# iangitonga/tinyllama.cpp

Measured on AMD Instinct MI355X. Metric: decode tok/s TinyLlama-1.1B q4 ctx=2048, 1 GPU; achieved HBM GB/s vs peak, higher is better.
Workload: dtype q4 weights x q8 activations (int8 dot, f32 accumulate); 1 GPU; TinyLlama-1.1B q4 greedy single-token decode, batch 1 per GPU, steps end at n=2048 (BASELINE.json configs[3]); ctx=2048, graph=True, steps_per_graph_replay=4, kv_cache=q8 blocks (reference layout), argmax=device, parallelism=replicas x1

## Files before the change

### __graft_entry__.py

```python
import importlib.util
import os
import sys

ROOT = os.path.dirname(os.path.abspath(__file__))
PKG_DIR = os.path.join(ROOT, "tinyllama.cpp_amd")
PKG_NAME = "tinyllama_cpp_amd"


def load_package():
    if PKG_NAME in sys.modules:
        return sys.modules[PKG_NAME]
    spec = importlib.util.spec_from_file_location(
        PKG_NAME, os.path.join(PKG_DIR, "__init__.py"), submodule_search_locations=[PKG_DIR])
    mod = importlib.util.module_from_spec(spec)
    sys.modules[PKG_NAME] = mod
    spec.loader.exec_module(mod)
    return mod


def build():
    pkg = load_package()
    pkg.build.build_all()
    if ROOT not in sys.path:
        sys.path.insert(0, ROOT)
    from oracle import orc
    orc.build(ref=os.path.isdir("/root/reference"))
    if os.path.isdir("/root/reference"):
        orc.build_dropin()
    build_neighbour()
    api = pkg.hipabi.GtenHip()
    for name in api.SYMBOLS + api.SAMPLE_SYMBOLS + api.SCORE_SYMBOLS + api.PREFIX_SYMBOLS + api.PREFIX_DECODE_SYMBOLS + api.BIAS_SYMBOLS + api.LOGPROBS_SYMBOLS + api.NUCLEUS_SYMBOLS + api.PENALTY_SYMBOLS + api.FSM_SYMBOLS + api.REGEX_SYMBOLS + api.PREFIXES_SYMBOLS + api.GROUPS_SYMBOLS + api.CONTINUE_SYMBOLS + api.BEAM_SYMBOLS:
        getattr(api.lib, name)
    host = pkg.hostabi.GtenHost()
    for name in host.SYMBOLS + host.SAMPLE_SYMBOLS + host.SCORE_SYMBOLS + host.PREFIX_SYMBOLS + host.PREFIX_DECODE_SYMBOLS + host.BIAS_SYMBOLS + host.LOGPROBS_SYMBOLS + host.NUCLEUS_SYMBOLS + host.PENALTY_SYMBOLS + host.FSM_SYMBOLS + host.REGEX_SYMBOLS + host.PREFIXES_SYMBOLS + host.SAMPLES_SYMBOLS + host.SESSIONS_SYMBOLS + host.BEAM_SYMBOLS:
        getattr(host.lib, name)


def build_neighbour():
    import shutil
    import subprocess
    d = os.path.join(ROOT, "tools", "mfma_neighbour")
    src, lib = os.path.join(d, "neighbour.hip"), os.path.join(d, "libneighbour.so")
    hipcc = shutil.which("hipcc") or "/opt/rocm/bin/hipcc"
    if not os.path.exists(src) or not os.path.exists(hipcc):
        return
    if not os.path.exists(lib) or os.path.getmtime(lib) < os.path.getmtime(src):
        subprocess.run([hipcc, "--offload-arch=gfx950", "-O2", "-shared", "-fPIC", "-o", lib, src], check=True, capture_output=True)


def smoke():
    if ROOT not in sys.path:
        sys.path.insert(0, ROOT)
    sys.path.insert(0, os.path.join(ROOT, "tests"))
    pkg = load_package()
    from smoke_check import run_smoke
    run_smoke(pkg)


if __name__ == "__main__":
    build()
    print("build ok")
```

### include/gten_hip_ab.h

```cpp
#pragma once

#ifdef __cplusplus
extern "C" {
#endif

int gten_hip_set_decode_attn_classic(int v);

#ifdef __cplusplus
}
#endif
```

### tinyllama.cpp_amd/build.py

```python
import os
import shutil
import subprocess

PKG = os.path.dirname(os.path.abspath(__file__))
ROOT = os.path.dirname(PKG)
CSRC = os.path.join(PKG, "csrc")
HOST = os.path.join(PKG, "host")
INCLUDE = os.path.join(ROOT, "include")

HIP_LIB = os.path.join(CSRC, "libgten_hip.so")
HOST_LIB = os.path.join(HOST, "libgten_host.so")

HIPCC = shutil.which("hipcc") or "/opt/rocm/bin/hipcc"
HIP_FLAGS = ["--offload-arch=gfx950", "-O3", "-std=c++17", "-ffp-contract=off", "-fno-slp-vectorize",
             "-Xclang", "-target-feature", "-Xclang", "-packed-fp32-ops", "-fPIC", "-shared",
             "-mllvm", "-amdgpu-kernarg-preload-count=16",
             "-Wall", "-Wno-unused-function", "-I" + INCLUDE]
CXX_FLAGS = ["-std=c++17", "-O2", "-fopenmp", "-fPIC", "-shared", "-Wall", "-I" + INCLUDE, "-I" + PKG]


_EXTRA = os.environ.get("GTEN_HIP_EXTRA_FLAGS", "").split()
HIP_FLAGS += _EXTRA
_FLAGS_STAMP = os.path.join(CSRC, "_obj", "flags.txt")


def _newer(target, sources):
    if not os.path.exists(target):
        return True
    t = os.path.getmtime(target)
    return any(os.path.getmtime(s) > t for s in sources)


def _sources(d, exts):
    out = []
    for base, _, files in os.walk(d):
        out += [os.path.join(base, f) for f in files if f.endswith(exts)]
    return sorted(out)


HIP_FILE_FLAGS = {}
HIP_OBJ = os.path.join(CSRC, "_obj")


def build_hip(force=False):
    from concurrent.futures import ThreadPoolExecutor
    srcs = _sources(CSRC, (".hip",))
    hdrs = _sources(CSRC, (".h",)) + _sources(INCLUDE, (".h",)) + [os.path.abspath(__file__)]
    os.makedirs(HIP_OBJ, exist_ok=True)
    compile_flags = [f for f in HIP_FLAGS if f != "-shared"]
    stamp = " ".join(_EXTRA)
    if (open(_FLAGS_STAMP).read() if os.path.exists(_FLAGS_STAMP) else "") != stamp:
        force = True
        with open(_FLAGS_STAMP, "w") as f:
            f.write(stamp)
    jobs, objs = [], []
    for src in srcs:
        obj = os.path.join(HIP_OBJ, os.path.basename(src) + ".o")
        objs.append(obj)
        if force or _newer(obj, [src] + hdrs):
            jobs.append([HIPCC] + compile_flags + HIP_FILE_FLAGS.get(os.path.basename(src), []) + ["-c", "-o", obj, src])
    if jobs:
        with ThreadPoolExecutor(max_workers=4) as pool:
            for r in pool.map(lambda cmd: subprocess.run(cmd, capture_output=True, text=True), jobs):
                if r.returncode != 0:
                    raise RuntimeError("hipcc failed: " + " ".join(r.args) + "\n" + r.stderr[-4000:])
    if jobs or force or _newer(HIP_LIB, objs):
        subprocess.run([HIPCC, "--offload-arch=gfx950", "-shared", "-fPIC", "-o", HIP_LIB] + objs, check=True)
    return HIP_LIB


HOST_CLI = os.path.join(HOST, "tinyllama_cli")
CLI_SRC = os.path.join(HOST, "tinyllama_cli.cpp")


def build_host(force=False):
    srcs = [s for s in _sources(HOST, (".cpp",)) if s != CLI_SRC]
    if not srcs:
        return None
    deps = srcs + _sources(HOST, (".h",)) + _sources(os.path.join(PKG, "gten"), (".h",)) + _sources(INCLUDE, (".h",))
    if force or _newer(HOST_LIB, deps) or _newer(HOST_LIB, [HIP_LIB]):
        subprocess.run(["g++"] + CXX_FLAGS + ["-o", HOST_LIB] + srcs +
                       ["-L" + CSRC, "-lgten_hip", "-Wl,-rpath,$ORIGIN/../csrc"], check=True)
    if os.path.exists(CLI_SRC) and (force or _newer(HOST_CLI, deps + [CLI_SRC]) or _newer(HOST_CLI, [HIP_LIB])):
        cli_flags = [f for f in CXX_FLAGS if f not in ("-shared", "-fPIC")]
        subprocess.run(["g++"] + cli_flags + ["-o", HOST_CLI, CLI_SRC, "-L" + CSRC, "-lgten_hip", "-Wl,-rpath,$ORIGIN/../csrc"], check=True)
    return HOST_LIB


def build_all(force=False):
    build_hip(force)
    build_host(force)
```

### tinyllama.cpp_amd/csrc/gten_decode.hip

```cpp
#include "gten_dev.h"
#include "gten_rt.h"
#include "gten_hip_sample.h"
#include "gten_hip_bias.h"
#include "gten_hip_logprobs.h"
#include "gten_hip_nucleus.h"
#include "gten_hip_penalty.h"
#include "gten_hip_fsm.h"
#include "gten_hip_regex.h"
#include "gten_hip_ab.h"
#include "gten_hip_prefix_decode.h"
#include "gten_hip_prefixes.h"
#include "gten_hip_groups.h"

#include <cmath>
#include <vector>
#include <algorithm>

#define DEC_SHARE_RECORDS (GTEN_PREFIXES_MAX + GTEN_GROUPS_MAX)

using namespace gtd;

extern __shared__ __attribute__((aligned(16))) uint8_t g_smem[];

#define DEC_CHUNK 256
#define ATT1V_VROW 68
#define ATT1V_PCOL 72
#define DEC_MAX_LANES 4
#define DEC_ATT_MAXCH 8
#define GEMVM_F16_LDS_LIMIT 65536

static int g_only_family = -1;
#define DEC_LAUNCH(tag, kernel, grid, block, smem, ...)                                        \
    do {                                                                                       \
        if (g_only_family < 0 || g_only_family == (tag)) GTR_LAUNCH(tag, kernel, grid, block, smem, __VA_ARGS__); \
    } while (0)

#define DEC_LAUNCH_HOT(tag, kernel, grid, block, smem, hw, a) \
    DEC_LAUNCH(tag, kernel, grid, block, smem, (hw).w[0], (hw).w[1], (hw).w[2], (hw).w[3], (hw).w[4], (hw).w[5], (hw).w[6], a)

struct DecStep {
    int n;
    int advance;
    int stop;
};


struct ActStage {
    float* row;
    float* red;
    ActQ8 q8;
};

__device__ __forceinline__ ActStage carve_stage(int d)
{
    ActStage s;
    s.red = (float*)g_smem;
    s.row = (float*)(g_smem + 64);
    s.q8 = actq8_carve(g_smem + 64 + (size_t)d * 4, d >> 5);
    return s;
}
static size_t stage_bytes(int d) { return 64 + (size_t)d * 4 + (size_t)(d >> 5) * 40; }

enum { PRO_EMBED = 0, PRO_RESID = 1, PRO_ATT = 2, PRO_ATTW = 3, PRO_ACTQ8 = 4 };
enum { EPI_RAW = 0, EPI_SILUMUL = 1, EPI_STAGE = 2, EPI_STAGE_FRAG = 3 };

#define WXP_PLANES 8
#include "gten_decode_wx.h"
#include "gten_decode_wide_wx.h"
#include "gten_decode_ffn.h"
#include "gten_decode_wxp.h"
#include "gten_decode_attn.h"
#include "gten_decode_attn_w.h"
#include "gten_decode_attn_exact64.h"
#include "gten_decode_attn_wide.h"
#include "gten_decode_attn_hm.h"
#include "gten_decode_sample.h"
#include "gten_decode_logprobs.h"
static_assert(LP_TOP == GTEN_HIP_LOGPROBS_TOP && sizeof(LpRecord) == GTEN_HIP_LOGPROBS_RECORD_BYTES, "gten_decode_logprobs.h and include/gten_hip_logprobs.h disagree");
#include "gten_decode_nucleus.h"
static_assert(CUT_MASS_BITS == GTEN_HIP_NUCLEUS_MASS_BITS && sizeof(CutInfo) == GTEN_HIP_NUCLEUS_INFO_BYTES && sizeof(CutInfo) == sizeof(gten_hip_cut_info),
              "gten_decode_nucleus.h and include/gten_hip_nucleus.h disagree");
#include "gten_decode_penalty.h"
#include "gten_decode_fsm.h"


using namespace gtr;

struct CapturedGraph { hipGraph_t graph; hipGraphExec_t exec; };

struct SamplerState {
    SampleParam* samp = nullptr;
    std::vector<SampleParam> samp_host;
    int n_sampling = 0;
    float* bias = nullptr;
    int n_bound = 0;
    bool bias_on = false;
    LpRecord* lp = nullptr;
    int n_asking = 0;
    bool lp_on = false;
    CutParam* cut = nullptr;
    std::vector<CutParam> cut_host;
    bool cut_on = false;
    PenParam* pen = nullptr;
    std::vector<PenParam> pen_host;
    int n_penalised = 0;
    size_t pen_lds = 0;
    bool pen_on = false;
    uint16_t* fsm_next = nullptr;
    uint8_t* fsm_flags = nullptr;
    std::vector<uint8_t> fsm_flags_host;
    int fsm_states = 0;
    FsmParam* fsm = nullptr;
    std::vector<FsmParam> fsm_host;
    int32_t* fsm_state = nullptr;
    int n_fsm = 0;
    bool fsm_on = false;
    uint8_t* vocab_bytes = nullptr;
    int32_t* vocab_offsets = nullptr;
    long long vocab_n_bytes = 0;
};

struct gten_hip_decoder {
    gten_hip_decoder_desc d;
    std::vector<gten_hip_layer_ptrs> layers;
    DecStep* step = nullptr;
    int32_t* tokens = nullptr;
    int32_t* result = nullptr;
    int32_t* ids_stage = nullptr;
    float *qkv_raw = nullptr, *proj_raw = nullptr, *down_raw = nullptr;
    float *scores = nullptr, *stats = nullptr, *att_part = nullptr;
    uint8_t *xbuf = nullptr, *hbuf = nullptr;
    float* act_f = nullptr;
    int8_t* act_q = nullptr;
    float* act_d = nullptr;
    int* act_sum = nullptr;
    float* best_val = nullptr;
    int* best_idx = nullptr;
    int n_best = 0;
    std::vector<DecStep> slots;
    int dev_n = -1;
    std::vector<int> dev_ns;
    int only_family = -1;
    int n_seq = 1;
    const void** kv_tab = nullptr;
    std::vector<const void*> kv_real;
    std::vector<char> kv_parked;
    void* dummy_kv = nullptr;
    int8_t* stg_q = nullptr;
    float* stg_d = nullptr;
    int* stg_sum = nullptr;
    float* stg_f = nullptr;
    float* logits_m = nullptr;
    float* gu_raw = nullptr;
    int n_chunks = 0;
    CapturedGraph graphs[2][2][1 << DEC_MAX_LANES] = {};
    SamplerState smp;
    unsigned lane_mask = 0;
    int last_run_lanes = 0;
    const float2* rope = nullptr;
    float2* rope_now = nullptr;
    bool exact = false;
    int attn_classic = 0;
    bool persist_on = false;
    struct PersistState* persist = nullptr;
    uint8_t* hm = nullptr;
    size_t hm_seq_stride = 0, hm_cache_bytes = 0, hm_chunk_bytes = 0;
    std::vector<char> hm_dirty;
    unsigned long long hm_imports = 0, hm_import_launches = 0;
    struct Pfx {
        uint8_t* hm = nullptr;
        const void** tab = nullptr;
        DecStep* step = nullptr;
        std::vector<const void*> kv;
        int len = 0;
        char dirty = 0;
        bool stale = false;
        unsigned long long imports = 0;
    } pfx[DEC_SHARE_RECORDS];
    int* share_dev = nullptr;
    int* which_dev = nullptr;
    uint8_t** pfx_hm_tab = nullptr;
    bool pfxn = false;
    std::vector<int> share_rows, share_cur, share_which, which_cur;
    unsigned long long hm_skip_imports = 0;
    unsigned long long watch_epoch = 0;
    bool watch_foreign = false;
    int lanes = 1;
    hipStream_t lane_stream[DEC_MAX_LANES] = {nullptr, nullptr, nullptr, nullptr};
    hipEvent_t lane_fork = nullptr, lane_join[DEC_MAX_LANES] = {nullptr, nullptr, nullptr, nullptr};
    struct BeamSearch* beam = nullptr;
};
static hipError_t beam_destroy(gten_hip_decoder* dc);

static inline bool sampler_on(const gten_hip_decoder* dc) { return dc->smp.n_sampling + dc->smp.n_bound + dc->smp.n_asking + dc->smp.n_penalised + dc->smp.n_fsm > 0; }

struct StepEnd {
    int rows;
    const float* logits; int row_stride;
    const SampleParam* samp;
    DecStep* step;
    int32_t* result; int result_stride;
    int32_t* tokens;
    LpRecord* lp;
    const CutParam* cut;
    const PenParam* pen;
    const FsmParam* fsm; int32_t* fsm_state;
    const float* best_val; const int* best_idx; int n_best, best_stride;
};

static int launch_step_end(gten_hip_decoder* dc, const StepEnd& e)
{
    const SamplerState& s = dc->smp;
    const int V = dc->d.n_vocab, tok_stride = dc->d.max_ctx + 1, rec_stride = dc->d.max_ctx + 2;
    const dim3 grid(e.rows), block(SMP_THREADS);
    const bool on = sampler_on(dc);
    if (on && s.fsm_on)
        DEC_LAUNCH(KT_DEC_SAMPLE, k_dec_sample_fsm, grid, block, s.pen_lds, e.logits, V, e.row_stride, e.samp, e.step, e.result, e.result_stride, e.tokens,
                   tok_stride, (const float*)s.bias, e.lp, rec_stride, e.cut, e.pen, (const uint16_t*)s.fsm_next, (const uint8_t*)s.fsm_flags, s.fsm_states,
                   e.fsm, e.fsm_state);
    else if (on && s.pen_on)
        DEC_LAUNCH(KT_DEC_SAMPLE, k_dec_sample_pen, grid, block, s.pen_lds, e.logits, V, e.row_stride, e.samp, e.step, e.result, e.result_stride, e.tokens,
                   tok_stride, (const float*)s.bias, e.lp, rec_stride, e.cut, e.pen);
    else if (on && s.cut_on)
        DEC_LAUNCH(KT_DEC_SAMPLE, k_dec_sample_cut, grid, block, 0, e.logits, V, e.row_stride, e.samp, e.step, e.result, e.result_stride, e.tokens, tok_stride,
                   (const float*)s.bias, e.lp, rec_stride, e.cut);
    else if (on && s.lp_on)
        DEC_LAUNCH(KT_DEC_SAMPLE, k_dec_sample_lp, grid, block, 0, e.logits, V, e.row_stride, e.samp, e.step, e.result, e.result_stride, e.tokens, tok_stride,
                   (const float*)s.bias, e.lp, rec_stride);
    else if (on && s.bias_on)
        DEC_LAUNCH(KT_DEC_SAMPLE, k_dec_sample_b, grid, block, 0, e.logits, V, e.row_stride, e.samp, e.step, e.result, e.result_stride, e.tokens, tok_stride,
                   (const float*)s.bias);
    else if (on)
        DEC_LAUNCH(KT_DEC_SAMPLE, k_dec_sample, grid, block, 0, e.logits, V, e.row_stride, e.samp, e.step, e.result, e.result_stride, e.tokens, tok_stride);
    else
        DEC_LAUNCH(KT_DEC_ARGMAX, k_dec_argmax, grid, dim3(1024), 0, e.best_val, e.best_idx, e.n_best, e.step, e.result, e.best_stride, e.result_stride,
                   e.tokens, tok_stride);
    return 0;
}

struct LaneBufs {
    int n_seq;
    DecStep* step; int32_t* tokens; int32_t* result; const SampleParam* samp; LpRecord* lp; const CutParam* cut; const PenParam* pen;
    const FsmParam* fsm; int32_t* fsm_state;
    float *qkv_raw, *proj_raw, *down_raw, *scores, *stats, *att_part;
    uint8_t *xbuf, *hbuf;
    float* act_f; int8_t* act_q; float* act_d; int* act_sum;
    const void** kv_tab;
    int8_t* stg_q; float* stg_d; int* stg_sum; float* stg_f;
    float* logits_m; float* gu_raw; float2* rope_now;
};
static LaneBufs lane_bufs(const gten_hip_decoder* dc, int lane)
{
    const gten_hip_decoder_desc& d = dc->d;
    const size_t SL = (size_t)(dc->n_seq / dc->lanes), o = (size_t)lane * SL;
    const size_t E = (size_t)d.n_embd, F = (size_t)d.n_ffn, dh = E / d.n_heads, KV = dh * d.n_kv_heads, V = (size_t)d.n_vocab;
    const size_t planes = dc->n_seq >= 16 ? 2 : 1, H = (size_t)d.n_heads, C = (size_t)dc->n_chunks;
    LaneBufs b;
    b.n_seq = (int)SL;
    b.step = dc->step + o; b.tokens = dc->tokens + o * (d.max_ctx + 1); b.result = dc->result + o * (d.max_ctx + 2); b.samp = dc->smp.samp + o;
    b.lp = dc->smp.lp ? dc->smp.lp + o * (d.max_ctx + 2) : nullptr;
    b.cut = dc->smp.cut ? dc->smp.cut + o : nullptr;
    b.pen = dc->smp.pen ? dc->smp.pen + o : nullptr;
    b.fsm = dc->smp.fsm ? dc->smp.fsm + o : nullptr;
    b.fsm_state = dc->smp.fsm_state ? dc->smp.fsm_state + o * (d.max_ctx + 2) : nullptr;
    const size_t rplanes = dc->n_seq >= 16 ? (size_t)WXP_PLANES : 1;
    b.qkv_raw = dc->qkv_raw + o * rplanes * (E + 2 * KV);
    b.proj_raw = dc->proj_raw + o * rplanes * E; b.down_raw = dc->down_raw + o * rplanes * E;
    b.scores = dc->scores + o * H * d.max_ctx; b.stats = dc->stats + o * H * C * 2; b.att_part = dc->att_part + o * H * C * dh;
    b.xbuf = dc->xbuf + o * E * 4; b.hbuf = dc->hbuf + o * E * 4;
    b.act_f = dc->act_f + o * F; b.act_q = dc->act_q + o * 2 * F; b.act_d = dc->act_d + o * (F / 32); b.act_sum = dc->act_sum + o * (F / 32);
    b.kv_tab = dc->kv_tab ? dc->kv_tab + o * d.n_layers * 2 : nullptr;
    b.stg_q = dc->stg_q ? dc->stg_q + o * 2 * E : nullptr; b.stg_d = dc->stg_d ? dc->stg_d + o * (E / 32) : nullptr;
    b.stg_sum = dc->stg_sum ? dc->stg_sum + o * (E / 32) : nullptr; b.stg_f = dc->stg_f ? dc->stg_f + o * E : nullptr;
    b.logits_m = dc->logits_m ? dc->logits_m + o * V : nullptr; b.gu_raw = dc->gu_raw ? dc->gu_raw + o * planes * 2 * F : nullptr;
    b.rope_now = dc->rope_now + o * (dh / 2);
    return b;
}

static bool g_decode_exact = false;
static bool g_exact_now = false;
static bool g_lane_skip = false;
static bool g_kv_head_major = true;
#define PFX_SHARED_DEFAULT true
static bool g_pfx_shared = PFX_SHARED_DEFAULT;
struct PfxArgs { const uint8_t* k = nullptr; const int* share = nullptr; const uint8_t* const* tab = nullptr; size_t layer_off = 0; const int* which = nullptr; };
extern "C" int gten_hip_set_kv_head_major(int on)
{
    g_kv_head_major = on != 0;
    return 0;
}
extern "C" int gten_hip_set_decode_exact(int on)
{
    g_decode_exact = on != 0;
    return 0;
}
static int g_attn_classic = 0;
static int g_attn_classic_now = 0;
extern "C" int gten_hip_set_decode_attn_classic(int v)
{
    GTR_REQUIRE(v >= 0 && v <= 2, "gten_hip_set_decode_attn_classic: %d is not 0, 1 or 2", v);
    g_attn_classic = v;
    return 0;
}

static bool attention_grouped_ok(const AttnArgs& t, int n_seq)
{
    const int grp = t.n_heads / t.n_kv;
    const int min_seq = 8;
    if (t.adtype == GTEN_F16 && n_seq < 16) return false;
    return n_seq >= min_seq && (t.adtype == GTEN_Q8 || t.adtype == GTEN_F16) && t.d_head == 64 && (grp == 8 || grp == 4 || grp == 2 || grp == 1);
}

static int grp_shift1_of(int n_heads, int n_kv)
{
    const int grp = n_heads / n_kv;
    return (grp > 0 && (grp & (grp - 1)) == 0) ? __builtin_ctz(grp) + 1 : 0;
}

static bool attention_one_pass(int d_head);

static bool grouped_mm(const AttnArgs& t, int n_seq)
{
    return n_seq >= 16 && t.adtype == GTEN_Q8 && t.d_head == 64 && !g_exact_now;
}

static bool grouped_hm_f16(const AttnArgs& t, int n_seq)
{
    return n_seq >= 16 && t.adtype == GTEN_F16 && t.d_head == 64 && t.hm_k && !g_exact_now;
}

static bool grouped_one_pass(const AttnArgs& t, int n_seq)
{
    if (grouped_mm(t, n_seq) || grouped_hm_f16(t, n_seq)) return true;
    return attention_one_pass(t.d_head) && t.adtype == GTEN_Q8 && n_seq <= 8;
}

template <int GRP, int ADT>
static int launch_attention_g(const AttnArgs& t, int n_seq, const PfxArgs& pfx)
{
    constexpr size_t NW = (ADT == GTEN_Q8) ? 17 : 32;
    const dim3 grid(n_seq, t.n_chunks, t.n_kv);
    if constexpr (ADT == GTEN_Q8) if (grouped_mm(t, n_seq) && t.hm_k) {
        const int n_cq = (t.n_chunks + HM_WAVES - 1) / HM_WAVES;
        if (pfx.tab) {
            if (n_seq >= 128)
                DEC_LAUNCH(KT_DEC_ATTN_SCORE, (k_dec_attn_hm_pfxn<GRP, true>), dim3(n_seq * n_cq * t.n_kv), dim3(64 * HM_WAVES), 2048, t, n_seq, n_cq, pfx.tab, pfx.layer_off, pfx.share, pfx.which);
            else
                DEC_LAUNCH(KT_DEC_ATTN_SCORE, (k_dec_attn_hm_pfxn<GRP, false>), dim3(n_seq * n_cq * t.n_kv), dim3(64 * HM_WAVES), 2048, t, n_seq, n_cq, pfx.tab, pfx.layer_off, pfx.share, pfx.which);
            return 0;
        }
        if (pfx.k) {
            if (n_seq >= 128)
                DEC_LAUNCH(KT_DEC_ATTN_SCORE, (k_dec_attn_hm_pfx<GRP, true>), dim3(n_seq * n_cq * t.n_kv), dim3(64 * HM_WAVES), 2048, t, n_seq, n_cq, pfx.k, pfx.share);
            else
                DEC_LAUNCH(KT_DEC_ATTN_SCORE, (k_dec_attn_hm_pfx<GRP, false>), dim3(n_seq * n_cq * t.n_kv), dim3(64 * HM_WAVES), 2048, t, n_seq, n_cq, pfx.k, pfx.share);
            return 0;
        }
        if (n_seq >= 128) DEC_LAUNCH(KT_DEC_ATTN_SCORE, (k_dec_attn_hm<GRP, true>), dim3(n_seq * n_cq * t.n_kv), dim3(64 * HM_WAVES), 2048, t, n_seq, n_cq);
        else DEC_LAUNCH(KT_DEC_ATTN_SCORE, (k_dec_attn_hm<GRP, false>), dim3(n_seq * n_cq * t.n_kv), dim3(64 * HM_WAVES), 2048, t, n_seq, n_cq);
        return 0;
    }
    if constexpr (ADT == GTEN_Q8) if (grouped_mm(t, n_seq)) {
        const size_t smem = (size_t)DEC_CHUNK * 68 + 2 * 8 * 264 * 2 + 16 * 64 + 32 * 4 + 8 * 4 + (size_t)4 * (DEC_MAXGRP + 2) * 2 + 128 + 128 * 4 + 80 + 64;
        GTR_REQUIRE((n_seq * t.n_chunks) % 8 == 0, "decoder: %d sequences x %d chunks is not a multiple of 8", n_seq, t.n_chunks);
        DEC_LAUNCH(KT_DEC_ATTN_SCORE, (k_dec_attn_mm_g<GRP>), dim3(n_seq * t.n_chunks * t.n_kv), dim3(256), smem, t, n_seq);
        return 0;
    }
    if constexpr (ADT == GTEN_Q8) if (grouped_one_pass(t, n_seq)) {
        constexpr size_t GP = (GRP + 1) / 2;
        const size_t smem = (size_t)(8 * GRP + 4 * GRP + 8 + 64) * 4 + (size_t)4 * (GRP + 2) * 2 + (size_t)(GRP + 2) * 64 + 16 +
                            (ADT == GTEN_Q8 ? 0 : (size_t)(GRP + 1) * 64 * 4) + 2 * GP * DEC_CHUNK * 4 + (size_t)DEC_CHUNK * NW * 4;
        DEC_LAUNCH(KT_DEC_ATTN_SCORE, (k_dec_attn_one_g<GRP, true, ADT>), grid, dim3(256), smem, t);
        return 0;
    }
    const size_t smem1 = (size_t)(8 * GRP + 4 * GRP + 8 + 64) * 4 + (size_t)4 * (GRP + 2) * 2 + (size_t)(GRP + 2) * 64 + 64 +
                         (ADT == GTEN_Q8 ? 0 : (size_t)(GRP + 1) * 64 * 4 + 16);
    const size_t smem2 = (size_t)((GRP + 1) / 2 * 2) * DEC_CHUNK * 4 + (size_t)DEC_CHUNK * NW * 4 + (size_t)(16 + 8 * GRP) * 4;
    const bool exact = n_seq <= 8 || g_exact_now;
    if (smem2 > 64 * 1024) {
        GTR_CHECK(hipFuncSetAttribute((const void*)k_dec_attn_pv_g<GRP, true, ADT>, hipFuncAttributeMaxDynamicSharedMemorySize, (int)smem2));
        GTR_CHECK(hipFuncSetAttribute((const void*)k_dec_attn_pv_g<GRP, false, ADT>, hipFuncAttributeMaxDynamicSharedMemorySize, (int)smem2));
    }
    if constexpr (ADT == GTEN_F16) if (grouped_hm_f16(t, n_seq)) {
        const int n_cq = (t.n_chunks + HM_WAVES - 1) / HM_WAVES;
// ... 74 lines not shown
            if (g_attn_classic_now == 0) {
                if (t.adtype == GTEN_Q8) {
                    GTR_CHECK(hipFuncSetAttribute((const void*)k_dec_attn_one64w<GTEN_Q8>, hipFuncAttributeMaxDynamicSharedMemorySize, (int)smem_v));
                    DEC_LAUNCH_HOT(KT_DEC_ATTN_SCORE, k_dec_attn_one64w<GTEN_Q8>, g64, dim3(512), smem_v, hw, t);
                } else {
                    GTR_CHECK(hipFuncSetAttribute((const void*)k_dec_attn_one64w<GTEN_F16>, hipFuncAttributeMaxDynamicSharedMemorySize, (int)smem_v));
                    DEC_LAUNCH_HOT(KT_DEC_ATTN_SCORE, k_dec_attn_one64w<GTEN_F16>, g64, dim3(512), smem_v, hw, t);
                }
                return 0;
            }
            if (t.adtype == GTEN_Q8) {
                GTR_CHECK(hipFuncSetAttribute((const void*)k_dec_attn_one64v<GTEN_Q8>, hipFuncAttributeMaxDynamicSharedMemorySize, (int)smem_v));
                DEC_LAUNCH_HOT(KT_DEC_ATTN_SCORE, k_dec_attn_one64v<GTEN_Q8>, g64, dim3(256), smem_v, hw, t);
            } else {
                GTR_CHECK(hipFuncSetAttribute((const void*)k_dec_attn_one64v<GTEN_F16>, hipFuncAttributeMaxDynamicSharedMemorySize, (int)smem_v));
                DEC_LAUNCH_HOT(KT_DEC_ATTN_SCORE, k_dec_attn_one64v<GTEN_F16>, g64, dim3(256), smem_v, hw, t);
            }
            return 0;
        }
        if (t.adtype == GTEN_Q8) {
            if (multi) DEC_LAUNCH_HOT(KT_DEC_ATTN_SCORE, (k_dec_attn_one64<GTEN_Q8, true>), g64, dim3(256), smem, hw, t);
            else DEC_LAUNCH_HOT(KT_DEC_ATTN_SCORE, (k_dec_attn_one64<GTEN_Q8, false>), g64, dim3(256), smem, hw, t);
        } else {
            if (multi) DEC_LAUNCH_HOT(KT_DEC_ATTN_SCORE, (k_dec_attn_one64<GTEN_F16, true>), g64, dim3(256), smem, hw, t);
            else DEC_LAUNCH_HOT(KT_DEC_ATTN_SCORE, (k_dec_attn_one64<GTEN_F16, false>), g64, dim3(256), smem, hw, t);
        }
        return 0;
    }
    if (t.d_head == 64) {
        const size_t nw = (t.adtype == GTEN_Q8) ? 17 : 32;
        const size_t smem2 = (size_t)2 * DEC_CHUNK * 4 + (size_t)DEC_CHUNK * nw * 4;
        const unsigned long long geo = (unsigned long long)(unsigned)t.kv_pitch | ((unsigned long long)(unsigned)t.max_ctx << 32);
        const unsigned long long heads = ((unsigned long long)(unsigned)t.n_heads << 32) | ((unsigned long long)(unsigned)t.n_kv << 40) |
                                         ((unsigned long long)(unsigned)t.grp_shift1 << 48);
        const AttnHotWords hs{{(unsigned long long)(uintptr_t)t.qkv_raw, (unsigned long long)(uintptr_t)t.rope_now, (unsigned long long)(uintptr_t)t.kcache,
                               (unsigned long long)(uintptr_t)t.step, geo, (unsigned long long)(unsigned)t.n_embd | heads, (unsigned long long)(uintptr_t)t.scores}};
        const AttnHotWords hp{{(unsigned long long)(uintptr_t)t.scores, (unsigned long long)(uintptr_t)t.stats, (unsigned long long)(uintptr_t)t.vcache,
                               (unsigned long long)(uintptr_t)t.step, geo, (unsigned long long)(unsigned)t.n_chunks | heads, (unsigned long long)(uintptr_t)t.att_part}};
        const bool multi = agrid.z > 1 || t.kv_tab != nullptr;
        const dim3 g64(agrid.y, agrid.x, agrid.z);
#define ATT_LAUNCH2(ADT, MULTI)                                                                                                          \
        do {                                                                                                                             \
            DEC_LAUNCH_HOT(KT_DEC_ATTN_SCORE, (k_dec_attn_score64<ADT, MULTI>), g64, dim3(256), smem1, hs, t);                           \
            DEC_LAUNCH_HOT(KT_DEC_ATTN_PV, (k_dec_attn_pv64<ADT, MULTI>), g64, dim3(256), smem2, hp, t);                                 \
        } while (0)
        if (t.adtype == GTEN_Q8) { if (multi) ATT_LAUNCH2(GTEN_Q8, true); else ATT_LAUNCH2(GTEN_Q8, false); }
        else { if (multi) ATT_LAUNCH2(GTEN_F16, true); else ATT_LAUNCH2(GTEN_F16, false); }
#undef ATT_LAUNCH2
        return 0;
    }
    DEC_LAUNCH(KT_DEC_ATTN_SCORE, k_dec_attn_score, agrid, dim3(256), smem1, t);
    DEC_LAUNCH(KT_DEC_ATTN_PV, k_dec_attn_pv, agrid, dim3(256), (size_t)2 * DEC_CHUNK * 4, t);
    return 0;
}

template <int WT, int PRO>
static GemvHotWords hot_of(const Gemv8Args& a)
{
    GemvHotWords hw;
    GemvHot& h = hw.h;
    if (PRO == PRO_RESID) { h.p0 = a.res_raw; h.p1 = a.res_a; h.p2 = a.norm_w; }
    else if (PRO == PRO_EMBED) { h.p0 = a.table; h.p1 = a.tokens; h.p2 = a.norm_w; }
    else if (PRO == PRO_ATT || PRO == PRO_ATTW) {
        h.p0 = a.att_part; h.p1 = (const void*)(uintptr_t)((unsigned)a.d_head_shift | ((unsigned)a.n_chunks << 8));
        h.p2 = (PRO == PRO_ATTW) ? a.att_stats : nullptr;
    }
    else { h.p0 = (WT == GTEN_F16) ? (const void*)a.act_f : (const void*)a.act_q; h.p1 = a.act_d; h.p2 = a.act_sum; }
    h.qs0 = a.qs[0]; h.ds0 = a.ds[0]; h.d_in = a.d_in; h.rows0 = a.rows[0]; h.step = a.step;
    return hw;
}

template <int WT, int PRO>
static GemvHotWords hot_of_gemv8(const Gemv8Args& a)
{
    GemvHotWords hw = hot_of<WT, PRO>(a);
    const unsigned long long r1 = a.n_mats > 1 ? (unsigned)a.rows[1] : 0u, r2 = a.n_mats > 2 ? (unsigned)a.rows[2] : 0u;
    hw.w[4] = (unsigned long long)(uintptr_t)(a.n_mats > 1 ? a.qs[1] : nullptr);
    hw.w[5] = (unsigned long long)(unsigned)a.d_in | ((unsigned long long)(unsigned)a.rows[0] << 16) | (r1 << 32) | (r2 << 48);
    hw.w[6] = (PRO == PRO_RESID) ? (unsigned long long)(uintptr_t)(a.n_mats > 2 ? a.qs[2] : nullptr) : (unsigned long long)(uintptr_t)a.step;
    return hw;
}

template <int WT, int PRO, int NCH, int R, int NT, int NM = 0>
static int launch_gemv8(int tag, const Gemv8Args& a, int total_rows)
{
    const int rows_per_wg = (NT / 64) * R;
    const dim3 grid((total_rows + rows_per_wg - 1) / rows_per_wg), block(NT);
    for (int k = 0; k + 1 < a.n_mats; k++) GTR_REQUIRE(a.rows[k] % R == 0, "decoder: concatenated matrices must hold a multiple of %d rows", R);
    const GemvHotWords hw = hot_of_gemv8<WT, PRO>(a);
    DEC_LAUNCH_HOT(tag, (k_dec_gemv8<WT, PRO, NCH, R, EPI_RAW, NT, NM>), grid, block, stage_bytes((PRO == PRO_ACTQ8 && WT != GTEN_F16) ? 32 : a.d_in), hw, a);
    return 0;
}

template <int WT>
static int launch_gateup8(const Gemv8Args& a, int n_ffn)
{
    const dim3 grid(n_ffn / 32), block(512);
    GTR_REQUIRE(n_ffn % 32 == 0, "decoder: n_ffn %d is not a multiple of 32", n_ffn);
    const GemvHotWords hw = hot_of_gemv8<WT, PRO_RESID>(a);
    DEC_LAUNCH_HOT(KT_DEC_GEMV_GATEUP, (k_dec_gemv8<WT, PRO_RESID, (WT == GTEN_F16 ? 4 : 1), 8, EPI_SILUMUL, 512>), grid, block, stage_bytes(a.d_in), hw, a);
    return 0;
}

static void set_mat(Gemv8Args& a, int k, const void* w, int wdtype, int rows, int cols)
{
    const size_t nb = (size_t)cols / 32;
    a.qs[k] = (const uint8_t*)w;
    a.ds[k] = (wdtype == GTEN_F16) ? nullptr
                                   : (const uint16_t*)((const uint8_t*)w + (size_t)rows * nb * (wdtype == GTEN_Q4 ? 16 : 32));
    a.rows[k] = rows;
}

template <int WT>
static int enqueue_step_q8act(gten_hip_decoder* dc)
{
    const gten_hip_decoder_desc& d = dc->d;
    const int E = d.n_embd, F = d.n_ffn, dh = E / d.n_heads, KV = dh * d.n_kv_heads;
    const size_t kv_pitch = gten_hip_row_bytes(d.adtype, KV);
    constexpr bool F16W = (WT == GTEN_F16);
    constexpr int NE = F16W ? 4 : 1;
    constexpr int NF = F16W ? 11 : 3;
    constexpr int NF12 = F16W ? 12 : NF;
    const bool wideF = F > 2048, widerF = F16W && F > NF * 512;
    float* xbuf = (float*)dc->xbuf;
    float* hbuf = (float*)dc->hbuf;
    int rc;
    for (int l = 0; l < d.n_layers; l++) {
        const gten_hip_layer_ptrs& L = dc->layers[l];
        Gemv8Args a{};
        a.step = dc->step; a.d_in = E; a.n_mats = 3;
        set_mat(a, 0, L.wq, WT, E, E); set_mat(a, 1, L.wk, WT, KV, E); set_mat(a, 2, L.wv, WT, KV, E);
        a.out = dc->qkv_raw; a.norm_w = (const uint16_t*)L.attn_norm; a.x_out = xbuf;
        if (l == 0) {
            a.table = d.embed; a.rope = dc->rope; a.rope_now = dc->rope_now; a.rope_half = dh / 2; a.n_vocab = d.n_vocab; a.tokens = dc->tokens;
            rc = launch_gemv8<WT, PRO_EMBED, NE, 2, 512>(KT_DEC_GEMV_QKV, a, E + 2 * KV);
        } else {
            a.res_a = hbuf; a.res_raw = dc->down_raw;
            rc = launch_gemv8<WT, PRO_RESID, NE, 2, 512>(KT_DEC_GEMV_QKV, a, E + 2 * KV);
        }
        if (rc) return rc;
        AttnArgs t{};
        t.step = dc->step; t.qkv_raw = dc->qkv_raw; t.kcache = (uint8_t*)L.kcache; t.vcache = (uint8_t*)L.vcache;
        t.kv_pitch = kv_pitch; t.scores = dc->scores; t.stats = dc->stats; t.att_part = dc->att_part; t.rope = dc->rope; t.rope_now = dc->rope_now;
        t.adtype = d.adtype; t.n_heads = d.n_heads; t.n_kv = d.n_kv_heads; t.d_head = dh; t.max_ctx = d.max_ctx;
        t.n_chunks = dc->n_chunks; t.n_embd = E;
        const dim3 agrid(d.n_heads, dc->n_chunks);
        const size_t smem1 = (size_t)(16 + 3 * dh + 16) * 4 + 32 + (size_t)3 * dh + 64;
        if (int arc = launch_attention(t, agrid, smem1)) return arc;
        Gemv8Args o{};
        o.step = dc->step; o.d_in = E; o.n_mats = 1; set_mat(o, 0, L.wo, WT, E, E); o.out = dc->proj_raw;
        o.att_part = dc->att_part; o.d_head = dh; o.d_head_shift = __builtin_ctz(dh); o.n_chunks = dc->n_chunks;
        o.att_stats = dc->stats;
        rc = attention_one_pass(dh) ? launch_gemv8<WT, PRO_ATTW, NE, 1, 512, 1>(KT_DEC_GEMV_O, o, E)
                                    : launch_gemv8<WT, PRO_ATT, NE, 1, 512, 1>(KT_DEC_GEMV_O, o, E);
        if (rc) return rc;
        Gemv8Args gu{};
        gu.step = dc->step; gu.d_in = E; gu.n_mats = 2; set_mat(gu, 0, L.wgate, WT, F, E); set_mat(gu, 1, L.wup, WT, F, E);
        gu.res_a = xbuf; gu.res_raw = dc->proj_raw; gu.x_out = hbuf; gu.norm_w = (const uint16_t*)L.ffn_norm;
        gu.act_q = dc->act_q; gu.act_d = dc->act_d; gu.act_sum = dc->act_sum; gu.act_f = dc->act_f;
        if ((rc = launch_gateup8<WT>(gu, F))) return rc;
        Gemv8Args dn{};
        dn.step = dc->step; dn.d_in = F; dn.n_mats = 1; set_mat(dn, 0, L.wdown, WT, E, F); dn.out = dc->down_raw;
        dn.act_q = dc->act_q; dn.act_d = dc->act_d; dn.act_sum = dc->act_sum;
        dn.act_f = dc->act_f;
        rc = widerF ? launch_gemv8<WT, PRO_ACTQ8, NF12, 2, 256, 1>(KT_DEC_GEMV_DOWN, dn, E)
             : wideF ? launch_gemv8<WT, PRO_ACTQ8, NF, 2, 256, 1>(KT_DEC_GEMV_DOWN, dn, E)
                     : launch_gemv8<WT, PRO_ACTQ8, NE, 2, 256, 1>(KT_DEC_GEMV_DOWN, dn, E);
        if (rc) return rc;
    }
    Gemv8Args hd{};
    hd.step = dc->step; hd.d_in = E; hd.n_mats = 1; set_mat(hd, 0, d.lm_head, WT, d.n_vocab, E); hd.out = d.logits;
    hd.res_a = hbuf; hd.res_raw = dc->down_raw; hd.x_out = nullptr; hd.norm_w = (const uint16_t*)d.final_norm;
    hd.best_val = dc->best_val; hd.best_idx = dc->best_idx;
    if ((rc = launch_gemv8<WT, PRO_RESID, NE, F16W ? 4 : 8, 512, 1>(KT_DEC_GEMV_HEAD, hd, d.n_vocab))) return rc;
    return launch_step_end(dc, StepEnd{1, d.logits, 0, dc->smp.samp, dc->step, dc->result, 0, dc->tokens, dc->smp.lp, dc->smp.cut, dc->smp.pen, dc->smp.fsm, dc->smp.fsm_state,
                                       dc->best_val, dc->best_idx, dc->n_best, 0});
}

template <int WT, int PRO>
static int launch_stage(int tag, Gemv8Args a, int n_seq)
{
    const GemvHotWords hw = hot_of_gemv8<WT, PRO>(a);
    DEC_LAUNCH_HOT(tag, (k_dec_gemv8<WT, PRO, 1, 1, EPI_STAGE, 512>), dim3(n_seq), dim3(512), stage_bytes(a.d_in), hw, a);
    return 0;
}

template <int WT, int PRO>
static int launch_stage_frag(int tag, Gemv8Args a, int n_seq)
{
    a.frag_rt = (n_seq + 15) / 16;
    const GemvHotWords hw = hot_of_gemv8<WT, PRO>(a);
    DEC_LAUNCH_HOT(tag, (k_dec_gemv8<WT, PRO, 1, 1, EPI_STAGE_FRAG, 512>), dim3(n_seq), dim3(512), stage_bytes(a.d_in), hw, a);
    return 0;
}

static size_t gemvm_lds_bytes(int wt, int n_seq, int d, bool silumul)
{
    size_t b = silumul ? (size_t)n_seq * 64 * 4 : 0;
    if (wt == GTEN_F16) b += ((size_t)n_seq * ((d + 511) / 512 * 512) * 4 <= GEMVM_F16_LDS_LIMIT) ? (size_t)n_seq * d * 4 : 0;
    else b += (size_t)n_seq * (d + (size_t)(d / 32) * 8);
    return b + 16;
}

template <int WT, int NCH, int R, int S, int NT>
static int launch_gemvm(int tag, const Gemv8Args& a, int total_rows)
{
    const int rows_per_wg = (NT / 64) * R;
    for (int k = 0; k + 1 < a.n_mats; k++) GTR_REQUIRE(a.rows[k] % R == 0, "decoder: concatenated matrices must hold a multiple of %d rows", R);
    const GemvHotWords hw = hot_of<WT, PRO_ACTQ8>(a);
    const size_t lds = gemvm_lds_bytes(WT, S, a.d_in, false);
    static bool raised = false;
    if (lds > 64 * 1024 && !raised) {
        GTR_CHECK(hipFuncSetAttribute((const void*)k_dec_gemvm<WT, NCH, R, S, EPI_RAW, NT>, hipFuncAttributeMaxDynamicSharedMemorySize, (int)lds));
        raised = true;
    }
    DEC_LAUNCH_HOT(tag, (k_dec_gemvm<WT, NCH, R, S, EPI_RAW, NT>), dim3((total_rows + rows_per_wg - 1) / rows_per_wg), dim3(NT), lds, hw, a);
    return 0;
}

template <int WT, int S>
static int enqueue_step_multi(gten_hip_decoder* dc)
{
    const gten_hip_decoder_desc& d = dc->d;
    const int E = d.n_embd, F = d.n_ffn, dh = E / d.n_heads, KV = dh * d.n_kv_heads, V = d.n_vocab;
    const size_t kv_pitch = gten_hip_row_bytes(d.adtype, KV);
    constexpr bool F16W = (WT == GTEN_F16);
    constexpr int NE = F16W ? 4 : 1, NF = F16W ? 11 : 3, NF12 = F16W ? 12 : NF;
    constexpr int RH = F16W ? 2 : 4;
    const bool wideF = F > 2048, widerF = F16W && F > NF * 512;
    float* xbuf = (float*)dc->xbuf;
    float* hbuf = (float*)dc->hbuf;
    int rc;
    Gemv8Args base{};
    base.step = dc->step; base.tok_stride = d.max_ctx + 1; base.part_stride = d.n_heads * dc->n_chunks * dh;
    base.best_stride = dc->n_best;
    for (int l = 0; l < d.n_layers; l++) {
        const gten_hip_layer_ptrs& L = dc->layers[l];
        Gemv8Args st = base;
        st.d_in = E; st.norm_w = (const uint16_t*)L.attn_norm; st.x_out = xbuf;
        st.act_q = dc->stg_q; st.act_d = dc->stg_d; st.act_sum = dc->stg_sum; st.act_f = dc->stg_f;
        if (l == 0) {
            st.table = d.embed; st.rope = dc->rope; st.rope_now = dc->rope_now; st.rope_half = dh / 2; st.n_vocab = V; st.tokens = dc->tokens;
            rc = launch_stage<WT, PRO_EMBED>(KT_DEC_STAGE, st, S);
        } else {
            st.res_a = hbuf; st.res_raw = dc->down_raw; st.raw_stride = E;
            rc = launch_stage<WT, PRO_RESID>(KT_DEC_STAGE, st, S);
        }
        if (rc) return rc;
        Gemv8Args a = base;
        a.d_in = E; a.n_mats = 3;
        set_mat(a, 0, L.wq, WT, E, E); set_mat(a, 1, L.wk, WT, KV, E); set_mat(a, 2, L.wv, WT, KV, E);
        a.out = dc->qkv_raw; a.raw_stride = E + 2 * KV;
        a.act_q = dc->stg_q; a.act_d = dc->stg_d; a.act_sum = dc->stg_sum; a.act_f = dc->stg_f;
        if ((rc = launch_gemvm<WT, NE, 2, S, 256>(KT_DEC_GEMV_QKV, a, E + 2 * KV))) return rc;
        AttnArgs t{};
        t.step = dc->step; t.qkv_raw = dc->qkv_raw; t.kv_pitch = kv_pitch; t.scores = dc->scores; t.stats = dc->stats;
        t.att_part = dc->att_part; t.rope = dc->rope; t.rope_now = dc->rope_now;
// ... 642 lines not shown
    dc->layers.assign(layers, layers + d.n_layers);
    dc->n_chunks = (d.max_ctx + DEC_CHUNK - 1) / DEC_CHUNK;
    static_assert(GTEN_ROPE_MAX_POS <= DEC_ATT_MAXCH * DEC_CHUNK, "max_ctx (checked above) bounds the attention chunks the consumers request up front");
    const int E = d.n_embd, F = d.n_ffn, KV = dh * d.n_kv_heads;
    const size_t S = (size_t)n_seq;
    GTR_CHECK(hipMalloc((void**)&dc->step, S * sizeof(DecStep)));
    GTR_CHECK(hipMemset(dc->step, 0, S * sizeof(DecStep)));
    GTR_CHECK(hipMalloc((void**)&dc->tokens, S * (size_t)(d.max_ctx + 1) * 4));
    GTR_CHECK(hipMemset(dc->tokens, 0, S * (size_t)(d.max_ctx + 1) * 4));
    GTR_CHECK(hipMalloc((void**)&dc->result, S * (size_t)(d.max_ctx + 2) * 4));
    GTR_CHECK(hipMemset(dc->result, 0, S * (size_t)(d.max_ctx + 2) * 4));
    GTR_CHECK(hipMalloc((void**)&dc->smp.samp, S * sizeof(SampleParam)));
    GTR_CHECK(hipMemset(dc->smp.samp, 0, S * sizeof(SampleParam)));
    dc->smp.samp_host.assign(S, SampleParam{});
    const size_t planes = wide ? 2 : 1;
    GTR_CHECK(hipMalloc((void**)&dc->qkv_raw, (wide ? (size_t)WXP_PLANES : 1) * S * (size_t)(E + 2 * KV) * 4));
    GTR_CHECK(hipMalloc((void**)&dc->proj_raw, (wide ? (size_t)WXP_PLANES : 1) * S * (size_t)E * 4));
    GTR_CHECK(hipMalloc((void**)&dc->down_raw, (wide ? (size_t)WXP_PLANES : 1) * S * (size_t)E * 4));
    GTR_CHECK(hipMalloc((void**)&dc->scores, S * (size_t)d.n_heads * d.max_ctx * 4));
    GTR_CHECK(hipMalloc((void**)&dc->stats, (S * (size_t)d.n_heads * dc->n_chunks * 2 + 16) * 4));
    GTR_CHECK(hipMemset(dc->stats, 0, (S * (size_t)d.n_heads * dc->n_chunks * 2 + 16) * 4));
    GTR_CHECK(hipMalloc((void**)&dc->att_part, S * (size_t)d.n_heads * dc->n_chunks * dh * 4));
    GTR_CHECK(hipMalloc((void**)&dc->xbuf, S * (size_t)E * 4));
    GTR_CHECK(hipMalloc((void**)&dc->hbuf, S * (size_t)E * 4));
    const size_t stage_rows = wide ? 2 * ((S + 15) / 16 * 16) : S;
    GTR_CHECK(hipMalloc((void**)&dc->act_q, stage_rows * (size_t)F));
    GTR_CHECK(hipMemset(dc->act_q, 0, stage_rows * (size_t)F));
    GTR_CHECK(hipMalloc((void**)&dc->act_d, S * (size_t)(F / 32) * 4));
    GTR_CHECK(hipMalloc((void**)&dc->act_sum, S * (size_t)(F / 32) * 4));
    GTR_CHECK(hipMalloc((void**)&dc->act_f, S * (size_t)F * 4));
    {
        const int r = (n_seq == 1) ? (d.wdtype == GTEN_F16 ? 4 : 8) : (d.wdtype == GTEN_F16 ? 2 : 4);
        dc->n_best = ((d.n_vocab + 8 * r - 1) / (8 * r)) * 8;
    }
    GTR_CHECK(hipMalloc((void**)&dc->best_val, S * (size_t)dc->n_best * 4));
    GTR_CHECK(hipMalloc((void**)&dc->best_idx, S * (size_t)dc->n_best * 4));
    if (n_seq > 1) {
        GTR_CHECK(hipMalloc((void**)&dc->stg_q, stage_rows * (size_t)E));
        GTR_CHECK(hipMemset(dc->stg_q, 0, stage_rows * (size_t)E));
        GTR_CHECK(hipMalloc((void**)&dc->stg_d, S * (size_t)(E / 32) * 4));
        GTR_CHECK(hipMalloc((void**)&dc->stg_sum, S * (size_t)(E / 32) * 4));
        GTR_CHECK(hipMalloc((void**)&dc->stg_f, S * (size_t)E * 4));
        GTR_CHECK(hipMalloc((void**)&dc->logits_m, S * (size_t)d.n_vocab * 4));
        if (wide) {
            GTR_CHECK(hipMalloc((void**)&dc->gu_raw, planes * S * (size_t)2 * F * 4));
            if (d.wdtype != GTEN_F16)
            {
                if (int rc = (d.wdtype == GTEN_Q4) ? mmv_prepare<GTEN_Q4>() : mmv_prepare<GTEN_Q8>()) return rc;
                if (int rc = (d.wdtype == GTEN_Q4) ? mmvh_prepare<GTEN_Q4>() : mmvh_prepare<GTEN_Q8>()) return rc;
            }
        }
        std::vector<const void*> tab(S * d.n_layers * 2);
        for (size_t q = 0; q < S; q++)
            for (int l = 0; l < d.n_layers; l++) {
                const gten_hip_kv_ptrs& p = kv[q * d.n_layers + l];
                tab[(q * d.n_layers + l) * 2] = p.kcache;
                tab[(q * d.n_layers + l) * 2 + 1] = p.vcache;
            }
        GTR_CHECK(hipMalloc((void**)&dc->kv_tab, tab.size() * sizeof(void*)));
        GTR_CHECK(hipMemcpy(dc->kv_tab, tab.data(), tab.size() * sizeof(void*), hipMemcpyHostToDevice));
        dc->kv_real = tab;
        dc->kv_parked.assign(S, 0);
        const size_t cache_bytes = (size_t)d.max_ctx * gten_hip_row_bytes(d.adtype, KV);
        GTR_CHECK(hipMalloc(&dc->dummy_kv, 2 * cache_bytes));
        GTR_CHECK(hipMemset(dc->dummy_kv, 0, 2 * cache_bytes));
        const int grp = d.n_heads / d.n_kv_heads;
        if (wide && g_kv_head_major && !dc->exact && (d.adtype == GTEN_Q8 || d.adtype == GTEN_F16) && dh == 64 && (grp == 8 || grp == 4 || grp == 2 || grp == 1)) {
            dc->hm_chunk_bytes = d.adtype == GTEN_Q8 ? HM_CHUNK_BYTES : HMF_CHUNK_BYTES;
            dc->hm_cache_bytes = (size_t)d.n_kv_heads * dc->n_chunks * dc->hm_chunk_bytes;
            dc->hm_seq_stride = (size_t)d.n_layers * 2 * dc->hm_cache_bytes;
            GTR_CHECK(hipMalloc((void**)&dc->hm, S * dc->hm_seq_stride));
            GTR_CHECK(hipMemset(dc->hm, 0, S * dc->hm_seq_stride));
            dc->hm_dirty.assign(S, 1);
            for (size_t q = 0; q < S; q++)
                for (size_t i = 0; i < (size_t)d.n_layers * 2; i++)
                    kv_watch_add(dc->kv_real[q * d.n_layers * 2 + i], cache_bytes, dc, &dc->hm_dirty[q]);
        }
    }
    if (int rc = rope_table(dh, &dc->rope)) return rc;
    GTR_CHECK(hipMalloc((void**)&dc->rope_now, S * (size_t)(dh / 2) * sizeof(float2)));
    GTR_CHECK(hipMemset(dc->rope_now, 0, S * (size_t)(dh / 2) * sizeof(float2)));
    if (dc->persist_on && n_seq == 1 && !dc->exact)
        if (int rc = persist_prepare(dc)) return rc;
    return 0;
}

#if GTEN_WITH_PERSIST
static int g_cu_count = -1;
static int persist_prepare(gten_hip_decoder* dc)
{
    if (dc->persist) return 0;
    if (!g_persist_all.empty()) { dc->persist_on = false; return 0; }
    if (g_cu_count < 0) {
        int dev = 0;
        GTR_CHECK(hipGetDevice(&dev));
        hipDeviceProp_t prop;
        GTR_CHECK(hipGetDeviceProperties(&prop, dev));
        g_cu_count = prop.multiProcessorCount;
    }
    const gten_hip_decoder_desc& d = dc->d;
    if (!persist_supported(d, dc->n_seq, dc->n_chunks, g_cu_count)) { dc->persist_on = false; return 0; }
    const int G = g_cu_count, E = d.n_embd, F = d.n_ffn, dh = E / d.n_heads, KV = dh * d.n_kv_heads;
    auto* ps = new PersistState;
    dc->persist = ps;
    g_persist_all.push_back(ps);
    std::vector<PLayer> tab((size_t)d.n_layers);
    for (int l = 0; l < d.n_layers; l++) {
        const gten_hip_layer_ptrs& L = dc->layers[l];
        tab[l] = PLayer{(const uint8_t*)L.wq, (const uint8_t*)L.wk, (const uint8_t*)L.wv, (const uint8_t*)L.wo, (const uint8_t*)L.wgate,
                        (const uint8_t*)L.wup, (const uint8_t*)L.wdown, (const uint16_t*)L.attn_norm, (const uint16_t*)L.ffn_norm,
                        (uint8_t*)L.kcache, (uint8_t*)L.vcache};
    }
    GTR_CHECK(hipMalloc((void**)&ps->layers, tab.size() * sizeof(PLayer)));
    GTR_CHECK(hipMemcpy(ps->layers, tab.data(), tab.size() * sizeof(PLayer), hipMemcpyHostToDevice));
    GTR_CHECK(hipMalloc((void**)&ps->ctl, 64));
    const unsigned ctl0[16] = {1u, 0u};
    GTR_CHECK(hipMemcpy(ps->ctl, ctl0, 64, hipMemcpyHostToDevice));
    PArgs& a = ps->args;
    a.rpa = (E + 2 * KV + G - 1) / G; a.rpo = (E + G - 1) / G; a.rph = (d.n_vocab + G - 1) / G; a.rw = (a.rph + 7) / 8;
    const size_t n_q = (size_t)G * a.rpa, n_part = (size_t)d.n_heads * dc->n_chunks * 66, n_att = (size_t)E, n_proj = (size_t)G * a.rpo,
                 n_act = (size_t)10 * (F / 32) + 8, n_down = (size_t)G * a.rpo, n_best = (size_t)2 * G;
    const size_t total = n_q + n_part + n_att + n_proj + n_act + n_down + n_best + 64;
    GTR_CHECK(hipMalloc((void**)&ps->gran, total * 8));
    GTR_CHECK(hipMemset(ps->gran, 0, total * 8));
    pu64* p = ps->gran;
    a.gq = p; p += n_q; a.gpart = p; p += n_part; a.gatt = p; p += n_att; a.gproj = p; p += n_proj;
    a.gact = p; p += (n_act + 7) / 8 * 8; a.gdown = p; p += n_down; a.gbest = p;
    if (const char* e = getenv("GTEN_HIP_PERSIST_STAMPS"); e && e[0] == '1') {
        ps->n_stamps = d.n_layers * 20 + 8;
        GTR_CHECK(hipMalloc((void**)&ps->stamps, (size_t)(d.n_layers * 20 + 8) * 4));
        GTR_CHECK(hipMemset(ps->stamps, 0, (size_t)(d.n_layers * 20 + 8) * 4));
    }
    a.layers = ps->layers; a.step = dc->step; a.tokens = dc->tokens; a.result = dc->result;
    a.embed = (const uint8_t*)d.embed; a.final_norm = (const uint16_t*)d.final_norm; a.lm_head = (const uint8_t*)d.lm_head;
    a.logits = d.logits; a.rope = dc->rope; a.ctl = ps->ctl; a.stamps = ps->stamps;
    a.n_layers = d.n_layers; a.E = E; a.F = F; a.KV = KV; a.n_heads = d.n_heads; a.n_kv = d.n_kv_heads; a.n_vocab = d.n_vocab;
    a.max_ctx = d.max_ctx; a.n_chunks = dc->n_chunks; a.kv_pitch = (int)gten_hip_row_bytes(d.adtype, KV);
    ps->grid = G;
    ps->smem = persist_smem();
    GTR_CHECK(hipFuncSetAttribute((const void*)k_dec_persist<GTEN_Q4>, hipFuncAttributeMaxDynamicSharedMemorySize, (int)ps->smem));
    return 0;
}
static hipError_t persist_free(gten_hip_decoder* dc)
{
    if (!dc->persist) return hipSuccess;
    PersistState* ps = dc->persist;
    g_persist_all.erase(std::remove(g_persist_all.begin(), g_persist_all.end(), ps), g_persist_all.end());
    hipError_t first = hipSuccess;
    for (void* b : {(void*)ps->layers, (void*)ps->ctl, (void*)ps->gran, (void*)ps->stamps})
        if (b) { const hipError_t e = hipFree(b); if (e != hipSuccess && first == hipSuccess) first = e; }
    delete ps;
    dc->persist = nullptr;
    return first;
}
#else
static int persist_prepare(gten_hip_decoder* dc) { dc->persist_on = false; return 0; }
static hipError_t persist_free(gten_hip_decoder*) { return hipSuccess; }
#endif

static hipError_t drop_graphs(gten_hip_decoder* dc)
{
    hipError_t first = hipSuccess;
    auto rel = [&](hipError_t e) { if (e != hipSuccess && first == hipSuccess) first = e; };
    for (auto& by_steps : dc->graphs)
        for (auto& by_slot : by_steps)
            for (CapturedGraph& c : by_slot) {
// ... 978 lines not shown
```

### tinyllama.cpp_amd/csrc/gten_decode_wx.h

```cpp

template <typename T>
__device__ __forceinline__ const T* from_word(unsigned long long w)
{
    return (const T*)(const __attribute__((address_space(1))) T*)w;
}
template <typename T>
__device__ __forceinline__ void store_global(void* p, T v)
{
    *(__attribute__((address_space(1))) T*)(uintptr_t)p = v;
}

struct Gemv8Args {
    const DecStep* step;
    const uint8_t* qs[3];
    const uint16_t* ds[3];
    int rows[3];
    int n_mats;
    int d_in;
    float* out;
    const void* table; int n_vocab; const int32_t* tokens;
    const float* res_a; const float* res_raw;
    float* x_out;
    const uint16_t* norm_w;
    const float* att_part; int d_head, n_chunks;
// ... 83 lines not shown
{
    float amax = 0.f;
#pragma unroll
    for (int i = 0; i < EPT; i++) amax = fmaxf(amax, fabsf(v[i]));
    const Q8Scale s = q8_scale_from_absmax(grp_max<EPT>(amax));
    int q[EPT], sum = 0;
#pragma unroll
    for (int i = 0; i < EPT; i++) { q[i] = q8_round(v[i], s.scale); sum += q[i]; }
    const int k = sub * EPT;
    if (a.h16) {
        uint16_t* hd = (uint16_t*)a.q + ((((size_t)b * a.rt + (a.row >> 4)) * 64 + (k >> 3) * 16 + (a.row & 15)) * 8 + (k & 7));
        unsigned hw[EPT / 2];
#pragma unroll
        for (int i = 0; i < EPT; i += 4) {
            hw[i / 2] = (unsigned)f2h((float)q[i] * s.ddeq) | ((unsigned)f2h((float)q[i + 2] * s.ddeq) << 16);
            hw[i / 2 + 1] = (unsigned)f2h((float)q[i + 1] * s.ddeq) | ((unsigned)f2h((float)q[i + 3] * s.ddeq) << 16);
        }
        if (EPT == 8) *(uint4*)hd = make_uint4(hw[0], hw[1], hw[EPT / 2 - 2], hw[EPT / 2 - 1]);
        else *(uint2*)hd = make_uint2(hw[0], hw[1]);
        return;
    }
    int8_t* dst = a.q + ((((size_t)b * a.rt + (a.row >> 4)) * 64 + (k >> 3) * 16 + (a.row & 15)) * 8 + (k & 7));
    const int lo = (q[0] & 0xff) | ((q[1] & 0xff) << 8) | ((q[2] & 0xff) << 16) | ((q[3] & 0xff) << 24);
    if (EPT == 8) {
        int2 pk;
        pk.x = lo;
        pk.y = (q[EPT - 4] & 0xff) | ((q[EPT - 3] & 0xff) << 8) | ((q[EPT - 2] & 0xff) << 16) | ((q[EPT - 1] & 0xff) << 24);
        *(int2*)dst = pk;
    } else {
        *(int*)dst = lo;
    }
    sum = grp_sum_i<EPT>(sum);
    if (sub == 0) { a.d[(size_t)b * 16 * a.rt + a.row] = s.ddeq; a.sum[(size_t)b * 16 * a.rt + a.row] = sum; }
}

template <int EPT> __device__ __forceinline__ void ldN(const float* p, float (&v)[EPT])
{
    const float4 a = ((const float4*)p)[0];
    v[0] = a.x; v[1] = a.y; v[2] = a.z; v[3] = a.w;
    if (EPT == 8) {
        const float4 b = ((const float4*)p)[1];
        v[EPT - 4] = b.x; v[EPT - 3] = b.y; v[EPT - 2] = b.z; v[EPT - 1] = b.w;
    }
}
template <int EPT> __device__ __forceinline__ void stN(float* p, const float (&v)[EPT])
{
    ((float4*)p)[0] = make_float4(v[0], v[1], v[2], v[3]);
    if (EPT == 8) ((float4*)p)[1] = make_float4(v[EPT - 4], v[EPT - 3], v[EPT - 2], v[EPT - 1]);
}
template <int EPT> __device__ __forceinline__ float sumsq_treeN(const float (&v)[EPT])
{
    float s = (v[0] * v[0] + v[1] * v[1]) + (v[2] * v[2] + v[3] * v[3]);
    if (EPT == 8) s = s + ((v[EPT - 4] * v[EPT - 4] + v[EPT - 3] * v[EPT - 3]) + (v[EPT - 2] * v[EPT - 2] + v[EPT - 1] * v[EPT - 1]));
    return s;
}

__device__ __forceinline__ float max32(float v) { return nn_max32(v); }
__device__ __forceinline__ int sum32_i(int v) { return sum32_lanes_i(v); }
__device__ __forceinline__ float q8_round32(float v)
{
    const Q8Scale s = q8_scale_from_absmax(max32(fabsf(v)));
    return (float)q8_round(v, s.scale) * s.ddeq;
}
__device__ __forceinline__ float act_round32(float v, bool f16)
{
    return f16 ? h2f(f2h(v)) : q8_round32(v);
}

struct GemvHot {
    const void* p0;
    const void* p1;
    const void* p2;
    const uint8_t* qs0; const uint16_t* ds0;
    int d_in, rows0;
    const DecStep* step;
};
static_assert(sizeof(GemvHot) == 56, "seven 64-bit scalars: the preloadable part of the argument segment");
union GemvHotWords {
    unsigned long long w[7];
    GemvHot h;
    __host__ __device__ GemvHotWords() : w{0, 0, 0, 0, 0, 0, 0} {}
};

template <int WT, int PRO, int NCH, int R, int EPI, int NT, int NM = 0>
__global__ __launch_bounds__(NT) void k_dec_gemv8(const unsigned long long h0, const unsigned long long h1, const unsigned long long h2,
                                                  const unsigned long long h3, const unsigned long long h4, const unsigned long long h5,
                                                  const unsigned long long h6, const Gemv8Args a)
{
    GemvHot hot;
    hot.p0 = from_word<void>(h0); hot.p1 = from_word<void>(h1); hot.p2 = from_word<void>(h2);
    hot.qs0 = from_word<uint8_t>(h3);
    const uint8_t* hot_qs1 = from_word<uint8_t>(h4);
    hot.d_in = (int)(h5 & 0xffffu); hot.rows0 = (int)((h5 >> 16) & 0xffffu);
    const int hot_rows1 = (int)((h5 >> 32) & 0xffffu), hot_rows2 = (int)(h5 >> 48);
    const uint8_t* hot_qs2 = (PRO == PRO_RESID) ? from_word<uint8_t>(h6) : a.qs[2];
    hot.step = (PRO == PRO_RESID) ? nullptr : from_word<DecStep>(h6);
    constexpr int WBYTES = (WT == GTEN_Q4) ? 16 : 32;
    hot.ds0 = (const uint16_t*)(hot.qs0 + (size_t)hot.rows0 * (hot.d_in >> 5) * WBYTES);
    constexpr int EPT = 2048 / NT;
    constexpr int LPB = 32 / EPT;
    constexpr int NW = NT / 64;
    static_assert(NT == 256 || NT == 512, "256 or 512 threads");
    static_assert(EPI != EPI_SILUMUL || NT == 512, "the FFN slice epilogue wants 8 waves");
    constexpr bool F16W = (WT == GTEN_F16);
    const int d = hot.d_in, nb = d >> 5;
    ActStage s = carve_stage((PRO == PRO_ACTQ8 && !F16W) ? 32 : d);
    const int lane = threadIdx.x & 63, wid = threadIdx.x >> 6;
    constexpr bool STG = (EPI == EPI_STAGE || EPI == EPI_STAGE_FRAG);
    const int seq = STG ? blockIdx.x : 0;
    const int n = (PRO == PRO_RESID) ? 0 : hot.step[seq].n;
    const float* res_raw = (const float*)hot.p0 + (size_t)seq * a.raw_stride;
    const float* res_a = (const float*)hot.p1 + (size_t)seq * d;
    float* x_out = a.x_out ? a.x_out + (size_t)seq * d : nullptr;
    const int32_t* tokens = (const int32_t*)hot.p1 + (size_t)seq * a.tok_stride;
    constexpr bool ATT = (PRO == PRO_ATT || PRO == PRO_ATTW);
    const float* att_part = (const float*)hot.p0 + (size_t)seq * a.part_stride;
    const float* att_stats = (const float*)hot.p2 + (size_t)seq * a.stats_stride;
    const uint16_t* norm_w = (const uint16_t*)hot.p2;
    const int att_shift = (int)((uintptr_t)hot.p1 & 0xff), att_chunks = (int)(((uintptr_t)hot.p1 >> 8) & 0xffff), att_dh = 1 << att_shift;
    if (STG) {
        s.q8.q = a.act_q + (size_t)seq * d;
        s.q8.d = a.act_d + (size_t)seq * nb;
        s.q8.sum = a.act_sum + (size_t)seq * nb;
        if (F16W) s.row = a.act_f + (size_t)seq * d;
    }
    const bool stores_x = STG || blockIdx.x == 0;
    const int gi = threadIdx.x, base = gi * EPT, blk = gi / LPB, sub = gi % LPB;
    const bool on = base < d;
    const int sbase = on ? base : 0;

    float pin0[EPT], pin1[EPT];
#pragma unroll
    for (int i = 0; i < EPT; i++) { pin0[i] = 0.f; pin1[i] = 0.f; }
    if (PRO == PRO_RESID) { ldN<EPT>(res_raw + sbase, pin0); ldN<EPT>(res_a + sbase, pin1); }
    float pin0b[(STG && PRO == PRO_RESID) ? EPT : 1];
    if constexpr (STG && PRO == PRO_RESID) ldN<EPT>(res_raw + a.raw_plane + sbase, pin0b);
    float pinx[(STG && PRO == PRO_RESID) ? WXP_PLANES - 2 : 1][EPT];
    if constexpr (STG && PRO == PRO_RESID) {
        if (a.raw_nplanes == WXP_PLANES) {
#pragma unroll
            for (int q = 2; q < WXP_PLANES; q++) ldN<EPT>(res_raw + (size_t)q * a.raw_plane + sbase, pinx[q - 2]);
        }
    }
    unsigned nw[4] = {0, 0, 0, 0};
    if (PRO == PRO_EMBED || PRO == PRO_RESID) {
        if (EPT == 8) { const uint4 t = *(const uint4*)(norm_w + sbase); nw[0] = t.x; nw[1] = t.y; nw[2] = t.z; nw[3] = t.w; }
        else { const uint2 t = *(const uint2*)(norm_w + sbase); nw[0] = t.x; nw[1] = t.y; }
    }
    float apart[ATT ? DEC_ATT_MAXCH : 1][EPT];
    float2 cst[PRO == PRO_ATTW ? DEC_ATT_MAXCH : 1];
    if (PRO == PRO_ATTW) {
        const unsigned h = (unsigned)sbase >> att_shift;
#pragma unroll
        for (int j = 0; j < DEC_ATT_MAXCH; j++) cst[j] = ((const float2*)att_stats)[h * (unsigned)att_chunks + (unsigned)min(j, att_chunks - 1)];
    }
    if (ATT) {
        const unsigned h = (unsigned)sbase >> att_shift, e = (unsigned)sbase & (unsigned)(att_dh - 1);
        const unsigned row0 = h * (unsigned)att_chunks;
#pragma unroll
        for (int j = 0; j < DEC_ATT_MAXCH; j++)
            ldN<EPT>(att_part + (((row0 + (unsigned)min(j, att_chunks - 1)) << att_shift) + e), apart[j]);
    }
    unsigned emb[4] = {0, 0, 0, 0};
    float emb_delta = 0.f;
    if (PRO == PRO_EMBED && F16W) {
        const uint16_t* src = (const uint16_t*)hot.p0 + (size_t)tokens[n - 1] * d + sbase;
        if (EPT == 8) { const uint4 t = *(const uint4*)src; emb[0] = t.x; emb[1] = t.y; emb[2] = t.z; emb[3] = t.w; }
        else { const uint2 t = *(const uint2*)src; emb[0] = t.x; emb[1] = t.y; }
    }
    float2 rot_now = make_float2(1.f, 0.f);
    if (PRO == PRO_EMBED) rot_now = a.rope[(size_t)(n - 1) * a.rope_half + (threadIdx.x & (a.rope_half - 1))];
    if (PRO == PRO_EMBED && !F16W) {
        const int tok = tokens[n - 1];
        const int sb = on ? blk : 0, ssub = on ? sub : 0;
        const int byte0 = (ssub * EPT) & 15;
        const uint8_t* src;
        const uint16_t* dsp;
        if (WT == GTEN_Q4) {
            src = (const uint8_t*)hot.p0 + ((size_t)tok * nb + sb) * 16 + byte0;
            dsp = (const uint16_t*)((const uint8_t*)hot.p0 + (size_t)a.n_vocab * nb * 16);
        } else {
            src = (const uint8_t*)hot.p0 + (size_t)tok * nb * 32 + (size_t)((ssub * EPT) >> 4) * nb * 16 + (size_t)sb * 16 + byte0;
            dsp = (const uint16_t*)((const uint8_t*)hot.p0 + (size_t)a.n_vocab * nb * 32);
        }
        emb[0] = *(const unsigned*)src;
        if (EPT == 8) emb[1] = *(const unsigned*)(src + 4);
        emb_delta = h2f(dsp[(size_t)tok * nb + sb]);
    }

    const int rows0 = hot.rows0, rows1 = (NM != 1) ? hot_rows1 : 0, rows2 = (NM != 1) ? hot_rows2 : 0;
    const int total = rows0 + rows1 + rows2;
    const int r0 = (EPI == EPI_SILUMUL) ? (wid >> 2) * rows0 + blockIdx.x * 32 + (wid & 3) * R
                                        : (blockIdx.x * NW + wid) * R;
    uint4 wq[R][NCH], wq1[R][NCH];
    uint16_t wd[R][NCH];
    int lr0 = r0, rows_m = rows0;
    const uint8_t* qbase = hot.qs0;
    if (lr0 >= rows0 && rows1 > 0) {
        lr0 -= rows0; qbase = hot_qs1; rows_m = rows1;
        if (lr0 >= rows1 && rows2 > 0) { lr0 -= rows1; qbase = hot_qs2; rows_m = rows2; }
    }
    const uint16_t* dbase = (const uint16_t*)(qbase + (size_t)rows_m * nb * WBYTES);
#pragma unroll
    for (int j = 0; j < R; j++) {
        if (STG) break;
        const int lr = min(lr0 + j, rows_m - 1);
        const uint16_t* drow = dbase + (size_t)lr * nb;
#pragma unroll
        for (int c = 0; c < NCH; c++) {
            const int b = (c * 64 + lane < nb) ? c * 64 + lane : 0;
            if (F16W) {
                const int e = (c * 512 + lane * 8 < d) ? c * 512 + lane * 8 : 0;
                wq[j][c] = ld_w16((const uint16_t*)qbase + (size_t)lr * d + e);
                wq1[j][c] = make_uint4(0, 0, 0, 0);
                wd[j][c] = 0;
                continue;
            }
            if (WT == GTEN_Q4) {
                wq[j][c] = ld_w16((const uint4*)(qbase + (size_t)lr * nb * 16) + b);
            } else {
                const uint4* q0 = (const uint4*)(qbase + (size_t)lr * nb * 32);
                wq[j][c] = ld_w16(q0 + b);
                wq1[j][c] = ld_w16(q0 + nb + b);
            }
            wd[j][c] = ld_w2(drow + b);
        }
    }
    __builtin_amdgcn_sched_barrier(0);

    if (PRO != PRO_ACTQ8) {
        float v[EPT];
        float ss = 0.f;
        if (PRO == PRO_EMBED) {
#pragma unroll
            for (int i = 0; i < EPT; i++) {
                if (F16W) {
                    v[i] = h2f((uint16_t)((i & 1) ? (emb[i >> 1] >> 16) : (emb[i >> 1] & 0xffffu)));
                } else {
                    const unsigned byte = (emb[i >> 2] >> ((i & 3) * 8)) & 0xffu;
                    if (WT == GTEN_Q4) v[i] = (float)((((sub * EPT) < 16) ? (int)(byte >> 4) : (int)(byte & 0x0fu)) - 7) * emb_delta;
                    else v[i] = (float)(int)(int8_t)byte * emb_delta;
                }
            }
            if (WT == GTEN_Q4) q8_roundN<EPT>(v);
        } else if (PRO == PRO_RESID) {
#pragma unroll
            for (int i = 0; i < EPT; i++) v[i] = pin0[i];
            if constexpr (STG && PRO == PRO_RESID) {
#pragma unroll
                for (int i = 0; i < EPT; i++) v[i] += a.raw_plane ? pin0b[i] : 0.f;
                if (a.raw_nplanes == WXP_PLANES) {
#pragma unroll
                    for (int q = 2; q < WXP_PLANES; q++)
#pragma unroll
                        for (int i = 0; i < EPT; i++) v[i] += pinx[q - 2][i];
                }
            }
            act_roundN<WT, EPT>(v);
#pragma unroll
            for (int i = 0; i < EPT; i++) v[i] = pin1[i] + v[i];
            act_roundN<WT, EPT>(v);
        } else if (PRO == PRO_ATTW) {
            const int nch = (n + DEC_CHUNK - 1) / DEC_CHUNK;
            float M = -INFINITY;
#pragma unroll
            for (int j = 0; j < DEC_ATT_MAXCH; j++) M = fmaxf(M, (j < nch) ? cst[j].x : -INFINITY);
            float w[DEC_ATT_MAXCH], L = 0.f;
#pragma unroll
            for (int j = 0; j < DEC_ATT_MAXCH; j++) {
                w[j] = (j < nch) ? cst[j].y * __expf(cst[j].x - M) : 0.f;
                L += w[j];
            }
            const float rL = recip_rn(L);
#pragma unroll
            for (int j = 0; j < DEC_ATT_MAXCH; j++) w[j] = (nch == 1) ? 1.0f : w[j] * rL;
#pragma unroll
            for (int i = 0; i < EPT; i++) v[i] = 0.f;
#pragma unroll
            for (int j = 0; j < DEC_ATT_MAXCH; j++)
#pragma unroll
                for (int i = 0; i < EPT; i++) v[i] += (j < nch) ? w[j] * apart[j][i] : 0.f;
        } else {
            const int nch = (n + DEC_CHUNK - 1) / DEC_CHUNK;
#pragma unroll
            for (int i = 0; i < EPT; i++) v[i] = 0.f;
#pragma unroll
            for (int j = 0; j < DEC_ATT_MAXCH; j++)
#pragma unroll
                for (int i = 0; i < EPT; i++) v[i] += (j < nch) ? apart[j][i] : 0.f;
        }
        if (PRO == PRO_EMBED || PRO == PRO_RESID) {
            if (on) {
                if (x_out && stores_x) stN<EPT>(x_out + base, v);
                ss = sumsq_treeN<EPT>(v);
            }
            ss = block_sum_tree_n<NW, true>(ss, s.red);
            const float ms = ((d & (d - 1)) == 0) ? __builtin_ldexpf(ss, -__builtin_ctz(d)) : ss / (float)d;
            const float inv = recip_rn(sqrtf(ms) + 1e-6f);
#pragma unroll
            for (int i = 0; i < EPT; i++) {
                const uint16_t hw = (uint16_t)((i & 1) ? (nw[i >> 1] >> 16) : (nw[i >> 1] & 0xffffu));
                v[i] = v[i] * inv * h2f(hw);
            }
        }
        if (F16W) {
            act_roundN<WT, EPT>(v);
            if (EPI == EPI_STAGE_FRAG) {
                if (on) {
// ... 286 lines not shown
```

### tinyllama.cpp_amd/csrc/gten_dev.h

```cpp
#pragma once

#include <hip/hip_runtime.h>
#include <stdint.h>

#include "../../include/gten_hip.h"

#define GTEN_WAVE 64
#define GTEN_QBLK 32
#define GTEN_Q8_BYTES 34
#define GTEN_Q4_BYTES 18

namespace gtd {

__device__ __forceinline__ float h2f(uint16_t h)
{
    _Float16 x;
    __builtin_memcpy(&x, &h, 2);
    return (float)x;
}
__device__ __forceinline__ _Float16 f2hv(float f)
{
    asm("" : "+v"(f));
    return (_Float16)f;
}
__device__ __forceinline__ uint16_t f2h(float f)
{
    const _Float16 x = f2hv(f);
    uint16_t h;
    __builtin_memcpy(&h, &x, 2);
    return h;
}

#ifndef GTEN_NT_WEIGHTS
#define GTEN_NT_WEIGHTS 1
#endif
typedef unsigned gt_u4v __attribute__((ext_vector_type(4)));
__device__ __forceinline__ uint4 ld_w16(const void* p)
{
#if GTEN_NT_WEIGHTS
    const gt_u4v v = __builtin_nontemporal_load((const gt_u4v*)p);
#else
    const gt_u4v v = *(const gt_u4v*)p;
#endif
    return make_uint4(v.x, v.y, v.z, v.w);
}
__device__ __forceinline__ uint16_t ld_w2(const uint16_t* p)
{
#if GTEN_NT_WEIGHTS
    return __builtin_nontemporal_load(p);
#else
    return *p;
#endif
}

template <int CTRL, int ROW_MASK = 0xF>
__device__ __forceinline__ float dpp_mov(float v)
{
    return __int_as_float(__builtin_amdgcn_update_dpp(0, __float_as_int(v), CTRL, ROW_MASK, 0xF, false));
}
template <int CTRL, int ROW_MASK = 0xF>
__device__ __forceinline__ int dpp_mov_i(int v)
{
    return __builtin_amdgcn_update_dpp(0, v, CTRL, ROW_MASK, 0xF, false);
}
__device__ __forceinline__ float quad_max(float v)
{
    v = fmaxf(v, dpp_mov<0xB1>(v));
    return fmaxf(v, dpp_mov<0x4E>(v));
}
__device__ __forceinline__ int quad_sum_i(int v)
{
    v += dpp_mov_i<0xB1>(v);
    return v + dpp_mov_i<0x4E>(v);
}

template <int CTRL>
__device__ __forceinline__ int nn_max_step(int i)
{
    return max(i, __builtin_amdgcn_update_dpp(0, i, CTRL, 0xF, 0xF, false));
}
__device__ __forceinline__ float nn_max4(float v)
{
    int i = __float_as_int(v);
    i = nn_max_step<0xB1>(i);
    i = nn_max_step<0x4E>(i);
    return __int_as_float(i);
}
__device__ __forceinline__ float nn_max8(float v)
{
    int i = __float_as_int(nn_max4(v));
    i = nn_max_step<0x141>(i);
    return __int_as_float(i);
}
__device__ __forceinline__ float row16_absmax(float v)
{
    int i = __float_as_int(nn_max8(v));
    return __int_as_float(nn_max_step<0x140>(i));
}
__device__ __forceinline__ float nn_max32(float v)
{
    int i = __float_as_int(nn_max8(v));
    i = nn_max_step<0x140>(i);
    const auto r = __builtin_amdgcn_permlane16_swap(i, i, false, false);
    return __int_as_float(max((int)r[0], (int)r[1]));
}
__device__ __forceinline__ int sum32_lanes_i(int v)
{
    v += __builtin_amdgcn_update_dpp(0, v, 0xB1, 0xF, 0xF, false);
    v += __builtin_amdgcn_update_dpp(0, v, 0x4E, 0xF, 0xF, false);
    v += __builtin_amdgcn_update_dpp(0, v, 0x141, 0xF, 0xF, false);
    v += __builtin_amdgcn_update_dpp(0, v, 0x140, 0xF, 0xF, false);
    const auto r = __builtin_amdgcn_permlane16_swap(v, v, false, false);
    return (int)r[0] + (int)r[1];
}

__device__ __forceinline__ float wave_sum(float v)
{
    v += dpp_mov<0xB1>(v);
    v += dpp_mov<0x4E>(v);
    v += dpp_mov<0x141>(v);
    v += dpp_mov<0x140>(v);
    v += dpp_mov<0x142, 0xA>(v);
    v += dpp_mov<0x143, 0xC>(v);
    return __int_as_float(__builtin_amdgcn_readlane(__float_as_int(v), 63));
}
__device__ __forceinline__ float wave_max(float v)
{
#pragma unroll
    for (int o = 32; o > 0; o >>= 1) v = fmaxf(v, __shfl_xor(v, o, 64));
    return v;
}
template <int CTRL, int ROW_MASK>
__device__ __forceinline__ float dpp_keep(float v)
{
    return __int_as_float(__builtin_amdgcn_update_dpp(__float_as_int(v), __float_as_int(v), CTRL, ROW_MASK, 0xF, false));
// ... 422 lines not shown
```

### tinyllama.cpp_amd/hipabi.py

```python
import ctypes as C
import os

import numpy as np

from . import build as _build

I32, F16, F32, Q8, Q4 = 0, 1, 2, 3, 4


class GtenHipError(RuntimeError):
    pass


def _sig(lib, name, res, args):
    f = getattr(lib, name)
    f.restype = res
    f.argtypes = args
    return f


class DeviceBuffer:

    def __init__(self, api, nbytes):
        self.api = api
        self.nbytes = int(nbytes)
        p = C.c_void_p()
        api._check(api._malloc(C.byref(p), self.nbytes))
        self.ptr = p.value

    @classmethod
    def from_numpy(cls, api, arr):
        arr = np.ascontiguousarray(arr)
        buf = cls(api, arr.nbytes)
        buf.upload(arr)
        return buf

    def upload(self, arr, offset=0):
        arr = np.ascontiguousarray(arr)
        assert offset + arr.nbytes <= self.nbytes
        self.api._check(self.api._h2d(self.ptr + offset, arr.ctypes.data_as(C.c_void_p), arr.nbytes))

    def download(self, dtype=np.uint8, shape=None, offset=0, nbytes=None):
        nbytes = self.nbytes - offset if nbytes is None else nbytes
        out = np.empty(nbytes, dtype=np.uint8)
        self.api._check(self.api._d2h(out.ctypes.data_as(C.c_void_p), self.ptr + offset, nbytes))
        out = out.view(dtype)
        return out.reshape(shape) if shape is not None else out

    def zero(self, byte=0):
        self.api._check(self.api._memset(self.ptr, byte, self.nbytes))

    def free(self):
        if self.ptr:
            self.api._check(self.api._free(self.ptr))
            self.ptr = None

    def __del__(self):
        try:
            self.free()
        except Exception:
            pass


class BlockDesc(C.Structure):
    _fields_ = ([(k, C.c_int) for k in ("adtype", "wdtype", "n_embd", "n_heads", "n_kv_heads", "n_ffn")] +
                [(k, C.c_void_p) for k in ("attn_norm_w", "wq", "wk", "wv", "wo", "ffn_norm_w", "wgate", "wup", "wdown", "inp",
                                           "attn_norm_out", "q", "k", "v", "attn_out", "o", "h", "ffn_norm_out", "gate", "up", "down", "out")])


class RowCtx(C.Structure):
    _fields_ = [("k", C.c_void_p), ("v", C.c_void_p), ("len", C.c_int32)]


class GtenHip:

    SYMBOLS = [
        "gten_hip_device_count", "gten_hip_init", "gten_hip_last_error", "gten_hip_stream", "gten_hip_sync", "gten_hip_select_stream", "gten_hip_stream_wait", "gten_hip_stream_idle",
        "gten_hip_malloc", "gten_hip_free", "gten_hip_memset", "gten_hip_memcpy_h2d", "gten_hip_memcpy_d2h",
        "gten_hip_memcpy_d2d", "gten_hip_prof_enable", "gten_hip_prof_read", "gten_hip_prof_family_name",
        "gten_hip_selftest_q8scale", "gten_hip_row_bytes", "gten_hip_pack_weight", "gten_hip_token_embed",
        "gten_hip_block_rows", "gten_hip_set_block_rows", "gten_hip_matmul_2d", "gten_hip_rms_norm", "gten_hip_rotary_emb", "gten_hip_silu", "gten_hip_mul",
        "gten_hip_add", "gten_hip_qkv_attn", "gten_hip_argmax_row", "gten_hip_set_prefill_exact", "gten_hip_set_decode_exact", "gten_hip_set_decode_persistent", "gten_hip_persist_status", "gten_hip_set_row_segments", "gten_hip_row_segments_ok", "gten_hip_copy_ranges",
        "gten_hip_decoder_create", "gten_hip_decoder_destroy", "gten_hip_decoder_set_tokens",
        "gten_hip_decoder_step", "gten_hip_decoder_steps", "gten_hip_decoder_generate", "gten_hip_decoder_generate_multi", "gten_hip_decoder_step_ragged", "gten_hip_decoder_result", "gten_hip_decoder_time_family",
        "gten_hip_decoder_create_multi", "gten_hip_decoder_set_tokens_seq", "gten_hip_decoder_result_seq",
        "gten_hip_decoder_logits_seq",
        "gten_hip_decoder_lane_info", "gten_hip_set_lane_skip", "gten_hip_decoder_slot_start", "gten_hip_decoder_slot_start_until", "gten_hip_decoder_slot_park", "gten_hip_decoder_slot_bind", "gten_hip_decoder_slots_apply", "gten_hip_decoder_run", "gten_hip_decoder_run_lanes", "gten_hip_decoder_slot_ids", "gten_hip_decoder_slot_ids_all",
        "gten_hip_set_kv_head_major", "gten_hip_decoder_kv_info", "gten_hip_kv_watch_selftest", "gten_hip_set_ffn_streamed", "gten_hip_set_wx_planes",
    ]
    SAMPLE_SYMBOLS = ["gten_hip_decoder_set_sampling", "gten_hip_sample_rows"]
    BIAS_SYMBOLS = ["gten_hip_decoder_set_bias_table", "gten_hip_decoder_set_seq_bias", "gten_hip_sample_rows_biased", "gten_hip_decoder_bias_info"]
    BIAS_TABLES = 16
    LOGPROBS_SYMBOLS = ["gten_hip_decoder_set_logprobs", "gten_hip_decoder_logprobs", "gten_hip_decoder_logprobs_info", "gten_hip_row_top_logprobs"]
    LOGPROBS_TOP = 20
    NUCLEUS_SYMBOLS = ["gten_hip_decoder_set_cut", "gten_hip_decoder_cut_info", "gten_hip_sample_rows_cut"]
    CUT_INFO = np.dtype([("Z", np.uint64), ("n_cand", np.int32), ("n_nucleus", np.int32), ("n_minp", np.int32), ("n_keep", np.int32)])
    PENALTY_SYMBOLS = ["gten_hip_decoder_set_penalty", "gten_hip_decoder_penalty_info", "gten_hip_penalize_rows", "gten_hip_sample_rows_pen"]
    PENALTY_HISTORY_MAX = 65535
    FSM_SYMBOLS = ["gten_hip_fsm_check", "gten_hip_decoder_set_fsm", "gten_hip_decoder_set_seq_fsm", "gten_hip_decoder_fsm_info",
                   "gten_hip_decoder_slot_states", "gten_hip_mask_rows_fsm", "gten_hip_sample_rows_fsm"]
    REGEX_SYMBOLS = ["gten_hip_fsm_expand", "gten_hip_fsm_check_dev", "gten_hip_decoder_set_vocab_bytes", "gten_hip_decoder_set_fsm_parts"]
    FSM_EXPAND_CHUNK, FSM_EXPAND_PASS, FSM_EXPAND_STATES = 4096, 8, 64
    FSM_DEAD = 0xFFFF
    FSM_MAX_BYTES = 1 << 30
    AB_SYMBOLS = ["gten_hip_set_decode_attn_classic"]
    SCORE_SYMBOLS = ["gten_hip_row_logprobs"]
    PREFIX_SYMBOLS = ["gten_hip_block_rows_prefixed"]
    CONTINUE_SYMBOLS = ["gten_hip_block_rows_continued", "gten_hip_set_row_contexts"]
    PREFIX_DECODE_SYMBOLS = ["gten_hip_decoder_prefix_set", "gten_hip_decoder_slot_share", "gten_hip_decoder_prefix_info",
                             "gten_hip_set_prefix_decode_shared"]
    PREFIXES_SYMBOLS = ["gten_hip_decoder_prefixes_set", "gten_hip_decoder_prefixes_share",
                        "gten_hip_decoder_prefixes_info"]
    GROUPS_SYMBOLS = ["gten_hip_decoder_group_set", "gten_hip_decoder_group_share",
                      "gten_hip_decoder_groups_info"]
    BEAM_SYMBOLS = ["gten_hip_beam_round", "gten_hip_permute_sets", "gten_hip_decoder_beam_begin", "gten_hip_decoder_beam_round",
                    "gten_hip_decoder_beam_live", "gten_hip_decoder_beam_read", "gten_hip_decoder_beam_end", "gten_hip_decoder_beam_info"]
    BEAM_MAX = 8
    GROUPS_MAX = 64
    PREFIXES_MAX = 8

    def __init__(self, path=None):
        path = path or _build.HIP_LIB
        if not os.path.exists(path):
            raise GtenHipError(f"{path} is missing: run __graft_entry__.build() (hipcc --offload-arch=gfx950)")
        self.path = path
        self.lib = L = C.CDLL(path, mode=C.RTLD_GLOBAL)
        vp, sz, ci = C.c_void_p, C.c_size_t, C.c_int
        self._count = _sig(L, "gten_hip_device_count", ci, [])
        self._init = _sig(L, "gten_hip_init", ci, [ci])
        self._err = _sig(L, "gten_hip_last_error", C.c_char_p, [])
        self._stream = _sig(L, "gten_hip_stream", vp, [])
        self._sync = _sig(L, "gten_hip_sync", ci, [])
        self._selftest_q8 = _sig(L, "gten_hip_selftest_q8scale", ci, [C.POINTER(C.c_ulonglong), C.POINTER(C.c_ulonglong)])
        self._malloc = _sig(L, "gten_hip_malloc", ci, [C.POINTER(vp), sz])
        self._free = _sig(L, "gten_hip_free", ci, [vp])
        self._memset = _sig(L, "gten_hip_memset", ci, [vp, ci, sz])
        self._h2d = _sig(L, "gten_hip_memcpy_h2d", ci, [vp, vp, sz])
        self._d2h = _sig(L, "gten_hip_memcpy_d2h", ci, [vp, vp, sz])
        self._d2d = _sig(L, "gten_hip_memcpy_d2d", ci, [vp, vp, sz])
        self._row_bytes = _sig(L, "gten_hip_row_bytes", sz, [ci, ci])
        self._prof_enable = _sig(L, "gten_hip_prof_enable", ci, [ci])
        self._prof_read = _sig(L, "gten_hip_prof_read", ci, [ci, C.POINTER(ci), C.POINTER(C.c_double)])
        self._prof_name = _sig(L, "gten_hip_prof_family_name", C.c_char_p, [ci])
        self._pack = _sig(L, "gten_hip_pack_weight", ci, [vp, ci, ci, ci, vp])
        self._embed = _sig(L, "gten_hip_token_embed", ci, [vp, ci, ci, vp, vp, ci, sz, ci, ci, ci])
        self._matmul = _sig(L, "gten_hip_matmul_2d", ci, [vp, ci, sz, vp, ci, vp, ci, sz, ci, ci, ci, ci])
        self._rms = _sig(L, "gten_hip_rms_norm", ci, [vp, ci, sz, vp, vp, sz, ci, ci, ci])
        self._rope = _sig(L, "gten_hip_rotary_emb", ci, [vp, ci, sz, ci, ci, ci, ci])
        self._silu = _sig(L, "gten_hip_silu", ci, [vp, vp, ci, sz, ci, ci, ci])
        self._mul = _sig(L, "gten_hip_mul", ci, [vp, vp, vp, ci, sz, ci, ci, ci])
        self._add = _sig(L, "gten_hip_add", ci, [vp, vp, vp, ci, sz, ci, ci, ci])
        self._attn = _sig(L, "gten_hip_qkv_attn", ci, [vp, vp, vp, vp, ci, sz, sz, sz, ci, ci, ci, ci, ci])
        self._prefill_exact = _sig(L, "gten_hip_set_prefill_exact", ci, [ci])
        self._block_rows = _sig(L, "gten_hip_block_rows", ci, [C.POINTER(BlockDesc), ci, ci])
        self._block_rows_prefixed = _sig(L, "gten_hip_block_rows_prefixed", ci, [C.POINTER(BlockDesc), ci, vp, vp, ci])
        self._set_row_contexts = _sig(L, "gten_hip_set_row_contexts", ci, [vp, ci, ci])
        self._block_rows_continued = _sig(L, "gten_hip_block_rows_continued", ci, [C.POINTER(BlockDesc), ci, ci])
        self._set_block_rows = _sig(L, "gten_hip_set_block_rows", ci, [ci])
        self._prefix_decode_shared = _sig(L, "gten_hip_set_prefix_decode_shared", ci, [ci])
        self._group_set = _sig(L, "gten_hip_decoder_group_set", ci, [vp, ci, vp, ci])
        self._group_share = _sig(L, "gten_hip_decoder_group_share", ci, [vp, ci, ci, ci])
        self._groups_info = _sig(L, "gten_hip_decoder_groups_info", ci, [vp, ci, ci, C.POINTER(ci), C.POINTER(ci), C.POINTER(ci),
                                                                         C.POINTER(C.c_ulonglong), C.POINTER(ci)])
        self._decode_exact = _sig(L, "gten_hip_set_decode_exact", ci, [ci])
        self._decode_attn_classic = _sig(L, "gten_hip_set_decode_attn_classic", ci, [ci])
        self._decode_persistent = _sig(L, "gten_hip_set_decode_persistent", ci, [ci])
        self._kv_head_major = _sig(L, "gten_hip_set_kv_head_major", ci, [ci])
        self._kv_watch_selftest = _sig(L, "gten_hip_kv_watch_selftest", ci, [])
        self._ffn_streamed = _sig(L, "gten_hip_set_ffn_streamed", ci, [ci])
        self._wx_planes = _sig(L, "gten_hip_set_wx_planes", ci, [ci])
        self._lane_skip = _sig(L, "gten_hip_set_lane_skip", ci, [ci])
        self._persist_status = _sig(L, "gten_hip_persist_status", ci, [C.POINTER(ci), C.POINTER(C.c_ulonglong), C.POINTER(C.c_uint), C.c_void_p, ci])
        self._set_row_segments = _sig(L, "gten_hip_set_row_segments", ci, [C.c_void_p, ci])
        self._copy_ranges = _sig(L, "gten_hip_copy_ranges", ci, [C.c_void_p, ci])
        self._set_sampling = _sig(L, "gten_hip_decoder_set_sampling", ci, [vp, ci, ci, C.c_float, C.c_uint64, C.c_uint32])
        self._sample_rows = _sig(L, "gten_hip_sample_rows", ci, [vp, ci, ci, C.c_longlong, vp, vp, C.c_uint64, vp, vp, vp])
        self._sample_rows_biased = _sig(L, "gten_hip_sample_rows_biased", ci, [vp, ci, ci, C.c_longlong, vp, C.c_longlong, vp, vp, C.c_uint64, vp, vp, vp])
        self._set_bias_table = _sig(L, "gten_hip_decoder_set_bias_table", ci, [vp, ci, vp, vp, ci, C.c_float])
        self._set_seq_bias = _sig(L, "gten_hip_decoder_set_seq_bias", ci, [vp, ci, ci, ci])
        self._bias_info = _sig(L, "gten_hip_decoder_bias_info", ci, [vp, C.POINTER(ci), vp, vp, ci, C.POINTER(vp)])
        self._set_logprobs = _sig(L, "gten_hip_decoder_set_logprobs", ci, [vp, ci, ci])
        self._dec_logprobs = _sig(L, "gten_hip_decoder_logprobs", ci, [vp, ci, ci, ci, ci, vp, vp, vp])
        self._logprobs_info = _sig(L, "gten_hip_decoder_logprobs_info", ci, [vp, C.POINTER(ci), vp, C.POINTER(vp), C.POINTER(C.c_longlong), C.POINTER(ci)])
        self._row_top_logprobs = _sig(L, "gten_hip_row_top_logprobs", ci, [vp, ci, ci, C.c_longlong, vp, ci, vp, vp, vp])
        self._set_cut = _sig(L, "gten_hip_decoder_set_cut", ci, [vp, ci, C.c_float, C.c_float])
        self._cut_info = _sig(L, "gten_hip_decoder_cut_info", ci, [vp, vp, vp, vp, C.POINTER(ci)])
        self._sample_rows_cut = _sig(L, "gten_hip_sample_rows_cut", ci, [vp, ci, ci, C.c_longlong, vp, C.c_longlong, vp, vp, C.c_uint64, vp, vp, vp, vp, vp, vp])
        self._set_penalty = _sig(L, "gten_hip_decoder_set_penalty", ci, [vp, ci, C.c_float, C.c_float, C.c_float, ci, ci])
        self._penalty_info = _sig(L, "gten_hip_decoder_penalty_info", ci, [vp, vp, vp, vp, vp, vp, C.POINTER(ci)])
        self._penalize_rows = _sig(L, "gten_hip_penalize_rows", ci, [vp, ci, ci, C.c_longlong, vp, C.c_longlong, vp, vp, vp, vp, vp, vp, C.c_longlong])
        self._sample_rows_pen = _sig(L, "gten_hip_sample_rows_pen", ci, [vp, ci, ci, C.c_longlong, vp, C.c_longlong, vp, vp, C.c_uint64, vp, vp, vp, vp,
                                                                         vp, vp, vp, vp, vp, vp, vp])
        self._fsm_check = _sig(L, "gten_hip_fsm_check", ci, [vp, vp, C.c_longlong, C.c_longlong, C.POINTER(C.c_longlong)])
        self._set_fsm = _sig(L, "gten_hip_decoder_set_fsm", ci, [vp, vp, vp, ci])
        self._set_seq_fsm = _sig(L, "gten_hip_decoder_set_seq_fsm", ci, [vp, ci, ci, ci])
        self._fsm_info = _sig(L, "gten_hip_decoder_fsm_info", ci, [vp, C.POINTER(ci), vp, vp, C.POINTER(ci), ci, ci, ci, vp, C.POINTER(vp), C.POINTER(vp)])
        self._slot_states = _sig(L, "gten_hip_decoder_slot_states", ci, [vp, ci, ci, ci, vp])
        self._slot_start_until = _sig(L, "gten_hip_decoder_slot_start_until", ci, [vp, ci, ci, ci])
        self._slot_park = _sig(L, "gten_hip_decoder_slot_park", ci, [vp, ci])
        self._decoder_run = _sig(L, "gten_hip_decoder_run", ci, [vp, ci])
        self._slot_ids = _sig(L, "gten_hip_decoder_slot_ids", ci, [vp, ci, ci, ci, vp])
        self._fsm_expand = _sig(L, "gten_hip_fsm_expand", ci, [vp, vp, ci, ci, ci, vp, C.c_longlong, vp, vp, vp, ci, ci])
        self._fsm_check_dev = _sig(L, "gten_hip_fsm_check_dev", ci, [vp, vp, C.c_longlong, C.c_longlong, C.POINTER(C.c_longlong)])
        self._set_vocab_bytes = _sig(L, "gten_hip_decoder_set_vocab_bytes", ci, [vp, vp, vp])
        self._set_fsm_parts = _sig(L, "gten_hip_decoder_set_fsm_parts", ci, [vp, ci, vp, vp, ci])
        self._mask_rows_fsm = _sig(L, "gten_hip_mask_rows_fsm", ci, [vp, ci, ci, C.c_longlong, vp, vp, ci, vp, vp, vp, vp, vp, vp, vp, C.c_longlong])
        self._sample_rows_fsm = _sig(L, "gten_hip_sample_rows_fsm", ci, [vp, ci, ci, C.c_longlong, vp, vp, ci, vp, vp, vp, C.c_uint64, vp, vp, vp, vp,
                                                                         vp, vp, vp, vp, vp, vp, vp, vp])
        self._row_logprobs = _sig(L, "gten_hip_row_logprobs", ci, [vp, ci, ci, C.c_longlong, vp, vp, vp, vp])
        self._argmax_row = _sig(L, "gten_hip_argmax_row", ci, [vp, ci, vp])
        self._beam_round = _sig(L, "gten_hip_beam_round", ci, [vp, ci, vp, vp, vp, C.c_longlong, vp, ci, vp, vp, ci, vp])
        self._permute_sets = _sig(L, "gten_hip_permute_sets", ci, [vp, ci, sz, sz, vp, ci, vp, vp, ci])
        self._beam_begin = _sig(L, "gten_hip_decoder_beam_begin", ci, [vp, vp, ci, vp, ci])
        self._dec_beam_round = _sig(L, "gten_hip_decoder_beam_round", ci, [vp])
        self._beam_live = _sig(L, "gten_hip_decoder_beam_live", ci, [vp, C.POINTER(ci)])
        self._beam_read = _sig(L, "gten_hip_decoder_beam_read", ci, [vp, ci, vp, vp, vp])
        self._beam_end = _sig(L, "gten_hip_decoder_beam_end", ci, [vp])
        self._beam_info = _sig(L, "gten_hip_decoder_beam_info", ci, [vp, C.POINTER(ci), C.POINTER(C.c_ulonglong), C.POINTER(C.c_ulonglong)])
        self.initialised = False

    def _check(self, rc):
        if rc != 0:
            raise GtenHipError(f"gten_hip error {rc}: {self._err().decode(errors='replace')}")

    def device_count(self):
        return self._count()

    def init(self, device=0):
        if self.device_count() <= device:
            raise GtenHipError(f"no MI355X visible (device_count={self.device_count()}, asked for {device}); "
                               "there is no CPU fallback for the gten_hip path")
        self._check(self._init(device))
        self.initialised = True
        return self

    def sync(self):
        self._check(self._sync())

    def selftest_q8scale(self):
        a, b = C.c_ulonglong(0), C.c_ulonglong(0)
        self._check(self._selftest_q8(C.byref(a), C.byref(b)))
        return a.value, b.value

    def stream(self):
        return self._stream()

    def set_row_segments(self, starts):
        if not starts:
            self._check(self._set_row_segments(None, 0))
# ... 292 lines not shown
        w = max(n_top, 1)
        out = DeviceBuffer(self, 4 * n_rows * (1 + 2 * w))
        self._check(self._row_top_logprobs(logits.ptr, n_rows, n_vocab, row_stride, t.ptr, n_top, out.ptr, out.ptr + 4 * n_rows,
                                           out.ptr + 4 * n_rows * (1 + w)))
        self.sync()
        got = out.download(np.uint8)
        lp = got[: 4 * n_rows].view(np.float32).copy()
        ti = got[4 * n_rows: 4 * n_rows * (1 + w)].view(np.int32).reshape(n_rows, w)[:, :n_top].copy()
        tl = got[4 * n_rows * (1 + w):].view(np.float32).reshape(n_rows, w)[:, :n_top].copy()
        return lp, ti, tl

    def row_top_logprobs_rc(self, logits, n_rows, n_vocab, row_stride, n_top):
        buf = DeviceBuffer(self, 4 * max(n_rows, 1) * 48)
        buf.zero()
        r = 4 * max(n_rows, 1)
        return self._row_top_logprobs(logits.ptr, n_rows, n_vocab, row_stride, buf.ptr, n_top, buf.ptr + r, buf.ptr + 2 * r, buf.ptr + 24 * r)

    def row_logprobs_rc(self, logits, n_rows, n_vocab, row_stride):
        buf = DeviceBuffer(self, 16 * max(n_rows, 1))
        buf.zero()
        return self._row_logprobs(logits.ptr, n_rows, n_vocab, row_stride, buf.ptr, buf.ptr + 4 * max(n_rows, 1), None, None)

    def argmax_row(self, logits, n, offset=0):
        out = DeviceBuffer(self, 4)
        self._check(self._argmax_row(logits.ptr + offset, n, out.ptr))
        return int(out.download(np.int32)[0])

    BEAM_GROUP = np.dtype([("row0", np.int32), ("n_beams", np.int32), ("prompt_len", np.int32), ("max_new", np.int32), ("eos", np.int32)])
    BEAM_STATE = np.dtype([("cum", np.float32, 8), ("fin_final", np.float32, 8), ("fin_cum", np.float32, 8), ("fin_t", np.int32, 8),
                           ("fin_beam", np.int32, 8), ("n_fin", np.int32), ("done", np.int32), ("t", np.int32), ("stepped", np.int32)])

    def beam_round(self, groups, state, top_id, top_lp, row_stride, w, n_w, parent, ids, trellis_rows, next_id):
        self._check(self._beam_round(groups.ptr, groups.nbytes // self.BEAM_GROUP.itemsize, state.ptr, top_id.ptr, top_lp.ptr, int(row_stride), w.ptr,
                                     int(n_w), parent.ptr, ids.ptr, int(trellis_rows), next_id.ptr))

    def permute_sets_rc(self, ranges, offset, nbytes, groups, n_groups, state, parent, trellis_rows=1):
        rec = np.zeros(len(ranges), np.dtype([("base", np.uint64, 8), ("group", np.int32), ("pad", np.int32)]))
        for i, (g, bases) in enumerate(ranges):
            rec["group"][i] = g
            rec["base"][i, : len(bases)] = bases
        return self._permute_sets(rec.ctypes.data_as(C.c_void_p), len(ranges), int(offset), int(nbytes), int(groups), int(n_groups),
                                  int(state) if state else None, int(parent), int(trellis_rows))

    def permute_sets(self, ranges, offset, nbytes, groups, n_groups, state, parent, trellis_rows=1):
        self._check(self.permute_sets_rc(ranges, offset, nbytes, groups, n_groups, state, parent, trellis_rows))

    def decoder_beam_begin(self, dec, groups, w):
        g = np.array([tuple(int(v) for v in x) for x in groups], dtype=self.BEAM_GROUP)
        w = np.ascontiguousarray(w, dtype=np.float32)
        return self._beam_begin(dec, g.ctypes.data_as(C.c_void_p), len(g), w.ctypes.data_as(C.c_void_p), len(w))

    def decoder_beam_round(self, dec):
        self._check(self._dec_beam_round(dec))

    def decoder_beam_live(self, dec):
        n = C.c_int(-1)
        self._check(self._beam_live(dec, C.byref(n)))
        return n.value

    def decoder_beam_read(self, dec, g, max_new):
        st = np.zeros(1, self.BEAM_STATE)
        par, ids = np.zeros((max_new, 8), np.int32), np.zeros((max_new, 8), np.int32)
        self._check(self._beam_read(dec, int(g), st.ctypes.data_as(C.c_void_p), par.ctypes.data_as(C.c_void_p), ids.ctypes.data_as(C.c_void_p)))
        t = int(st["t"][0])
        return st[0], par[:t].copy(), ids[:t].copy()

    def decoder_beam_end(self, dec):
        return self._beam_end(dec)

    def decoder_beam_info(self, dec):
        r, b, n = C.c_int(0), C.c_ulonglong(0), C.c_ulonglong(0)
        self._check(self._beam_info(dec, C.byref(r), C.byref(b), C.byref(n)))
        return r.value, b.value, n.value

    def last_error(self):
        return self._err().decode(errors="replace")

    def set_decode_exact(self, on):
        self._check(self._decode_exact(1 if on else 0))

    def set_decode_attn_classic(self, on):
        self._check(self._decode_attn_classic(int(on)))

    def decoder_group_set(self, dec, g, kv, rows):
        if kv is None:
            return self._group_set(dec, int(g), None, 0)
        kv = np.ascontiguousarray(kv, dtype=np.uint64).reshape(-1, 2)
        return self._group_set(dec, int(g), kv.ctypes.data_as(C.c_void_p), int(rows))

    def decoder_group_share(self, dec, seq, g, rows):
        return self._group_share(dec, int(seq), int(g), int(rows))

    def decoder_groups_info(self, dec, seq, g=0):
        sg, ch, rows, imp, sh = C.c_int(-1), C.c_int(0), C.c_int(0), C.c_ulonglong(0), C.c_int(0)
        self._check(self._groups_info(dec, int(seq), int(g), C.byref(sg), C.byref(ch), C.byref(rows), C.byref(imp), C.byref(sh)))
        return sg.value, ch.value, rows.value, imp.value, sh.value

    def set_prefix_decode_shared(self, on):
        self._check(self._prefix_decode_shared(-1 if on is None else 1 if on else 0))

    def set_kv_head_major(self, on):
        self._check(self._kv_head_major(1 if on else 0))

    def set_ffn_streamed(self, on):
        self._check(self._ffn_streamed(1 if on else 0))

    def set_wx_planes(self, on):
        self._check(self._wx_planes(1 if on else 0))

    def kv_watch_selftest(self):
        return int(self._kv_watch_selftest())

    def set_decode_persistent(self, on):
        self._check(self._decode_persistent(1 if on else 0))

    def set_lane_skip(self, on):
        self._check(self._lane_skip(1 if on else 0))

    def persist_status(self, n_stamps=0):
        nd, nl, ab = C.c_int(0), C.c_ulonglong(0), C.c_uint(0)
        st = (C.c_uint * max(n_stamps, 1))()
        self._check(self._persist_status(C.byref(nd), C.byref(nl), C.byref(ab), C.cast(st, C.c_void_p) if n_stamps else None, n_stamps))
        return nd.value, nl.value, ab.value, list(st)[:n_stamps]

    def set_prefill_exact(self, on):
        self._check(self._prefill_exact(1 if on else 0))

    def select_stream(self, idx):
        self._check(self.lib.gten_hip_select_stream(int(idx)))

    def set_block_rows(self, on):
        self._check(self._set_block_rows(1 if on else 0))

    def block_rows(self, n, start_pos, ints, bufs):
        d = BlockDesc()
        for k, v in ints.items():
            setattr(d, k, int(v))
        for k, v in bufs.items():
            setattr(d, k, v.ptr)
        rc = self._block_rows(C.byref(d), n, start_pos)
        if rc == 1:
            return False
        self._check(rc)
        return True

    def block_rows_prefixed(self, n, ints, bufs, k_prefix, v_prefix, prefix_len):
        d = BlockDesc()
        for k, v in ints.items():
            setattr(d, k, int(v))
        for k, v in bufs.items():
            setattr(d, k, v.ptr)
        rc = self._block_rows_prefixed(C.byref(d), n, getattr(k_prefix, "ptr", k_prefix), getattr(v_prefix, "ptr", v_prefix), int(prefix_len))
        if rc == 1:
            return False
        self._check(rc)
        return True

    def set_row_contexts(self, contexts):
        if not contexts:
            self._check(self._set_row_contexts(None, 0, 0))
            return
        n_layers, n_seg = len(contexts), len(contexts[0])
        arr = (RowCtx * (n_layers * n_seg))()
        for l, row in enumerate(contexts):
            if len(row) != n_seg:
                raise ValueError("set_row_contexts: every layer lists the same segments")
# ... 103 lines not shown
```

### tinyllama.cpp_amd/hostabi.py

```python
import ctypes as C
import os

import numpy as np

from . import build as _build
from .hipabi import GtenHipError, load as _load_hip


class HostConfig(C.Structure):
    _fields_ = [(k, C.c_int) for k in
                ("n_vocab", "max_ctx", "n_embd", "n_ffn", "n_layers", "n_heads", "n_kv_heads", "wdtype", "adtype")]

    def weight_shapes(self):
        E, F, V = self.n_embd, self.n_ffn, self.n_vocab
        KV = (E // self.n_heads) * self.n_kv_heads
        W, F16 = self.wdtype, 1
        out = [(V, E, W)]
        for _ in range(self.n_layers):
            out += [(E, E, W), (KV, E, W), (KV, E, W), (E, E, W), (F, E, W), (F, E, W), (E, F, W), (1, E, F16), (1, E, F16)]
        return out + [(1, E, F16), (V, E, W)]


class HostPenalties(C.Structure):
    _fields_ = ([(k, C.c_void_p) for k in ("rep", "freq", "pres", "last_n", "count_prompt")] +
                [(k, C.c_float) for k in ("rep_all", "freq_all", "pres_all")] + [(k, C.c_int32) for k in ("last_n_all", "count_prompt_all")])


def _sig(lib, name, res, args):
    f = getattr(lib, name)
    f.restype = res
    f.argtypes = args
    return f


class GtenHost:
    SYMBOLS = [
        "gten_host_default_config", "gten_host_model_create", "gten_host_model_free", "gten_host_model_n_weights",
        "gten_host_model_weight_bytes", "gten_host_model_set_weight", "gten_host_model_load_gten",
        "gten_host_model_load_synthetic", "gten_host_model_logits", "gten_host_model_greedy", "gten_host_model_generate",
        "gten_host_tokenizer_create", "gten_host_tokenizer_free", "gten_host_tokenizer_encode", "gten_host_tokenizer_decode",
        "gten_host_synth_weight", "gten_host_write_gten", "gten_host_synthetic_tokens",
        "gten_host_model_set_fast_decode", "gten_host_model_decode_begin", "gten_host_model_decode_step", "gten_host_model_decode_steps", "gten_host_batch_decode_steps",
        "gten_host_model_decode_result", "gten_host_model_time_family",
        "gten_host_batch_create", "gten_host_batch_free", "gten_host_batch_load_synthetic", "gten_host_batch_set_weight",
        "gten_host_batch_prefill", "gten_host_batch_prefill_many", "gten_host_batch_generate", "gten_host_batch_serve", "gten_host_batch_serve2", "gten_host_batch_set_serve_schedule", "gten_host_batch_set_serve_spares", "gten_host_batch_set_serve_ramp", "gten_host_batch_decode_begin", "gten_host_batch_decode_step", "gten_host_batch_decode_step_ragged",
        "gten_host_batch_decode_result", "gten_host_batch_logits", "gten_host_batch_time_family", "gten_host_batch_kv_info", "gten_host_batch_seq_steps",
    ]
    SAMPLE_SYMBOLS = ["gten_host_model_generate_topk", "gten_host_batch_generate_topk", "gten_host_batch_serve_topk"]
    BIAS_SYMBOLS = ["gten_host_model_set_bias_table", "gten_host_batch_set_bias_table", "gten_host_batch_set_sampling", "gten_host_batch_set_seq_bias",
                    "gten_host_batch_bias_info", "gten_host_model_set_seq_bias", "gten_host_model_set_sampling", "gten_host_model_step_logits", "gten_host_model_generate_biased", "gten_host_batch_generate_biased",
                    "gten_host_batch_serve_biased"]
    LOGPROBS_SYMBOLS = ["gten_host_model_set_logprobs", "gten_host_batch_set_logprobs", "gten_host_model_logprobs", "gten_host_batch_logprobs",
                        "gten_host_model_generate_lp", "gten_host_batch_generate_lp", "gten_host_batch_serve_lp", "gten_host_model_score_top"]
    LOGPROBS_TOP = 20
    NUCLEUS_SYMBOLS = ["gten_host_model_set_cut", "gten_host_batch_set_cut", "gten_host_model_cut_info", "gten_host_batch_cut_info",
                       "gten_host_model_generate_nucleus", "gten_host_batch_generate_nucleus", "gten_host_batch_serve_nucleus"]
    PENALTY_SYMBOLS = ["gten_host_model_set_penalty", "gten_host_batch_set_penalty", "gten_host_model_penalty_info", "gten_host_batch_penalty_info",
                       "gten_host_model_generate_penalized", "gten_host_batch_generate_penalized", "gten_host_batch_serve_penalized"]
    FSM_SYMBOLS = ["gten_host_fsm_create", "gten_host_fsm_free", "gten_host_fsm_add_stop", "gten_host_fsm_add_choices", "gten_host_fsm_add_table",
                   "gten_host_fsm_n_states", "gten_host_fsm_tables", "gten_host_model_set_fsm", "gten_host_batch_set_fsm", "gten_host_model_fsm_info",
                   "gten_host_batch_fsm_info", "gten_host_model_set_seq_fsm", "gten_host_batch_set_seq_fsm", "gten_host_model_fsm_states",
                   "gten_host_batch_fsm_states", "gten_host_batch_fsm_decoder", "gten_host_model_generate_fsm", "gten_host_batch_generate_fsm", "gten_host_batch_serve_fsm"]
    REGEX_SYMBOLS = ["gten_host_fsm_set_vocab", "gten_host_tokenizer_vocab_bytes", "gten_host_fsm_add_regex", "gten_host_regex_byte_dfa",
                     "gten_host_fsm_n_regex"]
    SCORE_SYMBOLS = ["gten_host_model_score", "gten_host_model_logits_all", "gten_host_model_score_many"]
    PREFIX_SYMBOLS = ["gten_host_batch_set_prefix", "gten_host_batch_prefix_info"]
    PREFIX_DECODE_SYMBOLS = ["gten_host_batch_prefix_decode_info", "gten_host_batch_prefix_decode_share",
                             "gten_host_set_prefix_decode_shared"]
    PREFIXES_SYMBOLS = ["gten_host_batch_prefixes_set", "gten_host_batch_prefixes_info", "gten_host_batch_prefixes_decode_info",
                        "gten_host_batch_prefixes_decode_share", "gten_host_batch_prefixes_steps",
                        "gten_host_prefixes_match"]
    SAMPLES_SYMBOLS = ["gten_host_batch_serve_samples", "gten_host_batch_samples_info", "gten_host_batch_set_groups_cap",
                       "gten_host_batch_group_decode_set", "gten_host_batch_group_decode_share", "gten_host_batch_groups_decode_info",
                       "gten_host_samples_rank", "gten_host_samples_rank_records"]
    GROUPS_MAX = 64
    SESSIONS_SYMBOLS = ["gten_host_batch_extend_info", "gten_host_batch_extend_many", "gten_host_session_plan", "gten_host_batch_sessions_reserve",
                        "gten_host_batch_session_open", "gten_host_batch_session_close", "gten_host_batch_session_info", "gten_host_batch_session_ids",
                        "gten_host_batch_session_truncate", "gten_host_batch_sessions_info", "gten_host_batch_serve_sessions"]
    SESSIONS_MAX = 256
    BEAM_SYMBOLS = ["gten_host_batch_beam_search", "gten_host_beam_weights", "gten_host_beam_backtrack", "gten_host_beam_finalize"]
    BEAM_MAX = 8
    BEAM_ENDED = ("eos", "length")
    SAMPLES_MAX = 64

    def __init__(self, path=None):
        path = path or _build.HOST_LIB
        if not os.path.exists(path):
            raise GtenHipError(f"{path} is missing: run __graft_entry__.build()")
        self.hip = _load_hip()
        self.lib = L = C.CDLL(path)
        vp, sz, ci = C.c_void_p, C.c_size_t, C.c_int
        cfgp = C.POINTER(HostConfig)
        self._defcfg = _sig(L, "gten_host_default_config", None, [cfgp, ci, ci])
        self._create = _sig(L, "gten_host_model_create", vp, [cfgp])
        self._free = _sig(L, "gten_host_model_free", None, [vp])
        self._nw = _sig(L, "gten_host_model_n_weights", ci, [vp])
        self._wb = _sig(L, "gten_host_model_weight_bytes", sz, [vp, ci])
        self._setw = _sig(L, "gten_host_model_set_weight", ci, [vp, ci, vp, sz])
        self._loadg = _sig(L, "gten_host_model_load_gten", ci, [vp, C.c_char_p])
        self._loads = _sig(L, "gten_host_model_load_synthetic", ci, [vp, C.c_uint64])
        self._logits = _sig(L, "gten_host_model_logits", ci, [vp, vp, ci, ci, vp])
        self._greedy = _sig(L, "gten_host_model_greedy", ci, [vp, vp, ci, ci, ci])
        self._generate = _sig(L, "gten_host_model_generate", ci, [vp, vp, ci, ci, ci])
        self._generate_topk = _sig(L, "gten_host_model_generate_topk", ci, [vp, vp, ci, ci, ci, ci, C.c_float, C.c_uint64, C.c_uint32])
        self._bserve_topk = _sig(L, "gten_host_batch_serve_topk", ci, [vp, vp, vp, ci, ci, ci, ci, ci, ci, vp, vp, vp, vp, ci, vp, vp, ci,
                                                                      C.c_float, C.c_uint64])
        self._bgen_topk = _sig(L, "gten_host_batch_generate_topk", ci, [vp, vp, vp, ci, ci, ci, ci, C.c_float, C.c_uint64, vp, vp, vp])
        self._m_bias_table = _sig(L, "gten_host_model_set_bias_table", ci, [vp, ci, vp, vp, ci, C.c_float])
        self._b_bias_table = _sig(L, "gten_host_batch_set_bias_table", ci, [vp, ci, vp, vp, ci, C.c_float])
        self._b_set_sampling = _sig(L, "gten_host_batch_set_sampling", ci, [vp, ci, ci, C.c_float, C.c_uint64, C.c_uint32])
        self._b_seq_bias = _sig(L, "gten_host_batch_set_seq_bias", ci, [vp, ci, ci, ci])
        self._m_seq_bias = _sig(L, "gten_host_model_set_seq_bias", ci, [vp, ci, ci])
        self._m_set_sampling = _sig(L, "gten_host_model_set_sampling", ci, [vp, ci, C.c_float, C.c_uint64, C.c_uint32])
        self._m_step_logits = _sig(L, "gten_host_model_step_logits", ci, [vp, vp])
        self._b_bias_info = _sig(L, "gten_host_batch_bias_info", ci, [vp, vp, vp])
        self._generate_biased = _sig(L, "gten_host_model_generate_biased", ci, [vp, vp, ci, ci, ci, ci, C.c_float, C.c_uint64, C.c_uint32, ci, ci])
        self._bgen_biased = _sig(L, "gten_host_batch_generate_biased", ci, [vp, vp, vp, ci, ci, ci, vp, vp, ci, C.c_float, C.c_uint64, vp, vp, vp, vp, vp])
        self._bserve_biased = _sig(L, "gten_host_batch_serve_biased", ci, [vp, vp, vp, ci, ci, ci, ci, ci, ci, vp, vp, vp, vp, ci, vp, vp, ci,
                                                                          C.c_float, C.c_uint64, vp, vp])
        self._m_set_lp = _sig(L, "gten_host_model_set_logprobs", ci, [vp, ci])
        self._b_set_lp = _sig(L, "gten_host_batch_set_logprobs", ci, [vp, ci, ci])
        self._m_lp = _sig(L, "gten_host_model_logprobs", ci, [vp, ci, ci, ci, vp, vp, vp])
        self._b_lp = _sig(L, "gten_host_batch_logprobs", ci, [vp, ci, ci, ci, ci, vp, vp, vp])
        self._generate_lp = _sig(L, "gten_host_model_generate_lp", ci, [vp, vp, ci, ci, ci, ci, C.c_float, C.c_uint64, C.c_uint32, ci, ci, ci, vp, vp, vp])
        self._bgen_lp = _sig(L, "gten_host_batch_generate_lp", ci, [vp, vp, vp, ci, ci, ci, vp, vp, ci, C.c_float, C.c_uint64, vp, vp, vp, vp, vp,
                                                                    vp, ci, vp, vp, vp])
        self._bserve_lp = _sig(L, "gten_host_batch_serve_lp", ci, [vp, vp, vp, ci, ci, ci, ci, ci, ci, vp, vp, vp, vp, ci, vp, vp, ci,
                                                                  C.c_float, C.c_uint64, vp, vp, vp, ci, vp, vp, vp])
        self._m_set_cut = _sig(L, "gten_host_model_set_cut", ci, [vp, C.c_float, C.c_float])
        self._b_set_cut = _sig(L, "gten_host_batch_set_cut", ci, [vp, ci, C.c_float, C.c_float])
        self._m_cut_info = _sig(L, "gten_host_model_cut_info", ci, [vp, vp, vp, vp])
        self._b_cut_info = _sig(L, "gten_host_batch_cut_info", ci, [vp, vp, vp, vp])
        self._generate_nuc = _sig(L, "gten_host_model_generate_nucleus", ci, [vp, vp, ci, ci, ci, ci, C.c_float, C.c_uint64, C.c_uint32, ci, ci, ci,
                                                                              C.c_float, C.c_float, vp, vp, vp])
        self._bgen_nuc = _sig(L, "gten_host_batch_generate_nucleus", ci, [vp, vp, vp, ci, ci, ci, vp, vp, ci, C.c_float, C.c_uint64, vp, vp, vp, vp, vp,
                                                                          vp, ci, vp, vp, vp, vp, vp, C.c_float, C.c_float])
        self._bserve_nuc = _sig(L, "gten_host_batch_serve_nucleus", ci, [vp, vp, vp, ci, ci, ci, ci, ci, ci, vp, vp, vp, vp, ci, vp, vp, ci,
                                                                         C.c_float, C.c_uint64, vp, vp, vp, ci, vp, vp, vp, vp, vp, C.c_float, C.c_float])
        pen = C.POINTER(HostPenalties)
        self._m_set_pen = _sig(L, "gten_host_model_set_penalty", ci, [vp, C.c_float, C.c_float, C.c_float, ci, ci])
        self._b_set_pen = _sig(L, "gten_host_batch_set_penalty", ci, [vp, ci, C.c_float, C.c_float, C.c_float, ci, ci])
        self._m_pen_info = _sig(L, "gten_host_model_penalty_info", ci, [vp, vp, vp, vp, vp, vp])
        self._b_pen_info = _sig(L, "gten_host_batch_penalty_info", ci, [vp, vp, vp, vp, vp, vp])
        self._generate_pen = _sig(L, "gten_host_model_generate_penalized", ci, [vp, vp, ci, ci, ci, ci, C.c_float, C.c_uint64, C.c_uint32, ci, ci, ci,
                                                                                C.c_float, C.c_float, vp, vp, vp, pen])
        self._bgen_pen = _sig(L, "gten_host_batch_generate_penalized", ci, [vp, vp, vp, ci, ci, ci, vp, vp, ci, C.c_float, C.c_uint64, vp, vp, vp, vp, vp,
                                                                            vp, ci, vp, vp, vp, vp, vp, C.c_float, C.c_float, pen])
        self._bserve_pen = _sig(L, "gten_host_batch_serve_penalized", ci, [vp, vp, vp, ci, ci, ci, ci, ci, ci, vp, vp, vp, vp, ci, vp, vp, ci,
                                                                           C.c_float, C.c_uint64, vp, vp, vp, ci, vp, vp, vp, vp, vp, C.c_float, C.c_float, pen])
        self._fsm_create = _sig(L, "gten_host_fsm_create", vp, [ci])
        self._fsm_free = _sig(L, "gten_host_fsm_free", None, [vp])
        self._fsm_add_stop = _sig(L, "gten_host_fsm_add_stop", ci, [vp, vp, vp, ci])
        self._fsm_add_choices = _sig(L, "gten_host_fsm_add_choices", ci, [vp, vp, vp, ci])
        self._fsm_add_table = _sig(L, "gten_host_fsm_add_table", ci, [vp, vp, vp, ci])
        self._fsm_n_states = _sig(L, "gten_host_fsm_n_states", ci, [vp])
        self._fsm_tables = _sig(L, "gten_host_fsm_tables", ci, [vp, C.POINTER(vp), C.POINTER(vp)])
        self._fsm_set_vocab = _sig(L, "gten_host_fsm_set_vocab", ci, [vp, vp, vp])
        self._tok_vocab_bytes = _sig(L, "gten_host_tokenizer_vocab_bytes", C.c_longlong, [vp, ci, vp, ci, vp, C.c_longlong, vp])
        self._fsm_add_regex = _sig(L, "gten_host_fsm_add_regex", ci, [vp, C.c_char_p, ci, C.POINTER(ci)])
        self._regex_byte_dfa = _sig(L, "gten_host_regex_byte_dfa", ci, [C.c_char_p, vp, vp, ci, C.POINTER(ci)])
        self._fsm_n_regex = _sig(L, "gten_host_fsm_n_regex", ci, [vp])
        self._m_set_fsm = _sig(L, "gten_host_model_set_fsm", ci, [vp, vp])
        self._b_set_fsm = _sig(L, "gten_host_batch_set_fsm", ci, [vp, vp])
        self._m_fsm_info = _sig(L, "gten_host_model_fsm_info", ci, [vp, C.POINTER(ci), vp, vp])
        self._b_fsm_info = _sig(L, "gten_host_batch_fsm_info", ci, [vp, C.POINTER(ci), vp, vp])
        self._m_set_seq_fsm = _sig(L, "gten_host_model_set_seq_fsm", ci, [vp, ci, ci])
        self._b_set_seq_fsm = _sig(L, "gten_host_batch_set_seq_fsm", ci, [vp, ci, ci, ci])
        self._m_fsm_states = _sig(L, "gten_host_model_fsm_states", ci, [vp, ci, ci, vp])
        self._b_fsm_states = _sig(L, "gten_host_batch_fsm_states", ci, [vp, ci, ci, ci, vp])
        self._b_fsm_decoder = _sig(L, "gten_host_batch_fsm_decoder", vp, [vp])
        self._generate_fsm = _sig(L, "gten_host_model_generate_fsm", ci, [vp, vp, ci, ci, ci, ci, C.c_float, C.c_uint64, C.c_uint32, ci, ci, ci,
                                                                          C.c_float, C.c_float, vp, vp, vp, pen, ci, vp])
        self._bgen_fsm = _sig(L, "gten_host_batch_generate_fsm", ci, [vp, vp, vp, ci, ci, ci, vp, vp, ci, C.c_float, C.c_uint64, vp, vp, vp, vp, vp,
                                                                      vp, ci, vp, vp, vp, vp, vp, C.c_float, C.c_float, pen, vp, vp])
        self._bserve_fsm = _sig(L, "gten_host_batch_serve_fsm", ci, [vp, vp, vp, ci, ci, ci, ci, ci, ci, vp, vp, vp, vp, ci, vp, vp, ci,
                                                                     C.c_float, C.c_uint64, vp, vp, vp, ci, vp, vp, vp, vp, vp, C.c_float, C.c_float, pen,
                                                                     vp, vp])
        self._bserve_sessions = _sig(L, "gten_host_batch_serve_sessions", ci, [vp, vp, vp, ci, ci, ci, ci, ci, ci, vp, vp, vp, vp, ci, vp, vp, ci,
                                                                               C.c_float, C.c_uint64, vp, vp, vp, ci, vp, vp, vp, vp, vp, C.c_float, C.c_float, pen,
                                                                               vp, vp, vp])
        self._bsess_reserve = _sig(L, "gten_host_batch_sessions_reserve", ci, [vp, ci])
        self._bsess_open = _sig(L, "gten_host_batch_session_open", ci, [vp])
        self._bsess_close = _sig(L, "gten_host_batch_session_close", ci, [vp, ci])
        self._bsess_info = _sig(L, "gten_host_batch_session_info", ci, [vp, ci, C.POINTER(ci), C.POINTER(ci), C.POINTER(ci), C.POINTER(ci)])
        self._bsess_ids = _sig(L, "gten_host_batch_session_ids", ci, [vp, ci, vp, ci])
        self._bsess_truncate = _sig(L, "gten_host_batch_session_truncate", ci, [vp, ci, ci])
        _ull = C.c_ulonglong
        self._bsessions_info = _sig(L, "gten_host_batch_sessions_info", ci, [vp, C.POINTER(ci), C.POINTER(_ull), C.POINTER(_ull), C.POINTER(_ull),
                                                                             C.POINTER(_ull), C.POINTER(_ull)])
        self._score_top = _sig(L, "gten_host_model_score_top", ci, [vp, vp, ci, ci, vp, ci, vp, vp, vp, vp])
        self._score = _sig(L, "gten_host_model_score", ci, [vp, vp, ci, ci, vp, vp, vp])
        self._logits_all = _sig(L, "gten_host_model_logits_all", ci, [vp, vp, ci, ci, vp])
        self._score_many = _sig(L, "gten_host_model_score_many", ci, [vp, vp, vp, ci, vp, vp, vp])
        self._tok_create = _sig(L, "gten_host_tokenizer_create", vp, [C.c_char_p, ci])
        self._tok_free = _sig(L, "gten_host_tokenizer_free", None, [vp])
        self._tok_encode = _sig(L, "gten_host_tokenizer_encode", ci, [vp, C.c_char_p, ci, vp, ci])
        self._tok_decode = _sig(L, "gten_host_tokenizer_decode", C.c_char_p, [vp, ci, ci])
        self._setfast = _sig(L, "gten_host_model_set_fast_decode", ci, [vp, ci])
        self._dbegin = _sig(L, "gten_host_model_decode_begin", ci, [vp, vp, ci])
        self._dstep = _sig(L, "gten_host_model_decode_step", ci, [vp, ci, ci])
        self._dsteps = _sig(L, "gten_host_model_decode_steps", ci, [vp, ci, ci, ci])
        self._bsteps = _sig(L, "gten_host_batch_decode_steps", ci, [vp, ci, ci, ci])
        self._dresult = _sig(L, "gten_host_model_decode_result", ci, [vp, ci, C.POINTER(C.c_int32)])
        self._timefam = _sig(L, "gten_host_model_time_family", ci, [vp, ci, ci, ci, C.POINTER(C.c_double), C.POINTER(ci)])
        self._bcreate = _sig(L, "gten_host_batch_create", vp, [cfgp, ci])
        self._bfree = _sig(L, "gten_host_batch_free", None, [vp])
        self._bloads = _sig(L, "gten_host_batch_load_synthetic", ci, [vp, C.c_uint64])
        self._bsetw = _sig(L, "gten_host_batch_set_weight", ci, [vp, ci, vp, sz])
        self._bprefill = _sig(L, "gten_host_batch_prefill", ci, [vp, ci, vp, ci, vp])
        self._bprefill_many = _sig(L, "gten_host_batch_prefill_many", ci, [vp, vp, vp, vp, ci, vp])
        self._bbegin = _sig(L, "gten_host_batch_decode_begin", ci, [vp, ci, vp, ci])
        self._bstep = _sig(L, "gten_host_batch_decode_step", ci, [vp, ci, ci])
        self._bstepr = _sig(L, "gten_host_batch_decode_step_ragged", ci, [vp, vp, ci])
        self._bgen = _sig(L, "gten_host_batch_generate", ci, [vp, vp, vp, ci, ci, ci, vp, vp])
        self._bserve = _sig(L, "gten_host_batch_serve2", ci, [vp, vp, vp, ci, ci, ci, ci, ci, ci, vp, vp, vp, vp, ci])
        self._bsched = _sig(L, "gten_host_batch_set_serve_schedule", ci, [vp, ci])
        self._bspares = _sig(L, "gten_host_batch_set_serve_spares", ci, [vp, ci])
        self._bramp = _sig(L, "gten_host_batch_set_serve_ramp", ci, [vp, ci])
        self._bresult = _sig(L, "gten_host_batch_decode_result", ci, [vp, ci, ci, C.POINTER(C.c_int32)])
        self._blogits = _sig(L, "gten_host_batch_logits", ci, [vp, ci, vp])
        self._btime = _sig(L, "gten_host_batch_time_family", ci, [vp, ci, ci, ci, C.POINTER(C.c_double), C.POINTER(ci)])
        self._bseqsteps = _sig(L, "gten_host_batch_seq_steps", ci, [vp, ci, vp, ci, ci, ci])
        self._bkvinfo = _sig(L, "gten_host_batch_kv_info", ci, [vp, C.POINTER(ci), C.POINTER(C.c_ulonglong), C.POINTER(C.c_ulonglong)])
        self._bsetprefix = _sig(L, "gten_host_batch_set_prefix", ci, [vp, vp, ci])
        self._bprefixinfo = _sig(L, "gten_host_batch_prefix_info", ci, [vp, C.POINTER(ci), C.POINTER(C.c_ulonglong), C.POINTER(C.c_ulonglong)])
        self._bpdinfo = _sig(L, "gten_host_batch_prefix_decode_info", ci,
                             [vp, ci, C.POINTER(ci), C.POINTER(ci), C.POINTER(C.c_ulonglong), C.POINTER(C.c_ulonglong)])
        self._bpdshare = _sig(L, "gten_host_batch_prefix_decode_share", ci, [vp, ci, ci])
        self._pdshared = _sig(L, "gten_host_set_prefix_decode_shared", ci, [ci])
        ull = C.c_ulonglong
        self._bpsset = _sig(L, "gten_host_batch_prefixes_set", ci, [vp, ci, vp, ci])
        self._bpsinfo = _sig(L, "gten_host_batch_prefixes_info", ci, [vp, ci, C.POINTER(ci), C.POINTER(ull), C.POINTER(ull)])
        self._bpsdinfo = _sig(L, "gten_host_batch_prefixes_decode_info", ci,
                              [vp, ci, C.POINTER(ci), C.POINTER(ci), ci, C.POINTER(ci), C.POINTER(ull), C.POINTER(ci)])
        self._bpsdshare = _sig(L, "gten_host_batch_prefixes_decode_share", ci, [vp, ci, ci, ci])
        self._bpssteps = _sig(L, "gten_host_batch_prefixes_steps", ci, [vp, ci, vp, ci, ci, ci])
        self._psmatch = _sig(L, "gten_host_prefixes_match", ci, [vp, vp, ci, ci, vp, ci])
        self._bserve_samples = _sig(L, "gten_host_batch_serve_samples", ci, [vp, vp, vp, ci, ci, ci, ci, ci, ci, vp, vp, vp, vp, ci, vp, vp, ci,
                                                                             C.c_float, C.c_uint64, vp, vp, vp, ci, vp, vp, vp, vp, vp, C.c_float, C.c_float, pen,
                                                                             vp, vp, vp, ci])
        self._bsamples_info = _sig(L, "gten_host_batch_samples_info", ci, [vp, C.POINTER(ull), C.POINTER(ull), C.POINTER(ull), C.POINTER(ull), C.POINTER(ci)])
        self._bgroups_cap = _sig(L, "gten_host_batch_set_groups_cap", ci, [vp, ci])
        self._bextend_many = _sig(L, "gten_host_batch_extend_many", ci, [vp, vp, vp, vp, vp, ci, vp, vp])
        self._bextend_info = _sig(L, "gten_host_batch_extend_info", ci, [vp, C.POINTER(ull), C.POINTER(ull), C.POINTER(ull), C.POINTER(ull)])
        self._session_plan = _sig(L, "gten_host_session_plan", ci, [ci, ci, ci, ci, C.POINTER(ci), C.POINTER(ci), C.POINTER(ci)])
        self._bbeam = _sig(L, "gten_host_batch_beam_search", ci, [vp, vp, vp, ci, ci, ci, ci, C.c_float, vp, vp, vp, vp, vp, vp, C.POINTER(ci)])
        self._beam_weights = _sig(L, "gten_host_beam_weights", ci, [ci, C.c_float, vp])
        self._beam_backtrack = _sig(L, "gten_host_beam_backtrack", ci, [vp, vp, ci, ci, ci, vp])
        self._beam_finalize = _sig(L, "gten_host_beam_finalize", ci, [vp, vp, vp, ci, ci, vp, ci, vp, vp, vp, vp, vp])
        self._bgdset = _sig(L, "gten_host_batch_group_decode_set", ci, [vp, ci, ci, ci])
        self._bgdshare = _sig(L, "gten_host_batch_group_decode_share", ci, [vp, ci, ci, ci])
        self._bgdinfo = _sig(L, "gten_host_batch_groups_decode_info", ci, [vp, ci, ci, C.POINTER(ci), C.POINTER(ci), C.POINTER(ci), C.POINTER(ull), C.POINTER(ci)])
        self._samples_rank = _sig(L, "gten_host_samples_rank", ci, [vp, vp, ci, vp])
# ... 9 lines not shown

    def synth_weight(self, cfg, seed, idx):
        rows, cols, dt = cfg.weight_shapes()[idx]
        out = np.zeros(rows * self.hip.row_bytes(dt, cols), np.uint8)
        rc = self._synthw(C.byref(cfg), seed, idx, out.ctypes.data_as(C.c_void_p), out.size)
        if rc:
            raise GtenHipError(f"gten_host_synth_weight rc={rc}")
        return out

    def write_gten(self, cfg, seed, path):
        rc = self._writeg(C.byref(cfg), seed, path.encode())
        if rc:
            raise GtenHipError(f"gten_host_write_gten rc={rc}")

    def set_prefix_decode_shared(self, on):
        rc = self._pdshared(-1 if on is None else 1 if on else 0)
        if rc:
            raise GtenHipError(f"gten_host_set_prefix_decode_shared rc={rc}")

    def samples_rank(self, logprob_sum, n_new):
        sums, nn = np.ascontiguousarray(logprob_sum, dtype=np.float64), np.ascontiguousarray(n_new, dtype=np.int32)
        assert len(sums) == len(nn)
        order = np.zeros(max(len(nn), 1), np.int32)
        rc = self._samples_rank(_ptr(sums), _ptr(nn), len(nn), _ptr(order))
        if rc:
            raise ValueError(f"samples_rank rc={rc}")
        return order[: len(nn)].copy()

    def samples_rank_records(self, records, n_prompt, n_new):
        rec, nn = np.ascontiguousarray(records, dtype=np.float32), np.ascontiguousarray(n_new, dtype=np.int32)
        assert rec.ndim == 2 and rec.shape[0] == len(nn)
        order = np.zeros(max(len(nn), 1), np.int32)
        rc = self._samples_rank_records(_ptr(rec), rec.shape[1], int(n_prompt), _ptr(nn), len(nn), _ptr(order))
        if rc:
            raise ValueError(f"samples_rank_records rc={rc}")
        return order[: len(nn)].copy()

    def prefixes_match(self, prefixes, prompt):
        prefixes = [[] if p is None else list(p) for p in prefixes]
        lens = np.ascontiguousarray([len(p) for p in prefixes], dtype=np.int32)
        max_len = int(lens.max()) if len(prefixes) else 0
        flat = np.zeros((max(len(prefixes), 1), max(max_len, 1)), np.int32)
        for i, p in enumerate(prefixes):
            flat[i, :len(p)] = p
        prompt = np.ascontiguousarray(prompt, dtype=np.int32)
        return self._psmatch(flat.ctypes.data_as(C.c_void_p), lens.ctypes.data_as(C.c_void_p), len(prefixes), max(max_len, 1),
                             prompt.ctypes.data_as(C.c_void_p), len(prompt))

    def beam_weights(self, max_new, length_penalty):
        w = np.zeros(max_new + 1, np.float32)
        if self._beam_weights(int(max_new), float(length_penalty), _ptr(w)):
            raise GtenHipError("beam_weights: bad arguments")
        return w

    def beam_backtrack(self, parent, ids, t, b):
        parent, ids = np.ascontiguousarray(parent, dtype=np.int32).reshape(-1, 8), np.ascontiguousarray(ids, dtype=np.int32).reshape(-1, 8)
        out = np.zeros(max(int(t), 1), np.int32)
        n = self._beam_backtrack(_ptr(parent), _ptr(ids), len(parent), int(t), int(b), _ptr(out))
        return None if n < 0 else out[:n].copy()

    def beam_finalize(self, state, parent, ids, n_beams, w, max_new):
        parent, ids = np.ascontiguousarray(parent, dtype=np.int32).reshape(-1, 8), np.ascontiguousarray(ids, dtype=np.int32).reshape(-1, 8)
        st = np.frombuffer(np.asarray(state).tobytes(), np.uint8).copy()
        assert st.size == 176
        w = np.ascontiguousarray(w, dtype=np.float32)
        oi, on = np.zeros((n_beams, max_new), np.int32), np.zeros(n_beams, np.int32)
        of, oc, oe = np.zeros(n_beams, np.float32), np.zeros(n_beams, np.float32), np.zeros(n_beams, np.int32)
        n = self._beam_finalize(_ptr(st), _ptr(parent), _ptr(ids), len(parent), int(n_beams), _ptr(w), int(max_new), _ptr(oi), _ptr(on), _ptr(of), _ptr(oc), _ptr(oe))
        if n < 0:
            raise GtenHipError("beam_finalize: bad arguments")
        return [(oi[i, : on[i]].copy(), of[i], oc[i], self.BEAM_ENDED[oe[i]]) for i in range(n)]

    def session_plan(self, n_ids, rows, n_new, segmented=True):
        ctx, k, path = C.c_int(0), C.c_int(0), C.c_int(0)
        if self._session_plan(int(n_ids), int(rows), int(n_new), 1 if segmented else 0, C.byref(ctx), C.byref(k), C.byref(path)) != 0:
            return None
        return ctx.value, k.value, path.value

    def synthetic_tokens(self, count, seed=12345, n_vocab=32003):
        out = np.zeros(count, np.int32)
        self._stoks(out.ctypes.data_as(C.c_void_p), count, seed, n_vocab)
        return out

    def model(self, cfg):
        return HostModel(self, cfg)

    def batch(self, cfg, n_seq):
        return HostBatch(self, cfg, n_seq)

    def tokenizer(self, path, vocab_size=32000):
        return HostTokenizer(self, path, vocab_size)


def bias_pairs(pairs=(), fill=0.0, allow=None):
    if allow is not None:
        merged = {int(i): 0.0 for i in allow}
        if len(merged) != len(list(allow)):
            raise ValueError("allow lists an id twice")
        for i, v in pairs:
            if int(i) in merged:
                merged[int(i)] = float(v)
            else:
                raise ValueError(f"pair id {i} is not among the allowed ids")
        pairs, fill = list(merged.items()), -np.inf
    ids = np.ascontiguousarray([int(i) for i, _ in pairs], dtype=np.int32)
    values = np.ascontiguousarray([float(v) for _, v in pairs], dtype=np.float32)
    return ids, values, float(fill)


SERVE_STATS = ("prompt_tokens", "new_tokens", "steps", "admissions", "prefill_s", "decode_s", "lane_steps", "lane_rows", "moved")


def _ptr(a):
    return None if a is None else a.ctypes.data_as(C.c_void_p)


def _pack(prompts):
    mp = max(len(p) for p in prompts)
    pr, npr = np.zeros((len(prompts), mp), np.int32), np.zeros(len(prompts), np.int32)
    for j, p in enumerate(prompts):
        pr[j, : len(p)] = p
        npr[j] = len(p)
    return pr, npr, mp


def _each(v, n, dt, full=False):
    if v is None:
        return None, None
    if np.isscalar(v):
        return (np.full(n, v, dt), None) if full else (None, v)
    a = np.ascontiguousarray(v, dtype=dt)
    assert len(a) == n
    return a, None


def _request_args(n, top_k, temp, seed):
    (ks, k1), (ts, t1) = _each(top_k, n, np.int32), _each(temp, n, np.float32)
    return [_ptr(ks), _ptr(ts), 0 if ks is not None else int(k1), 1.0 if ts is not None else float(t1), C.c_uint64(int(seed))]


def _full_args(n, *pairs):
    return [_ptr(_each(v, n, dt, full=True)[0]) for v, dt in pairs]


def _n_tops(n_top, n):
    if n_top is None:
        return None, 0
    a = np.full(n, n_top, np.int32) if np.isscalar(n_top) else np.ascontiguousarray([-1 if v is None else v for v in n_top], dtype=np.int32)
    assert len(a) == n
    return a, max(int(a.max()), 0)


def _records(n_top, n, width):
    nt, tw = _n_tops(n_top, n)
    lp, ti, tl = np.zeros((n, width), np.float32), np.full((n, width, tw), -1, np.int32), np.zeros((n, width, tw), np.float32)
    return [_ptr(nt), tw, _ptr(lp), _ptr(ti), _ptr(tl)], (lp, ti, tl)


def _samples_counts(n, n_prompts):
    ns = np.ascontiguousarray(np.broadcast_to(np.asarray(n, np.int32), (n_prompts,)))
    assert ns.min() >= 1 and ns.max() <= GtenHost.SAMPLES_MAX, "samples per prompt in [1, 64]"
    return ns


def _cut_args(n, top_p, min_p):
    (ps, p1), (ms, m1) = _each(top_p, n, np.float32), _each(min_p, n, np.float32)
# ... 318 lines not shown
    def generate(self, prompt, max_tokens, eos=-1):
        buf = np.zeros(max_tokens, np.int32)
        buf[: len(prompt)] = prompt
        total = self.host._generate(self.h, buf.ctypes.data_as(C.c_void_p), len(prompt), max_tokens, eos)
        return buf[:total].copy()

    def generate_topk(self, prompt, max_tokens, eos, top_k, temp, seed, stream=0):
        buf = np.zeros(max(max_tokens, len(prompt)), np.int32)
        buf[: len(prompt)] = prompt
        total = self.host._generate_topk(self.h, buf.ctypes.data_as(C.c_void_p), len(prompt), max_tokens, eos, int(top_k), float(temp),
                                         C.c_uint64(int(seed)), C.c_uint32(int(stream)))
        if total < 0:
            raise GtenHipError(f"generate_topk rc={total}")
        return buf[:total].copy()

    def set_bias_table_rc(self, table, pairs=(), fill=0.0, allow=None):
        ids, values, fill = bias_pairs(pairs, fill, allow)
        return self.host._m_bias_table(self.h, int(table), ids.ctypes.data_as(C.c_void_p), values.ctypes.data_as(C.c_void_p), len(ids), C.c_float(fill))

    def set_bias_table(self, table, pairs=(), fill=0.0, allow=None):
        rc = self.set_bias_table_rc(table, pairs, fill, allow)
        if rc:
            raise GtenHipError(f"set_bias_table rc={rc}: {self.host.hip._err().decode(errors='replace')}")

    def set_seq_bias_rc(self, table, until=0):
        return self.host._m_seq_bias(self.h, int(table), int(until))

    def set_sampling(self, top_k, temp=1.0, seed=0, stream=0):
        rc = self.host._m_set_sampling(self.h, int(top_k), float(temp), C.c_uint64(int(seed)), C.c_uint32(int(stream)))
        if rc:
            raise GtenHipError(f"set_sampling rc={rc}")

    def step_logits(self):
        out = np.zeros(self.cfg.n_vocab, np.float32)
        rc = self.host._m_step_logits(self.h, out.ctypes.data_as(C.c_void_p))
        if rc:
            raise GtenHipError(f"step_logits rc={rc}")
        return out

    def generate_biased(self, prompt, max_tokens, eos=-1, top_k=0, temp=1.0, seed=0, stream=0, table=-1, min_new=0):
        buf = np.zeros(max(max_tokens, len(prompt)), np.int32)
        buf[: len(prompt)] = prompt
        total = self.host._generate_biased(self.h, buf.ctypes.data_as(C.c_void_p), len(prompt), max_tokens, eos, int(top_k), float(temp),
                                           C.c_uint64(int(seed)), C.c_uint32(int(stream)), int(table), int(min_new))
        if total < 0:
            raise GtenHipError(f"generate_biased rc={total}")
        return buf[:total].copy()

    def set_logprobs_rc(self, n_top):
        return self.host._m_set_lp(self.h, int(n_top))

    def set_logprobs(self, n_top):
        rc = self.set_logprobs_rc(n_top)
        if rc:
            raise GtenHipError(f"set_logprobs rc={rc}: {self.host.hip._err().decode(errors='replace')}")

    def logprobs(self, n_from, count, n_top):
        lp, ti, tl = np.zeros(count, np.float32), np.full((count, n_top), -1, np.int32), np.zeros((count, n_top), np.float32)
        rc = self.host._m_lp(self.h, int(n_from), int(count), int(n_top), lp.ctypes.data_as(C.c_void_p), ti.ctypes.data_as(C.c_void_p),
                             tl.ctypes.data_as(C.c_void_p))
        if rc:
            raise GtenHipError(f"logprobs rc={rc}: {self.host.hip._err().decode(errors='replace')}")
        return lp, ti, tl

    def generate_logprobs(self, prompt, max_tokens, n_top, eos=-1, top_k=0, temp=1.0, seed=0, stream=0, table=-1, min_new=0):
        width = max(max_tokens, len(prompt))
        buf = np.zeros(width, np.int32)
        buf[: len(prompt)] = prompt
        lp, ti, tl = np.zeros(width, np.float32), np.full((width, n_top), -1, np.int32), np.zeros((width, n_top), np.float32)
        total = self.host._generate_lp(self.h, buf.ctypes.data_as(C.c_void_p), len(prompt), max_tokens, eos, int(top_k), float(temp),
                                       C.c_uint64(int(seed)), C.c_uint32(int(stream)), int(table), int(min_new), int(n_top),
                                       lp.ctypes.data_as(C.c_void_p), ti.ctypes.data_as(C.c_void_p), tl.ctypes.data_as(C.c_void_p))
        if total < 0:
            raise GtenHipError(f"generate_logprobs rc={total}: {self.host.hip._err().decode(errors='replace')}")
        return buf[:total].copy(), lp[:total].copy(), ti[:total].copy(), tl[:total].copy()

    def set_cut_rc(self, top_p, min_p):
        return self.host._m_set_cut(self.h, C.c_float(top_p), C.c_float(min_p))

    def set_cut(self, top_p=1.0, min_p=0.0):
        rc = self.set_cut_rc(top_p, min_p)
        if rc:
            raise GtenHipError(f"set_cut rc={rc}: {self.host.hip._err().decode(errors='replace')}")

    def cut_info(self):
        a, b, t = np.zeros(1, np.float32), np.zeros(1, np.float32), np.zeros(1, np.float32)
        on = self.host._m_cut_info(self.h, _ptr(a), _ptr(b), _ptr(t))
        if on < 0:
            raise GtenHipError(f"cut_info rc={on}")
        return a[0], b[0], t[0], bool(on)

    def generate_nucleus(self, prompt, max_tokens, eos=-1, top_k=0, temp=1.0, seed=0, stream=0, top_p=1.0, min_p=0.0, table=-1, min_new=0,
                         n_top=None):
        width = max(max_tokens, len(prompt))
        buf = np.zeros(width, np.int32)
        buf[: len(prompt)] = prompt
        ask = n_top is not None and n_top >= 0
        w = int(n_top) if ask else 0
        lp, ti, tl = np.zeros(width, np.float32), np.full((width, w), -1, np.int32), np.zeros((width, w), np.float32)
        total = self.host._generate_nuc(self.h, _ptr(buf), len(prompt), max_tokens, eos, int(top_k), float(temp), C.c_uint64(int(seed)),
                                        C.c_uint32(int(stream)), int(table), int(min_new), w if ask else -1, C.c_float(top_p), C.c_float(min_p),
                                        _ptr(lp) if ask else None, _ptr(ti) if ask else None, _ptr(tl) if ask else None)
        if total < 0:
            raise GtenHipError(f"generate_nucleus rc={total}: {self.host.hip._err().decode(errors='replace')}")
        ids = buf[:total].copy()
        return (ids, lp[:total].copy(), ti[:total].copy(), tl[:total].copy()) if ask else ids

    def set_penalty_rc(self, rep, freq=0.0, pres=0.0, start=0, last_n=0):
        return self.host._m_set_pen(self.h, C.c_float(rep), C.c_float(freq), C.c_float(pres), int(start), int(last_n))

    def set_penalty(self, rep=1.0, freq=0.0, pres=0.0, start=0, last_n=0):
        rc = self.set_penalty_rc(rep, freq, pres, start, last_n)
        if rc:
            raise GtenHipError(f"set_penalty rc={rc}: {self.host.hip._err().decode(errors='replace')}")

    def penalty_info(self):
        r, f, p, s, l = np.zeros(1, np.float32), np.zeros(1, np.float32), np.zeros(1, np.float32), np.zeros(1, np.int32), np.zeros(1, np.int32)
        on = self.host._m_pen_info(self.h, _ptr(r), _ptr(f), _ptr(p), _ptr(s), _ptr(l))
        if on < 0:
            raise GtenHipError(f"penalty_info rc={on}")
        return r[0], f[0], p[0], int(s[0]), int(l[0]), bool(on)

    def generate_penalized(self, prompt, max_tokens, eos=-1, top_k=0, temp=1.0, seed=0, stream=0, rep=1.0, freq=0.0, pres=0.0, last_n=0,
                           count_prompt=True, top_p=1.0, min_p=0.0, table=-1, min_new=0, n_top=None):
        width = max(max_tokens, len(prompt))
        buf = np.zeros(width, np.int32)
        buf[: len(prompt)] = prompt
        ask = n_top is not None and n_top >= 0
        w = int(n_top) if ask else 0
        lp, ti, tl = np.zeros(width, np.float32), np.full((width, w), -1, np.int32), np.zeros((width, w), np.float32)
        pen = _penalty_arg(1, float(rep), float(freq), float(pres), int(last_n), bool(count_prompt))
        total = self.host._generate_pen(self.h, _ptr(buf), len(prompt), max_tokens, eos, int(top_k), float(temp), C.c_uint64(int(seed)),
                                        C.c_uint32(int(stream)), int(table), int(min_new), w if ask else -1, C.c_float(top_p), C.c_float(min_p),
                                        _ptr(lp) if ask else None, _ptr(ti) if ask else None, _ptr(tl) if ask else None, C.byref(pen))
        if total < 0:
            raise GtenHipError(f"generate_penalized rc={total}: {self.host.hip._err().decode(errors='replace')}")
        ids = buf[:total].copy()
        return (ids, lp[:total].copy(), ti[:total].copy(), tl[:total].copy()) if ask else ids

    def set_fsm_rc(self, fsm):
        return self.host._m_set_fsm(self.h, fsm.h if fsm is not None else None)

    def set_fsm(self, fsm):
        rc = self.set_fsm_rc(fsm)
        if rc:
            raise GtenHipError(f"set_fsm rc={rc}: {self.host.hip._err().decode(errors='replace')}")

    def fsm_info(self):
        return _fsm_info(self.host._m_fsm_info, self.h, 1)

    def set_seq_fsm_rc(self, state, pos=0):
        return self.host._m_set_seq_fsm(self.h, int(state), int(pos))

    def set_seq_fsm(self, state, pos=0):
        rc = self.set_seq_fsm_rc(state, pos)
        if rc:
            raise GtenHipError(f"set_seq_fsm rc={rc}: {self.host.hip._err().decode(errors='replace')}")

    def fsm_states(self, n_from, count):
        out = np.zeros(max(count, 1), np.int32)
        rc = self.host._m_fsm_states(self.h, int(n_from), int(count), _ptr(out))
        if rc:
            raise GtenHipError(f"fsm_states rc={rc}: {self.host.hip._err().decode(errors='replace')}")
        return out[:count].copy()

    def generate_fsm(self, prompt, max_tokens, fsm_start, eos=-1, top_k=0, temp=1.0, seed=0, stream=0, rep=1.0, freq=0.0, pres=0.0, last_n=0,
# ... 145 lines not shown
    def set_serve_ramp(self, percent):
        self._ck(self.host._bramp(self.h, int(percent)), "set_serve_ramp")

    def serve(self, prompts, max_tokens, eos=-1, slice_steps=16, max_new=0, max_new_each=None):
        return self._serve(self.host._bserve, "batch_serve", prompts, max_tokens, eos, slice_steps, max_new, max_new_each)

    def serve_topk(self, prompts, max_tokens, eos, top_k, temp, seed, slice_steps=16, max_new=0, max_new_each=None):
        return self._serve(self.host._bserve_topk, "batch_serve_topk", prompts, max_tokens, eos, slice_steps, max_new, max_new_each,
                           *_request_args(len(prompts), top_k, temp, seed))

    def set_bias_table_rc(self, table, pairs=(), fill=0.0, allow=None):
        ids, values, fill = bias_pairs(pairs, fill, allow)
        return self.host._b_bias_table(self.h, int(table), ids.ctypes.data_as(C.c_void_p), values.ctypes.data_as(C.c_void_p), len(ids), C.c_float(fill))

    def set_bias_table(self, table, pairs=(), fill=0.0, allow=None):
        rc = self.set_bias_table_rc(table, pairs, fill, allow)
        if rc:
            raise GtenHipError(f"batch_set_bias_table rc={rc}: {self.host.hip._err().decode(errors='replace')}")

    def set_sampling(self, seq, top_k, temp=1.0, seed=0, stream=0):
        self._ck(self.host._b_set_sampling(self.h, int(seq), int(top_k), float(temp), C.c_uint64(int(seed)), C.c_uint32(int(stream))), "batch_set_sampling")

    def set_seq_bias_rc(self, seq, table, until=0):
        return self.host._b_seq_bias(self.h, int(seq), int(table), int(until))

    def set_seq_bias(self, seq, table, until=0):
        self._ck(self.set_seq_bias_rc(seq, table, until), "batch_set_seq_bias")

    def bias_info(self):
        t, u = np.zeros(self.n_seq, np.int32), np.zeros(self.n_seq, np.int32)
        n = self.host._b_bias_info(self.h, t.ctypes.data_as(C.c_void_p), u.ctypes.data_as(C.c_void_p))
        if n < 0:
            raise GtenHipError(f"batch_bias_info rc={n}")
        return n, t, u

    def generate_biased(self, prompts, max_tokens, eos=-1, top_k=0, temp=1.0, seed=0, streams=None, tables=None, min_new=None):
        n = self.n_seq
        return self._generate(self.host._bgen_biased, "batch_generate_biased", prompts, max_tokens, eos,
                              _request_args(n, top_k, temp, seed) + _full_args(n, (streams, np.uint32), (tables, np.int32), (min_new, np.int32)))

    def serve_biased(self, prompts, max_tokens, eos, top_k, temp, seed, tables=None, min_new=None, slice_steps=16, max_new=0, max_new_each=None):
        n = len(prompts)
        return self._serve(self.host._bserve_biased, "batch_serve_biased", prompts, max_tokens, eos, slice_steps, max_new, max_new_each,
                           *_request_args(n, top_k, temp, seed), *_full_args(n, (tables, np.int32), (min_new, np.int32)))

    def set_logprobs_rc(self, seq, n_top):
        return self.host._b_set_lp(self.h, int(seq), int(n_top))

    def set_logprobs(self, seq, n_top):
        rc = self.set_logprobs_rc(seq, n_top)
        if rc:
            raise GtenHipError(f"batch_set_logprobs rc={rc}: {self.host.hip._err().decode(errors='replace')}")

    def logprobs(self, seq, n_from, count, n_top):
        lp, ti, tl = np.zeros(count, np.float32), np.full((count, n_top), -1, np.int32), np.zeros((count, n_top), np.float32)
        rc = self.host._b_lp(self.h, int(seq), int(n_from), int(count), int(n_top), lp.ctypes.data_as(C.c_void_p), ti.ctypes.data_as(C.c_void_p),
                             tl.ctypes.data_as(C.c_void_p))
        if rc:
            raise GtenHipError(f"batch_logprobs rc={rc}: {self.host.hip._err().decode(errors='replace')}")
        return lp, ti, tl

    def generate_logprobs(self, prompts, max_tokens, n_top, eos=-1, top_k=0, temp=1.0, seed=0, streams=None, tables=None, min_new=None):
        n = self.n_seq
        args, rec = _records(n_top, n, max_tokens)
        ids = self._generate(self.host._bgen_lp, "batch_generate_lp", prompts, max_tokens, eos,
                             _request_args(n, top_k, temp, seed) + _full_args(n, (streams, np.uint32), (tables, np.int32), (min_new, np.int32)), args)
        return (ids, *rec)

    def serve_logprobs(self, prompts, max_tokens, eos, top_k, temp, seed, n_top, tables=None, min_new=None, slice_steps=16, max_new=0,
                       max_new_each=None):
        n = len(prompts)
        args, rec = _records(n_top, n, max(max_tokens, max(len(p) for p in prompts)))
        ids, st = self._serve(self.host._bserve_lp, "batch_serve_lp", prompts, max_tokens, eos, slice_steps, max_new, max_new_each,
                              *_request_args(n, top_k, temp, seed), *_full_args(n, (tables, np.int32), (min_new, np.int32)), *args)
        return (ids, st, *rec)

    def set_cut_rc(self, seq, top_p, min_p):
        return self.host._b_set_cut(self.h, int(seq), C.c_float(top_p), C.c_float(min_p))

    def set_cut(self, seq, top_p=1.0, min_p=0.0):
        rc = self.set_cut_rc(seq, top_p, min_p)
        if rc:
            raise GtenHipError(f"batch_set_cut rc={rc}: {self.host.hip._err().decode(errors='replace')}")

    def cut_info(self):
        a, b, t = np.zeros(self.n_seq, np.float32), np.zeros(self.n_seq, np.float32), np.zeros(self.n_seq, np.float32)
        on = self.host._b_cut_info(self.h, _ptr(a), _ptr(b), _ptr(t))
        if on < 0:
            raise GtenHipError(f"batch_cut_info rc={on}")
        return a, b, t, bool(on)

    def generate_nucleus(self, prompts, max_tokens, eos=-1, top_k=0, temp=1.0, seed=0, streams=None, top_p=1.0, min_p=0.0, tables=None,
                         min_new=None, n_top=None):
        n = self.n_seq
        args, rec = _records(n_top, n, max_tokens)
        if n_top is None:
            args = [None, 0, None, None, None]
        ids = self._generate(self.host._bgen_nuc, "batch_generate_nucleus", prompts, max_tokens, eos,
                             _request_args(n, top_k, temp, seed) + _full_args(n, (streams, np.uint32), (tables, np.int32), (min_new, np.int32)),
                             args + _cut_args(n, top_p, min_p))
        return ids if n_top is None else (ids, *rec)

    def serve_nucleus(self, prompts, max_tokens, eos, top_k, temp, seed, top_p=1.0, min_p=0.0, tables=None, min_new=None, n_top=None,
                      slice_steps=16, max_new=0, max_new_each=None):
        n = len(prompts)
        args, rec = _records(n_top, n, max(max_tokens, max(len(p) for p in prompts)))
        if n_top is None:
            args = [None, 0, None, None, None]
        ids, st = self._serve(self.host._bserve_nuc, "batch_serve_nucleus", prompts, max_tokens, eos, slice_steps, max_new, max_new_each,
                              *_request_args(n, top_k, temp, seed), *_full_args(n, (tables, np.int32), (min_new, np.int32)), *args,
                              *_cut_args(n, top_p, min_p))
        return (ids, st) if n_top is None else (ids, st, *rec)

    def set_penalty_rc(self, seq, rep, freq=0.0, pres=0.0, start=0, last_n=0):
        return self.host._b_set_pen(self.h, int(seq), C.c_float(rep), C.c_float(freq), C.c_float(pres), int(start), int(last_n))

    def set_penalty(self, seq, rep=1.0, freq=0.0, pres=0.0, start=0, last_n=0):
        rc = self.set_penalty_rc(seq, rep, freq, pres, start, last_n)
        if rc:
            raise GtenHipError(f"batch_set_penalty rc={rc}: {self.host.hip._err().decode(errors='replace')}")

    def penalty_info(self):
        n = self.n_seq
        r, f, p, s, l = np.zeros(n, np.float32), np.zeros(n, np.float32), np.zeros(n, np.float32), np.zeros(n, np.int32), np.zeros(n, np.int32)
        on = self.host._b_pen_info(self.h, _ptr(r), _ptr(f), _ptr(p), _ptr(s), _ptr(l))
        if on < 0:
            raise GtenHipError(f"batch_penalty_info rc={on}")
        return r, f, p, s, l, bool(on)

    def generate_penalized(self, prompts, max_tokens, eos=-1, top_k=0, temp=1.0, seed=0, streams=None, rep=1.0, freq=0.0, pres=0.0, last_n=0,
                           count_prompt=True, top_p=1.0, min_p=0.0, tables=None, min_new=None, n_top=None):
        n = self.n_seq
        args, rec = _records(n_top, n, max_tokens)
        if n_top is None:
            args = [None, 0, None, None, None]
        pen = _penalty_arg(n, rep, freq, pres, last_n, count_prompt)
        ids = self._generate(self.host._bgen_pen, "batch_generate_penalized", prompts, max_tokens, eos,
                             _request_args(n, top_k, temp, seed) + _full_args(n, (streams, np.uint32), (tables, np.int32), (min_new, np.int32)),
                             args + _cut_args(n, top_p, min_p) + [C.byref(pen)])
        return ids if n_top is None else (ids, *rec)

    def serve_penalized(self, prompts, max_tokens, eos, top_k, temp, seed, rep=1.0, freq=0.0, pres=0.0, last_n=0, count_prompt=True, top_p=1.0,
                        min_p=0.0, tables=None, min_new=None, n_top=None, slice_steps=16, max_new=0, max_new_each=None):
        n = len(prompts)
        args, rec = _records(n_top, n, max(max_tokens, max(len(p) for p in prompts)))
        if n_top is None:
            args = [None, 0, None, None, None]
        pen = _penalty_arg(n, rep, freq, pres, last_n, count_prompt)
        ids, st = self._serve(self.host._bserve_pen, "batch_serve_penalized", prompts, max_tokens, eos, slice_steps, max_new, max_new_each,
                              *_request_args(n, top_k, temp, seed), *_full_args(n, (tables, np.int32), (min_new, np.int32)), *args,
                              *_cut_args(n, top_p, min_p), C.byref(pen))
        return (ids, st) if n_top is None else (ids, st, *rec)

    def set_fsm_rc(self, fsm):
        return self.host._b_set_fsm(self.h, fsm.h if fsm is not None else None)

    def set_fsm(self, fsm):
        rc = self.set_fsm_rc(fsm)
        if rc:
            raise GtenHipError(f"batch_set_fsm rc={rc}: {self.host.hip._err().decode(errors='replace')}")

    def fsm_info(self):
        return _fsm_info(self.host._b_fsm_info, self.h, self.n_seq)

    def set_seq_fsm_rc(self, seq, state, pos=0):
        return self.host._b_set_seq_fsm(self.h, int(seq), int(state), int(pos))
# ... 288 lines not shown
```

Baseline: 2135 tok/s.

## Keep a budgeted subset of decode weights cache-resident via temporal loads

Adds a planner that ranks the per-step weight launches (QKV, O, gate/up, down per layer, plus the LM head) by size. It marks the smallest ones as resident until a byte budget is used up; the budget defaults to 160 MiB minus the KV cache and scratch. Marked launches use a kernel variant whose weight loads are ordinary cacheable loads instead of nontemporal ones, so those weights can stay in the large last-level cache across decode steps and need less HBM traffic. The trade-off is that cached weights compete with KV-cache and activation traffic for that cache. The plan applies only for single-sequence, non-exact, non-persistent decoders, and it adds query and override APIs plus an environment knob.

```diff
diff --git a/__graft_entry__.py b/__graft_entry__.py
--- a/__graft_entry__.py
+++ b/__graft_entry__.py
@@ -29,10 +29,10 @@
         orc.build_dropin()
     build_neighbour()
     api = pkg.hipabi.GtenHip()
-    for name in api.SYMBOLS + api.SAMPLE_SYMBOLS + api.SCORE_SYMBOLS + api.PREFIX_SYMBOLS + api.PREFIX_DECODE_SYMBOLS + api.BIAS_SYMBOLS + api.LOGPROBS_SYMBOLS + api.NUCLEUS_SYMBOLS + api.PENALTY_SYMBOLS + api.FSM_SYMBOLS + api.REGEX_SYMBOLS + api.PREFIXES_SYMBOLS + api.GROUPS_SYMBOLS + api.CONTINUE_SYMBOLS + api.BEAM_SYMBOLS:
+    for name in api.SYMBOLS + api.SAMPLE_SYMBOLS + api.SCORE_SYMBOLS + api.PREFIX_SYMBOLS + api.PREFIX_DECODE_SYMBOLS + api.BIAS_SYMBOLS + api.LOGPROBS_SYMBOLS + api.NUCLEUS_SYMBOLS + api.PENALTY_SYMBOLS + api.FSM_SYMBOLS + api.REGEX_SYMBOLS + api.PREFIXES_SYMBOLS + api.GROUPS_SYMBOLS + api.CONTINUE_SYMBOLS + api.BEAM_SYMBOLS + api.AB_SYMBOLS:
         getattr(api.lib, name)
     host = pkg.hostabi.GtenHost()
-    for name in host.SYMBOLS + host.SAMPLE_SYMBOLS + host.SCORE_SYMBOLS + host.PREFIX_SYMBOLS + host.PREFIX_DECODE_SYMBOLS + host.BIAS_SYMBOLS + host.LOGPROBS_SYMBOLS + host.NUCLEUS_SYMBOLS + host.PENALTY_SYMBOLS + host.FSM_SYMBOLS + host.REGEX_SYMBOLS + host.PREFIXES_SYMBOLS + host.SAMPLES_SYMBOLS + host.SESSIONS_SYMBOLS + host.BEAM_SYMBOLS:
+    for name in host.SYMBOLS + host.SAMPLE_SYMBOLS + host.SCORE_SYMBOLS + host.PREFIX_SYMBOLS + host.PREFIX_DECODE_SYMBOLS + host.BIAS_SYMBOLS + host.LOGPROBS_SYMBOLS + host.NUCLEUS_SYMBOLS + host.PENALTY_SYMBOLS + host.FSM_SYMBOLS + host.REGEX_SYMBOLS + host.PREFIXES_SYMBOLS + host.SAMPLES_SYMBOLS + host.SESSIONS_SYMBOLS + host.BEAM_SYMBOLS + host.RESIDENT_SYMBOLS:
         getattr(host.lib, name)
 
 
diff --git a/include/gten_hip_ab.h b/include/gten_hip_ab.h
--- a/include/gten_hip_ab.h
+++ b/include/gten_hip_ab.h
@@ -1,4 +1,6 @@
 #pragma once
+
+#include "gten_hip.h"
 
 #ifdef __cplusplus
 extern "C" {
@@ -6,6 +8,12 @@
 
 int gten_hip_set_decode_attn_classic(int v);
 
+int gten_hip_set_weight_resident_mb(int mb);
+int gten_hip_set_weight_resident_bytes(long long bytes);
+long long gten_hip_weight_resident_bytes(void);
+int gten_hip_decoder_resident(gten_hip_decoder* dec, int* launches, long long* bytes);
+int gten_hip_decoder_resident_budget(gten_hip_decoder* dec, long long* budget, long long* overhead);
+
 #ifdef __cplusplus
 }
 #endif
diff --git a/include/gten_host_resident.h b/include/gten_host_resident.h
--- /dev/null
+++ b/include/gten_host_resident.h
@@ -0,0 +1,19 @@
+#ifndef GTEN_HOST_RESIDENT_H
+#define GTEN_HOST_RESIDENT_H
+
+#include "gten_host.h"
+
+#ifdef __cplusplus
+extern "C" {
+#endif
+
+int gten_host_model_resident(gten_host_model* m, int* launches, long long* bytes, long long* budget, long long* overhead);
+int gten_host_batch_resident(gten_host_batch* b, int* launches, long long* bytes, long long* budget, long long* overhead);
+
+int gten_host_resident_plan(int n_layers, int n_embd, int n_ffn, int kv_width, int n_vocab, int block_bytes, long long budget,
+                            unsigned char* resident_out, long long* launch_bytes_out, long long* bytes_out);
+
+#ifdef __cplusplus
+}
+#endif
+#endif
diff --git a/tinyllama.cpp_amd/build.py b/tinyllama.cpp_amd/build.py
--- a/tinyllama.cpp_amd/build.py
+++ b/tinyllama.cpp_amd/build.py
@@ -45,7 +45,7 @@
 def build_hip(force=False):
     from concurrent.futures import ThreadPoolExecutor
     srcs = _sources(CSRC, (".hip",))
-    hdrs = _sources(CSRC, (".h",)) + _sources(INCLUDE, (".h",)) + [os.path.abspath(__file__)]
+    hdrs = _sources(CSRC, (".h",)) + _sources(INCLUDE, (".h",)) + [os.path.join(HOST, "resident_plan.h"), os.path.abspath(__file__)]
     os.makedirs(HIP_OBJ, exist_ok=True)
     compile_flags = [f for f in HIP_FLAGS if f != "-shared"]
     stamp = " ".join(_EXTRA)
diff --git a/tinyllama.cpp_amd/csrc/gten_decode.hip b/tinyllama.cpp_amd/csrc/gten_decode.hip
--- a/tinyllama.cpp_amd/csrc/gten_decode.hip
+++ b/tinyllama.cpp_amd/csrc/gten_decode.hip
@@ -11,8 +11,10 @@
 #include "gten_hip_prefix_decode.h"
 #include "gten_hip_prefixes.h"
 #include "gten_hip_groups.h"
+#include "../host/resident_plan.h"
 
 #include <cmath>
+#include <cstdlib>
 #include <vector>
 #include <algorithm>
 
@@ -163,6 +165,9 @@
     int attn_classic = 0;
     bool persist_on = false;
     struct PersistState* persist = nullptr;
+    gten::ResidentPlan resident;
+    long long resident_overhead = 0;
+    long long resident_budget = 0;
     uint8_t* hm = nullptr;
     size_t hm_seq_stride = 0, hm_cache_bytes = 0, hm_chunk_bytes = 0;
     std::vector<char> hm_dirty;
@@ -300,6 +305,48 @@
 {
     GTR_REQUIRE(v >= 0 && v <= 2, "gten_hip_set_decode_attn_classic: %d is not 0, 1 or 2", v);
     g_attn_classic = v;
+    return 0;
+}
+
+#ifndef GTEN_RESIDENT_MB_DEFAULT
+#define GTEN_RESIDENT_MB_DEFAULT 160
+#endif
+static long long g_resident_bytes = -1;
+static long long resident_setting_bytes()
+{
+    if (g_resident_bytes >= 0) return g_resident_bytes;
+    if (const char* e = getenv("GTEN_HIP_RESIDENT_MB"); e && e[0]) {
+        char* end = nullptr;
+        const long v = strtol(e, &end, 10);
+        if (end != e && *end == 0 && v >= 0 && v <= (1 << 20)) return (long long)v << 20;
+    }
+    return (long long)GTEN_RESIDENT_MB_DEFAULT << 20;
+}
+extern "C" int gten_hip_set_weight_resident_mb(int mb)
+{
+    GTR_REQUIRE(mb >= 0 && mb <= (1 << 20), "gten_hip_set_weight_resident_mb: %d MiB is not in [0, 2^20]", mb);
+    g_resident_bytes = (long long)mb << 20;
+    return 0;
+}
+extern "C" int gten_hip_set_weight_resident_bytes(long long bytes)
+{
+    GTR_REQUIRE(bytes >= 0 && bytes <= (1ll << 40), "gten_hip_set_weight_resident_bytes: %lld is not in [0, 2^40]", bytes);
+    g_resident_bytes = bytes;
+    return 0;
+}
+extern "C" long long gten_hip_weight_resident_bytes(void) { return resident_setting_bytes(); }
+extern "C" int gten_hip_decoder_resident(gten_hip_decoder* dc, int* launches, long long* bytes)
+{
+    GTR_REQUIRE(dc, "decoder_resident: null decoder");
+    if (launches) *launches = dc->resident.launches;
+    if (bytes) *bytes = dc->resident.bytes;
+    return 0;
+}
+extern "C" int gten_hip_decoder_resident_budget(gten_hip_decoder* dc, long long* budget, long long* overhead)
+{
+    GTR_REQUIRE(dc, "decoder_resident_budget: null decoder");
+    if (budget) *budget = dc->resident_budget;
+    if (overhead) *overhead = dc->resident_overhead;
     return 0;
 }
 
@@ -540,23 +587,26 @@
 }
 
 template <int WT, int PRO, int NCH, int R, int NT, int NM = 0>
-static int launch_gemv8(int tag, const Gemv8Args& a, int total_rows)
+static int launch_gemv8(int tag, const Gemv8Args& a, int total_rows, bool keep)
 {
     const int rows_per_wg = (NT / 64) * R;
     const dim3 grid((total_rows + rows_per_wg - 1) / rows_per_wg), block(NT);
     for (int k = 0; k + 1 < a.n_mats; k++) GTR_REQUIRE(a.rows[k] % R == 0, "decoder: concatenated matrices must hold a multiple of %d rows", R);
     const GemvHotWords hw = hot_of_gemv8<WT, PRO>(a);
-    DEC_LAUNCH_HOT(tag, (k_dec_gemv8<WT, PRO, NCH, R, EPI_RAW, NT, NM>), grid, block, stage_bytes((PRO == PRO_ACTQ8 && WT != GTEN_F16) ? 32 : a.d_in), hw, a);
+    const size_t lds = stage_bytes((PRO == PRO_ACTQ8 && WT != GTEN_F16) ? 32 : a.d_in);
+    if (keep) DEC_LAUNCH_HOT(tag, (k_dec_gemv8<WT, PRO, NCH, R, EPI_RAW, NT, NM, WLD_KEEP>), grid, block, lds, hw, a);
+    else DEC_LAUNCH_HOT(tag, (k_dec_gemv8<WT, PRO, NCH, R, EPI_RAW, NT, NM>), grid, block, lds, hw, a);
     return 0;
 }
 
 template <int WT>
-static int launch_gateup8(const Gemv8Args& a, int n_ffn)
+static int launch_gateup8(const Gemv8Args& a, int n_ffn, bool keep)
 {
     const dim3 grid(n_ffn / 32), block(512);
     GTR_REQUIRE(n_ffn % 32 == 0, "decoder: n_ffn %d is not a multiple of 32", n_ffn);
     const GemvHotWords hw = hot_of_gemv8<WT, PRO_RESID>(a);
-    DEC_LAUNCH_HOT(KT_DEC_GEMV_GATEUP, (k_dec_gemv8<WT, PRO_RESID, (WT == GTEN_F16 ? 4 : 1), 8, EPI_SILUMUL, 512>), grid, block, stage_bytes(a.d_in), hw, a);
+    if (keep) DEC_LAUNCH_HOT(KT_DEC_GEMV_GATEUP, (k_dec_gemv8<WT, PRO_RESID, (WT == GTEN_F16 ? 4 : 1), 8, EPI_SILUMUL, 512, 0, WLD_KEEP>), grid, block, stage_bytes(a.d_in), hw, a);
+    else DEC_LAUNCH_HOT(KT_DEC_GEMV_GATEUP, (k_dec_gemv8<WT, PRO_RESID, (WT == GTEN_F16 ? 4 : 1), 8, EPI_SILUMUL, 512>), grid, block, stage_bytes(a.d_in), hw, a);
     return 0;
 }
 
@@ -583,18 +633,20 @@
     float* xbuf = (float*)dc->xbuf;
     float* hbuf = (float*)dc->hbuf;
     int rc;
+    const auto keep = [&](size_t i) { return i < dc->resident.resident.size() && dc->resident.resident[i] != 0; };
     for (int l = 0; l < d.n_layers; l++) {
         const gten_hip_layer_ptrs& L = dc->layers[l];
+        const size_t l4 = (size_t)l * 4;
         Gemv8Args a{};
         a.step = dc->step; a.d_in = E; a.n_mats = 3;
         set_mat(a, 0, L.wq, WT, E, E); set_mat(a, 1, L.wk, WT, KV, E); set_mat(a, 2, L.wv, WT, KV, E);
         a.out = dc->qkv_raw; a.norm_w = (const uint16_t*)L.attn_norm; a.x_out = xbuf;
         if (l == 0) {
             a.table = d.embed; a.rope = dc->rope; a.rope_now = dc->rope_now; a.rope_half = dh / 2; a.n_vocab = d.n_vocab; a.tokens = dc->tokens;
-            rc = launch_gemv8<WT, PRO_EMBED, NE, 2, 512>(KT_DEC_GEMV_QKV, a, E + 2 * KV);
+            rc = launch_gemv8<WT, PRO_EMBED, NE, 2, 512>(KT_DEC_GEMV_QKV, a, E + 2 * KV, keep(l4));
         } else {
             a.res_a = hbuf; a.res_raw = dc->down_raw;
-            rc = launch_gemv8<WT, PRO_RESID, NE, 2, 512>(KT_DEC_GEMV_QKV, a, E + 2 * KV);
+            rc = launch_gemv8<WT, PRO_RESID, NE, 2, 512>(KT_DEC_GEMV_QKV, a, E + 2 * KV, keep(l4));
         }
         if (rc) return rc;
         AttnArgs t{};
@@ -609,28 +661,28 @@
         o.step = dc->step; o.d_in = E; o.n_mats = 1; set_mat(o, 0, L.wo, WT, E, E); o.out = dc->proj_raw;
         o.att_part = dc->att_part; o.d_head = dh; o.d_head_shift = __builtin_ctz(dh); o.n_chunks = dc->n_chunks;
         o.att_stats = dc->stats;
-        rc = attention_one_pass(dh) ? launch_gemv8<WT, PRO_ATTW, NE, 1, 512, 1>(KT_DEC_GEMV_O, o, E)
-                                    : launch_gemv8<WT, PRO_ATT, NE, 1, 512, 1>(KT_DEC_GEMV_O, o, E);
+        rc = attention_one_pass(dh) ? launch_gemv8<WT, PRO_ATTW, NE, 1, 512, 1>(KT_DEC_GEMV_O, o, E, keep(l4 + 1))
+                                    : launch_gemv8<WT, PRO_ATT, NE, 1, 512, 1>(KT_DEC_GEMV_O, o, E, keep(l4 + 1));
         if (rc) return rc;
         Gemv8Args gu{};
         gu.step = dc->step; gu.d_in = E; gu.n_mats = 2; set_mat(gu, 0, L.wgate, WT, F, E); set_mat(gu, 1, L.wup, WT, F, E);
         gu.res_a = xbuf; gu.res_raw = dc->proj_raw; gu.x_out = hbuf; gu.norm_w = (const uint16_t*)L.ffn_norm;
         gu.act_q = dc->act_q; gu.act_d = dc->act_d; gu.act_sum = dc->act_sum; gu.act_f = dc->act_f;
-        if ((rc = launch_gateup8<WT>(gu, F))) return rc;
+        if ((rc = launch_gateup8<WT>(gu, F, keep(l4 + 2)))) return rc;
         Gemv8Args dn{};
         dn.step = dc->step; dn.d_in = F; dn.n_mats = 1; set_mat(dn, 0, L.wdown, WT, E, F); dn.out = dc->down_raw;
         dn.act_q = dc->act_q; dn.act_d = dc->act_d; dn.act_sum = dc->act_sum;
         dn.act_f = dc->act_f;
-        rc = widerF ? launch_gemv8<WT, PRO_ACTQ8, NF12, 2, 256, 1>(KT_DEC_GEMV_DOWN, dn, E)
-             : wideF ? launch_gemv8<WT, PRO_ACTQ8, NF, 2, 256, 1>(KT_DEC_GEMV_DOWN, dn, E)
-                     : launch_gemv8<WT, PRO_ACTQ8, NE, 2, 256, 1>(KT_DEC_GEMV_DOWN, dn, E);
+        rc = widerF ? launch_gemv8<WT, PRO_ACTQ8, NF12, 2, 256, 1>(KT_DEC_GEMV_DOWN, dn, E, keep(l4 + 3))
+             : wideF ? launch_gemv8<WT, PRO_ACTQ8, NF, 2, 256, 1>(KT_DEC_GEMV_DOWN, dn, E, keep(l4 + 3))
+                     : launch_gemv8<WT, PRO_ACTQ8, NE, 2, 256, 1>(KT_DEC_GEMV_DOWN, dn, E, keep(l4 + 3));
         if (rc) return rc;
     }
     Gemv8Args hd{};
     hd.step = dc->step; hd.d_in = E; hd.n_mats = 1; set_mat(hd, 0, d.lm_head, WT, d.n_vocab, E); hd.out = d.logits;
     hd.res_a = hbuf; hd.res_raw = dc->down_raw; hd.x_out = nullptr; hd.norm_w = (const uint16_t*)d.final_norm;
     hd.best_val = dc->best_val; hd.best_idx = dc->best_idx;
-    if ((rc = launch_gemv8<WT, PRO_RESID, NE, F16W ? 4 : 8, 512, 1>(KT_DEC_GEMV_HEAD, hd, d.n_vocab))) return rc;
+    if ((rc = launch_gemv8<WT, PRO_RESID, NE, F16W ? 4 : 8, 512, 1>(KT_DEC_GEMV_HEAD, hd, d.n_vocab, keep((size_t)d.n_layers * 4)))) return rc;
     return launch_step_end(dc, StepEnd{1, d.logits, 0, dc->smp.samp, dc->step, dc->result, 0, dc->tokens, dc->smp.lp, dc->smp.cut, dc->smp.pen, dc->smp.fsm, dc->smp.fsm_state,
                                        dc->best_val, dc->best_idx, dc->n_best, 0});
 }
@@ -1439,6 +1491,17 @@
     GTR_CHECK(hipMemset(dc->rope_now, 0, S * (size_t)(dh / 2) * sizeof(float2)));
     if (dc->persist_on && n_seq == 1 && !dc->exact)
         if (int rc = persist_prepare(dc)) return rc;
+    {
+        const int block_bytes = d.wdtype == GTEN_F16 ? gten::kResidentBlockF16 : d.wdtype == GTEN_Q8 ? gten::kResidentBlockQ8 : gten::kResidentBlockQ4;
+        const long long kv_bytes = 2ll * d.n_layers * d.max_ctx * (long long)gten_hip_row_bytes(d.adtype, KV);
+        const long long scratch = 4ll * ((E + 2 * KV) + 2 * E + (long long)d.n_heads * d.max_ctx + 2ll * d.n_heads * dc->n_chunks + 16 +
+                                         (long long)d.n_heads * dc->n_chunks * dh + 2 * E + 2 * (F / 32) + F + 2 * dc->n_best + d.n_vocab) + F;
+        dc->resident_overhead = kv_bytes + scratch;
+        if (n_seq == 1 && !dc->exact && !dc->persist_on) {
+            dc->resident_budget = gten::resident_budget(resident_setting_bytes(), kv_bytes, scratch);
+            dc->resident = gten::resident_plan(gten::resident_step_launches(d.n_layers, E, F, KV, d.n_vocab, block_bytes), dc->resident_budget);
+        }
+    }
     return 0;
 }
 
diff --git a/tinyllama.cpp_amd/csrc/gten_decode_wx.h b/tinyllama.cpp_amd/csrc/gten_decode_wx.h
--- a/tinyllama.cpp_amd/csrc/gten_decode_wx.h
+++ b/tinyllama.cpp_amd/csrc/gten_decode_wx.h
@@ -189,7 +189,7 @@
     __host__ __device__ GemvHotWords() : w{0, 0, 0, 0, 0, 0, 0} {}
 };
 
-template <int WT, int PRO, int NCH, int R, int EPI, int NT, int NM = 0>
+template <int WT, int PRO, int NCH, int R, int EPI, int NT, int NM = 0, int WLD = WLD_NT>
 __global__ __launch_bounds__(NT) void k_dec_gemv8(const unsigned long long h0, const unsigned long long h1, const unsigned long long h2,
                                                   const unsigned long long h3, const unsigned long long h4, const unsigned long long h5,
                                                   const unsigned long long h6, const Gemv8Args a)
@@ -318,19 +318,19 @@
             const int b = (c * 64 + lane < nb) ? c * 64 + lane : 0;
             if (F16W) {
                 const int e = (c * 512 + lane * 8 < d) ? c * 512 + lane * 8 : 0;
-                wq[j][c] = ld_w16((const uint16_t*)qbase + (size_t)lr * d + e);
+                wq[j][c] = ld_w16<WLD>((const uint16_t*)qbase + (size_t)lr * d + e);
                 wq1[j][c] = make_uint4(0, 0, 0, 0);
                 wd[j][c] = 0;
                 continue;
             }
             if (WT == GTEN_Q4) {
-                wq[j][c] = ld_w16((const uint4*)(qbase + (size_t)lr * nb * 16) + b);
+                wq[j][c] = ld_w16<WLD>((const uint4*)(qbase + (size_t)lr * nb * 16) + b);
             } else {
                 const uint4* q0 = (const uint4*)(qbase + (size_t)lr * nb * 32);
-                wq[j][c] = ld_w16(q0 + b);
-                wq1[j][c] = ld_w16(q0 + nb + b);
-            }
-            wd[j][c] = ld_w2(drow + b);
+                wq[j][c] = ld_w16<WLD>(q0 + b);
+                wq1[j][c] = ld_w16<WLD>(q0 + nb + b);
+            }
+            wd[j][c] = ld_w2<WLD>(drow + b);
         }
     }
     __builtin_amdgcn_sched_barrier(0);
diff --git a/tinyllama.cpp_amd/csrc/gten_dev.h b/tinyllama.cpp_amd/csrc/gten_dev.h
--- a/tinyllama.cpp_amd/csrc/gten_dev.h
+++ b/tinyllama.cpp_amd/csrc/gten_dev.h
@@ -34,23 +34,21 @@
 #ifndef GTEN_NT_WEIGHTS
 #define GTEN_NT_WEIGHTS 1
 #endif
+enum { WLD_NT = 0, WLD_KEEP = 1 };
 typedef unsigned gt_u4v __attribute__((ext_vector_type(4)));
+template <int WLD = WLD_NT>
 __device__ __forceinline__ uint4 ld_w16(const void* p)
 {
-#if GTEN_NT_WEIGHTS
-    const gt_u4v v = __builtin_nontemporal_load((const gt_u4v*)p);
-#else
-    const gt_u4v v = *(const gt_u4v*)p;
-#endif
+    gt_u4v v;
+    if constexpr (GTEN_NT_WEIGHTS && WLD == WLD_NT) v = __builtin_nontemporal_load((const gt_u4v*)p);
+    else v = *(const gt_u4v*)p;
     return make_uint4(v.x, v.y, v.z, v.w);
 }
+template <int WLD = WLD_NT>
 __device__ __forceinline__ uint16_t ld_w2(const uint16_t* p)
 {
-#if GTEN_NT_WEIGHTS
-    return __builtin_nontemporal_load(p);
-#else
-    return *p;
-#endif
+    if constexpr (GTEN_NT_WEIGHTS && WLD == WLD_NT) return __builtin_nontemporal_load(p);
+    else return *p;
 }
 
 template <int CTRL, int ROW_MASK = 0xF>
diff --git a/tinyllama.cpp_amd/hipabi.py b/tinyllama.cpp_amd/hipabi.py
--- a/tinyllama.cpp_amd/hipabi.py
+++ b/tinyllama.cpp_amd/hipabi.py
@@ -103,7 +103,8 @@
     FSM_EXPAND_CHUNK, FSM_EXPAND_PASS, FSM_EXPAND_STATES = 4096, 8, 64
     FSM_DEAD = 0xFFFF
     FSM_MAX_BYTES = 1 << 30
-    AB_SYMBOLS = ["gten_hip_set_decode_attn_classic"]
+    AB_SYMBOLS = ["gten_hip_set_decode_attn_classic", "gten_hip_set_weight_resident_mb", "gten_hip_set_weight_resident_bytes", "gten_hip_weight_resident_bytes",
+                  "gten_hip_decoder_resident", "gten_hip_decoder_resident_budget"]
     SCORE_SYMBOLS = ["gten_hip_row_logprobs"]
     PREFIX_SYMBOLS = ["gten_hip_block_rows_prefixed"]
     CONTINUE_SYMBOLS = ["gten_hip_block_rows_continued", "gten_hip_set_row_contexts"]
@@ -165,6 +166,11 @@
         self._decode_exact = _sig(L, "gten_hip_set_decode_exact", ci, [ci])
         self._decode_attn_classic = _sig(L, "gten_hip_set_decode_attn_classic", ci, [ci])
         self._decode_persistent = _sig(L, "gten_hip_set_decode_persistent", ci, [ci])
+        self._weight_resident_mb = _sig(L, "gten_hip_set_weight_resident_mb", ci, [ci])
+        self._weight_resident_bytes = _sig(L, "gten_hip_set_weight_resident_bytes", ci, [C.c_longlong])
+        self._weight_resident_get = _sig(L, "gten_hip_weight_resident_bytes", C.c_longlong, [])
+        self._decoder_resident = _sig(L, "gten_hip_decoder_resident", ci, [vp, C.POINTER(ci), C.POINTER(C.c_longlong)])
+        self._decoder_resident_budget = _sig(L, "gten_hip_decoder_resident_budget", ci, [vp, C.POINTER(C.c_longlong), C.POINTER(C.c_longlong)])
         self._kv_head_major = _sig(L, "gten_hip_set_kv_head_major", ci, [ci])
         self._kv_watch_selftest = _sig(L, "gten_hip_kv_watch_selftest", ci, [])
         self._ffn_streamed = _sig(L, "gten_hip_set_ffn_streamed", ci, [ci])
@@ -623,6 +629,21 @@
     def set_decode_attn_classic(self, on):
         self._check(self._decode_attn_classic(int(on)))
 
+    def set_weight_resident_mb(self, mb):
+        self._check(self._weight_resident_mb(int(mb)))
+
+    def set_weight_resident_bytes(self, n):
+        self._check(self._weight_resident_bytes(int(n)))
+
+    def weight_resident_bytes(self):
+        return int(self._weight_resident_get())
+
+    def decoder_resident(self, dec):
+        n, b, budget, over = C.c_int(0), C.c_longlong(0), C.c_longlong(0), C.c_longlong(0)
+        self._check(self._decoder_resident(dec, C.byref(n), C.byref(b)))
+        self._check(self._decoder_resident_budget(dec, C.byref(budget), C.byref(over)))
+        return n.value, b.value, budget.value, over.value
+
     def decoder_group_set(self, dec, g, kv, rows):
         if kv is None:
             return self._group_set(dec, int(g), None, 0)
diff --git a/tinyllama.cpp_amd/host/capi_resident.cpp b/tinyllama.cpp_amd/host/capi_resident.cpp
--- /dev/null
+++ b/tinyllama.cpp_amd/host/capi_resident.cpp
@@ -0,0 +1,49 @@
+#include "../../include/gten_host_resident.h"
+
+#include "../../include/gten_hip_ab.h"
+#include "capi_handles.h"
+#include "resident_plan.h"
+
+using namespace gten;
+
+namespace {
+
+int info(gten_hip_decoder* dec, int* launches, long long* bytes, long long* budget, long long* overhead)
+{
+    if (!dec) return -1;
+    if (gten_hip_decoder_resident(dec, launches, bytes)) return -1;
+    if (gten_hip_decoder_resident_budget(dec, budget, overhead)) return -1;
+    return 0;
+}
+
+}
+
+extern "C" {
+
+int gten_host_model_resident(gten_host_model* m, int* launches, long long* bytes, long long* budget, long long* overhead)
+{
+    if (!m) return -1;
+    return info(m->model->decoder_handle(), launches, bytes, budget, overhead);
+}
+
+int gten_host_batch_resident(gten_host_batch* b, int* launches, long long* bytes, long long* budget, long long* overhead)
+{
+    if (!b) return -1;
+    return info(b->batch->decoder_handle(), launches, bytes, budget, overhead);
+}
+
+int gten_host_resident_plan(int n_layers, int n_embd, int n_ffn, int kv_width, int n_vocab, int block_bytes, long long budget,
+                            unsigned char* resident_out, long long* launch_bytes_out, long long* bytes_out)
+{
+    if (n_layers < 0 || n_embd <= 0 || n_ffn <= 0 || kv_width <= 0 || n_vocab <= 0 || block_bytes <= 0 || n_embd % 32 || n_ffn % 32) return -1;
+    const std::vector<ResidentLaunch> step = resident_step_launches(n_layers, n_embd, n_ffn, kv_width, n_vocab, block_bytes);
+    const ResidentPlan p = resident_plan(step, budget);
+    for (size_t i = 0; i < step.size(); i++) {
+        if (resident_out) resident_out[i] = (unsigned char)p.resident[i];
+        if (launch_bytes_out) launch_bytes_out[i] = step[i].bytes;
+    }
+    if (bytes_out) *bytes_out = p.bytes;
+    return p.launches;
+}
+
+}
diff --git a/tinyllama.cpp_amd/host/resident_plan.h b/tinyllama.cpp_amd/host/resident_plan.h
--- /dev/null
+++ b/tinyllama.cpp_amd/host/resident_plan.h
@@ -0,0 +1,63 @@
+#pragma once
+
+#include <algorithm>
+#include <cstddef>
+#include <vector>
+
+namespace gten {
+
+enum { kResidentQkv = 0, kResidentO = 1, kResidentGateUp = 2, kResidentDown = 3, kResidentHead = 4 };
+
+constexpr int kResidentBlockF16 = 64, kResidentBlockQ8 = 34, kResidentBlockQ4 = 18;
+
+struct ResidentLaunch {
+    int family = 0;
+    int layer = 0;
+    long long bytes = 0;
+};
+
+struct ResidentPlan {
+    std::vector<char> resident;
+    int launches = 0;
+    long long bytes = 0;
+};
+
+inline long long resident_weight_bytes(long long rows, long long cols, int block_bytes) { return rows * (cols / 32) * block_bytes; }
+
+inline std::vector<ResidentLaunch> resident_step_launches(int n_layers, int n_embd, int n_ffn, int kv_width, int n_vocab, int block_bytes)
+{
+    std::vector<ResidentLaunch> v;
+    const long long E = n_embd, F = n_ffn, KV = kv_width;
+    for (int l = 0; l < n_layers; l++) {
+        v.push_back(ResidentLaunch{kResidentQkv, l, resident_weight_bytes(E + 2 * KV, E, block_bytes)});
+        v.push_back(ResidentLaunch{kResidentO, l, resident_weight_bytes(E, E, block_bytes)});
+        v.push_back(ResidentLaunch{kResidentGateUp, l, resident_weight_bytes(2 * F, E, block_bytes)});
+        v.push_back(ResidentLaunch{kResidentDown, l, resident_weight_bytes(E, F, block_bytes)});
+    }
+    v.push_back(ResidentLaunch{kResidentHead, n_layers, resident_weight_bytes(n_vocab, E, block_bytes)});
+    return v;
+}
+
+inline ResidentPlan resident_plan(const std::vector<ResidentLaunch>& step, long long budget)
+{
+    ResidentPlan p;
+    p.resident.assign(step.size(), 0);
+    std::vector<size_t> order(step.size());
+    for (size_t i = 0; i < order.size(); i++) order[i] = i;
+    std::stable_sort(order.begin(), order.end(), [&](size_t a, size_t b) { return step[a].bytes < step[b].bytes; });
+    for (size_t i : order) {
+        const long long b = step[i].bytes;
+        if (b < 0 || budget - p.bytes < b) break;
+        p.resident[i] = 1;
+        p.launches++;
+        p.bytes += b;
+    }
+    return p;
+}
+
+inline long long resident_budget(long long all, long long kv_bytes, long long scratch_bytes)
+{
+    return std::max(0ll, all - std::max(0ll, kv_bytes) - std::max(0ll, scratch_bytes));
+}
+
+}
diff --git a/tinyllama.cpp_amd/hostabi.py b/tinyllama.cpp_amd/hostabi.py
--- a/tinyllama.cpp_amd/hostabi.py
+++ b/tinyllama.cpp_amd/hostabi.py
@@ -80,6 +80,8 @@
     SESSIONS_MAX = 256
     BEAM_SYMBOLS = ["gten_host_batch_beam_search", "gten_host_beam_weights", "gten_host_beam_backtrack", "gten_host_beam_finalize"]
     BEAM_MAX = 8
+    RESIDENT_SYMBOLS = ["gten_host_model_resident", "gten_host_batch_resident", "gten_host_resident_plan"]
+    RESIDENT_BLOCK_BYTES = {"f16": 64, "q8": 34, "q4": 18}
     BEAM_ENDED = ("eos", "length")
     SAMPLES_MAX = 64
 
@@ -169,6 +171,10 @@
         self._m_fsm_states = _sig(L, "gten_host_model_fsm_states", ci, [vp, ci, ci, vp])
         self._b_fsm_states = _sig(L, "gten_host_batch_fsm_states", ci, [vp, ci, ci, ci, vp])
         self._b_fsm_decoder = _sig(L, "gten_host_batch_fsm_decoder", vp, [vp])
+        ll, llp = C.c_longlong, C.POINTER(C.c_longlong)
+        self._m_resident = _sig(L, "gten_host_model_resident", ci, [vp, C.POINTER(ci), llp, llp, llp])
+        self._b_resident = _sig(L, "gten_host_batch_resident", ci, [vp, C.POINTER(ci), llp, llp, llp])
+        self._resident_plan = _sig(L, "gten_host_resident_plan", ci, [ci, ci, ci, ci, ci, ci, ll, vp, vp, llp])
         self._generate_fsm = _sig(L, "gten_host_model_generate_fsm", ci, [vp, vp, ci, ci, ci, ci, C.c_float, C.c_uint64, C.c_uint32, ci, ci, ci,
                                                                           C.c_float, C.c_float, vp, vp, vp, pen, ci, vp])
         self._bgen_fsm = _sig(L, "gten_host_batch_generate_fsm", ci, [vp, vp, vp, ci, ci, ci, vp, vp, ci, C.c_float, C.c_uint64, vp, vp, vp, vp, vp,
@@ -344,6 +350,21 @@
         self._stoks(out.ctypes.data_as(C.c_void_p), count, seed, n_vocab)
         return out
 
+    def resident_plan(self, n_layers, n_embd, n_ffn, kv_width, n_vocab, block_bytes, budget):
+        n = 4 * n_layers + 1
+        res, each, total = np.zeros(n, np.uint8), np.zeros(n, np.int64), C.c_longlong(0)
+        got = self._resident_plan(n_layers, n_embd, n_ffn, kv_width, n_vocab, block_bytes, int(budget), _ptr(res), _ptr(each), C.byref(total))
+        if got < 0:
+            raise GtenHipError(f"resident_plan rc={got}")
+        return res, each, got, total.value
+
+    def _resident_of(self, fn, h):
+        n, b, budget, over = C.c_int(0), C.c_longlong(0), C.c_longlong(0), C.c_longlong(0)
+        rc = fn(h, C.byref(n), C.byref(b), C.byref(budget), C.byref(over))
+        if rc:
+            raise GtenHipError(f"resident rc={rc}: {self.hip._err().decode(errors='replace')}")
+        return n.value, b.value, budget.value, over.value
+
     def model(self, cfg):
         return HostModel(self, cfg)
 
@@ -828,6 +849,9 @@
         rc = self.set_cut_rc(top_p, min_p)
         if rc:
             raise GtenHipError(f"set_cut rc={rc}: {self.host.hip._err().decode(errors='replace')}")
+
+    def resident(self):
+        return self.host._resident_of(self.host._m_resident, self.h)
 
     def cut_info(self):
         a, b, t = np.zeros(1, np.float32), np.zeros(1, np.float32), np.zeros(1, np.float32)
@@ -1139,6 +1163,9 @@
         rc = self.set_cut_rc(seq, top_p, min_p)
         if rc:
             raise GtenHipError(f"batch_set_cut rc={rc}: {self.host.hip._err().decode(errors='replace')}")
+
+    def resident(self):
+        return self.host._resident_of(self.host._b_resident, self.h)
 
     def cut_info(self):
         a, b, t = np.zeros(self.n_seq, np.float32), np.zeros(self.n_seq, np.float32), np.zeros(self.n_seq, np.float32)
```

New measurement: 2173 tok/s, median of 6. 1.02x the previous value.
